# Furyton/Recommender-Baseline-Model

Measured on AMD Instinct MI355X. Metric: training sequences/sec, SASRec L=200 d=128 at 1/2/4/8 MI355X; HR@10 parity, higher is better.
Workload: dtype bf16; 1 GPU; SASRec ML-1M shape (|items|=3416, seq_len=200, d=128, 2 blocks, 1 head, dropout 0.2); model=SASRec, global_batch=128, per_gpu_batch=128, seq_len=200, hidden=128, blocks=2, heads=1, num_items=3416, parallelism=dp1, hip_graph=True, bench_config=cfg2, sampler=host, steps_per_graph=10, full=False

## Files before the change

include/recsys_hip.h:

```cpp
#ifndef RECSYS_HIP_H
#define RECSYS_HIP_H
#include <stdint.h>
#ifdef __cplusplus
extern "C" {
#endif

#define RS_ERR_ARG 1001
#define RS_ERR_UNSUPPORTED 1002

typedef struct rs_epilogue {
  const float* bias;
  float alpha;
  int act;
  const void* aux;
  void* aux_out;
  int64_t ldaux;
  float drop_p;
  uint64_t drop_seed;
  const uint64_t* seed_base;
  int64_t drop_ld;
  const void* resid;
  int64_t ldres;
  const int64_t* rowmask_ids;
  int accumulate;
// ... 153 lines not shown
#define RS_STAMP_WGRAD_GROUPED 2
#define RS_STAMP_VOCAB_CE_FWD 3
int rs_kernel_stamps(uint64_t* buf, const double* step, int kind_mask);
int rs_kernel_stamp_count(void);
int rs_kernel_stamp_kinds(int* kinds, int n);
int rs_wall_clock_khz(int* khz);

int rs_seed_advance(uint64_t* seed_base, void* stream);
int rs_graph_upload(void* graph_exec, void* stream);

#ifdef __HIPCC__
typedef __bf16 rs_bf16;
#else
typedef uint16_t rs_bf16;
#endif

typedef struct rs_sas_embed_args {
  const int64_t* ids;
  const rs_bf16* item_emb;
  const rs_bf16* pos_emb;
  int64_t T;
  float scale;
  float drop_p;
  uint64_t salt;
  const uint64_t* seed_base;
  rs_bf16* x0;
  const int64_t* count_ids;
  int* count_parts;
} rs_sas_embed_args;

typedef struct rs_sas_in_args {
  int64_t M;
  const rs_bf16* x;
  int64_t ldx;
  const float* ln_w;
  const float* ln_b;
  float eps;
  rs_bf16* Q;
  float* mean;
  float* rstd;
  const rs_bf16* Wq;
  const float* bq;
  rs_bf16* q;
  const rs_bf16* Wkv;
  const float* bkv;
  rs_bf16* kv;
  rs_sas_embed_args e;
} rs_sas_in_args;

typedef struct rs_sas_head_args {
  const rs_bf16* E;
  const int64_t* pos;
  const int64_t* neg;
  const float* ln_w;
  const float* ln_b;
  float eps;
  const int* count_parts;
  int ncount;
  const float* divisor;
  rs_bf16* f;
  float* pl;
  float* nl;
  float* dpl;
  float* dnl;
  rs_bf16* dx;
  float* lnpart;
  float* part;
} rs_sas_head_args;

typedef struct rs_sas_out_args {
  int64_t M;
  const rs_bf16* o;
  const rs_bf16* Q;
  const rs_bf16* Wo;
  const float* bo;
  rs_bf16* x1;
  const float* ln_w;
  const float* ln_b;
  float eps;
  rs_bf16* z;
  float* mean;
  float* rstd;
  const rs_bf16* W1;
  const float* b1;
  rs_bf16* h1;
  const rs_bf16* W2;
  const float* b2;
  rs_bf16* xn;
  const int64_t* ids;
  float drop_p;
  uint64_t salt1;
  uint64_t salt2;
  const uint64_t* seed_base;
  rs_sas_head_args h;
} rs_sas_out_args;

typedef struct rs_sas_out_bwd_args {
  int64_t M;
  const rs_bf16* dxn;
  const int64_t* ids;
  const rs_bf16* h1;
  const rs_bf16* x1;
  const float* mean2;
  const float* rstd2;
  const float* ln_w;
  const rs_bf16* W2T;
  const rs_bf16* W1T;
  const rs_bf16* WoT;
  rs_bf16* dy2;
  rs_bf16* da1;
  rs_bf16* dx1;
  rs_bf16* dout;
  float* part;
  float drop_p;
  uint64_t salt1;
  uint64_t salt2;
  const uint64_t* seed_base;
  const rs_bf16* o;
  float* delta;
} rs_sas_out_bwd_args;

typedef struct rs_sas_in_bwd_args {
  int64_t M;
  const rs_bf16* dq;
  const rs_bf16* dkv;
  const rs_bf16* dx1;
  const rs_bf16* x;
  const float* mean1;
  const float* rstd1;
  const float* ln_w;
  const rs_bf16* WinT;
  int64_t ldwt;
  rs_bf16* dx;
  float* part;
} rs_sas_in_bwd_args;

int64_t rs_sas_block_grid(int64_t M);
int rs_sas_block_boundary_fused(int64_t M, int64_t d);

int rs_sas_block_in(int64_t d, const rs_sas_in_args* in, void* stream);
int rs_sas_block_out(int64_t d, const rs_sas_out_args* out, void* stream);
int rs_sas_block_out_bwd_delta(int64_t d, const rs_sas_out_bwd_args* out_bwd, void* stream);
int rs_sas_block_out_bwd(int64_t M, int64_t d, const void* dxn, const int64_t* ids, const void* h1, const void* x1,
                         const float* mean2, const float* rstd2, const float* ln_w, const void* W2T, const void* W1T,
                         const void* WoT, void* dy2, void* da1, void* dx1, void* dout, float* part, float drop_p,
                         uint64_t salt1, uint64_t salt2, const uint64_t* seed_base, void* stream);
int rs_sas_block_in_bwd(int64_t d, const rs_sas_in_bwd_args* in_bwd, void* stream);
int rs_sas_block_out_in(int64_t d, const rs_sas_out_args* out, const rs_sas_in_args* in, void* stream);
int rs_sas_block_in_out_bwd(int64_t d, const rs_sas_in_bwd_args* in_bwd, const rs_sas_out_bwd_args* out_bwd,
                            void* stream);
int rs_sas_block_out_head_bwd(int64_t d, const rs_sas_out_args* out, const rs_sas_out_bwd_args* out_bwd,
                              void* stream);

int64_t rs_touched_rows_ws_numel(int64_t rows);
int rs_touched_rows(const int64_t* ids, int64_t n, int64_t rows, int32_t* flags, int32_t* index, int32_t* count,
                    int32_t* ws, void* stream);
int rs_rows_pack(const float* src, int64_t rows, int64_t d, const int32_t* index, const int32_t* count,
                 float* compact, int64_t cap, void* stream);
int rs_rows_unpack(float* dst, int64_t rows, int64_t d, const int32_t* index, const float* compact, void* stream);

int64_t rs_unique_rows_ws_bytes(int64_t table_rows);
int rs_unique_rows(const int64_t* keys0, int64_t n0, const int64_t* keys1, int64_t n1, const int64_t* keys2,
                   int64_t n2, int64_t table_rows, int32_t* rows, int32_t* count, int64_t cap, void* ws,
                   int64_t ws_bytes, void* stream);
int rs_adam_rows(int64_t d, int64_t table_rows, const int32_t* rows, const int32_t* count, int64_t cap, float* p,
                 float* g, float* m, float* v, void* p_bf16, const double* state, const double* hyper, int zero_grad,
                 int max_wg, void* stream);

int rs_sgd_step(int64_t n, float* p, float* g, float* buf, void* p_bf16, double* state, const double* hyper,
                int zero_grad, int prepare, const float* grad_divisor, uint64_t* seed_base, const int64_t* tdesc,
                int ntd, int64_t tbase, void* wT, const float* loss_sum, float* loss_out, int max_wg, void* stream);

int rs_transpose_bf16(int64_t nmat, const int64_t* desc, int64_t max_tiles, const void* src, void* dst,
                      void* stream);

typedef struct {
  const void* dY; int64_t lddy;
  const void* X;  int64_t ldx;
  int64_t N, K;
  float* dW;
  float* db;
} rs_wgrad_problem;
typedef struct {
  const float* src; int64_t stride; int64_t splits; int64_t n; float* out;
} rs_reduce_segment;
int64_t rs_wgrad_grouped_slab_numel(int nprob, const rs_wgrad_problem* probs, int64_t M, int64_t rows_per_split);
int rs_wgrad_grouped_tile(int nprob, const rs_wgrad_problem* probs);
int rs_wgrad_grouped_tile_max(int nprob, const rs_wgrad_problem* probs, int max_tile);
int rs_wgrad_grouped(int nprob, const rs_wgrad_problem* probs, int64_t M, int64_t rows_per_split, float* slab,
                     int64_t slab_numel, int nextra, const rs_reduce_segment* extra, void* stream);
int rs_wgrad_grouped_max(int nprob, const rs_wgrad_problem* probs, int64_t M, int64_t rows_per_split, float* slab,
                         int64_t slab_numel, int nextra, const rs_reduce_segment* extra, int max_tile, void* stream);

int rs_wgrad_grouped_pos(int nprob, const rs_wgrad_problem* probs, int64_t M, int64_t rows_per_split, float* slab,
                         int64_t slab_numel, int nextra, const rs_reduce_segment* extra, const int64_t* ids,
                         int64_t T, const void* dx, int64_t d, float drop_p, uint64_t salt,
                         const uint64_t* seed_base, float* dpos, void* stream);
int rs_wgrad_grouped_pos_stats(int nprob, const rs_wgrad_problem* probs, int64_t M, int64_t rows_per_split,
                               float* slab, int64_t slab_numel, int nextra, const rs_reduce_segment* extra,
                               const int64_t* ids, int64_t T, const void* dx, int64_t d, float drop_p, uint64_t salt,
                               const uint64_t* seed_base, float* dpos, const float* head_part, int64_t head_blocks,
                               const float* head_divisor, float* loss_out, float* aux_out, void* stream);
int rs_reduce_segments(int nseg, const rs_reduce_segment* segs, int accumulate, void* stream);

int64_t rs_item_index_ws_bytes(int nsrc, int64_t rows, int64_t table_rows, int64_t d);
int rs_item_index_build(int nsrc, const int64_t* keys0, const int64_t* keys1, const int64_t* keys2, int64_t rows,
                        int64_t table_rows, int64_t d, void* ws, int64_t ws_bytes, void* stream);
int rs_item_index_layout(int nsrc, int64_t rows, int64_t table_rows, int64_t d, int64_t* out);
int rs_item_grad(const void* ws, int nsrc, int64_t rows, int64_t table_rows, int64_t d, const void* dx, float scale,
                 float drop_p, uint64_t salt, const uint64_t* seed_base, const void* f, const float* w1,
                 const float* w2, float* dtable, void* stream);
int rs_item_grad_marked(const void* ws, int nsrc, int64_t rows, int64_t table_rows, int64_t d, const void* dx,
                        float scale, float drop_p, uint64_t salt, const uint64_t* seed_base, const void* f,
                        const float* w1, const float* w2, float* dtable, uint8_t* row_marks, uint8_t* epoch_out,
                        void* stream);
int rs_item_grad_f32(const void* ws, int nsrc, int64_t rows, int64_t table_rows, int64_t d, const float* dx, float scale,
                     float drop_p, uint64_t salt, const uint64_t* seed_base, const float* f, const float* w1,
                     const float* w2, float* dtable, void* stream);

int rs_sas_head_fwd(int64_t M, int64_t d, const void* x, const float* ln_w, const float* ln_b, float eps, void* f,
                    float* mean, float* rstd, const void* E, const int64_t* pos, const int64_t* neg, float* pl,
                    float* nl, float* part, void* stream);
int rs_sas_head_bwd(int64_t M, int64_t d, const float* part, const float* divisor, float* out, const float* pl,
                    const float* nl, const float* dpl_in, const float* dnl_in, float* dpl, float* dnl,
                    const int64_t* pos, const int64_t* neg, const void* E, const void* x, const float* ln_w,
                    const float* mean, const float* rstd, void* dx, float* lnpart, void* stream);
int rs_sas_head_finish(int64_t nblk, const float* part, const float* divisor, float* out, void* stream);

int rs_sas_sample(const int64_t* user_offsets, const int64_t* user_items, int64_t n_users, int64_t item_num,
                  int64_t batch, int64_t max_len, uint64_t* seed_base, uint64_t salt, int64_t* seq, int64_t* pos,
                  int64_t* neg, void* stream);
int rs_bert_mask(const int64_t* user_offsets, const int64_t* user_items, int64_t n_users, int64_t num_items,
                 int64_t batch, int64_t max_len, double mask_prob, const int64_t* perm, uint64_t* state, uint64_t salt,
                 int64_t* tokens, int64_t* labels, void* stream);
int rs_sas_sample_draws(const int64_t* user_offsets, const int64_t* user_items, int64_t n_users, int64_t item_num,
                        int64_t batch, int64_t max_len, uint64_t* seed_base, uint64_t salt, int64_t* seq, int64_t* pos,
                        int64_t* neg, int64_t* draws, void* stream);
int rs_bert_mask_draws(const int64_t* user_offsets, const int64_t* user_items, int64_t n_users, int64_t num_items,
                       int64_t batch, int64_t max_len, double mask_prob, const int64_t* perm, uint64_t* state,
                       uint64_t salt, int64_t* tokens, int64_t* labels, int64_t* draws, void* stream);

int rs_rank_metrics(const float* scores, const float* labels, int64_t rows, int64_t cands, int nk, const int* ks,
                    float* ws, float* out, void* stream);

#define RS_TOPK_MAX 128
int64_t rs_full_ws_bytes(int dtype, int64_t B, int64_t d, int64_t nrange, int64_t K);
int rs_full_rank(int dtype, const void* h, int64_t ldh, int64_t B, int64_t d, const void* E, int64_t lde,
                 const float* bias, int64_t v_lo, int64_t v_hi, const int64_t* target, const int64_t* excl, int64_t nx,
                 int64_t ldx, void* ws, int* rank, float* target_score, void* stream);
int rs_full_topk(int dtype, const void* h, int64_t ldh, int64_t B, int64_t d, const void* E, int64_t lde,
                 const float* bias, int64_t v_lo, int64_t v_hi, const int64_t* excl, int64_t nx, int64_t ldx, int64_t K,
                 void* ws, int64_t* ids, float* scores, void* stream);
int rs_rank_to_metrics(const int* rank, int64_t rows, int nk, const int* ks, float* ws, float* out, void* stream);

int rs_sas_ce_rows_fwd(int dtype, int64_t M, int64_t d, const void* x, int64_t ldx, const int64_t* labels,
                       int64_t cap, const float* gamma, const float* beta, float eps, int32_t* idx, int32_t* rank,
                       int32_t* count, float* divisor, void* hl, int64_t ldh, int64_t* lab, float* mean, float* rstd,
                       void* stream);
int64_t rs_sas_ce_rows_nparts(int64_t M);
int rs_sas_ce_rows_bwd(int dtype, int64_t M, int64_t d, const float* slab, int splits, int64_t cap,
                       const int32_t* rank, const void* x, int64_t ldx, const float* gamma, const float* mean,
                       const float* rstd, void* dx, int64_t lddx, float* part, void* stream);

int64_t rs_sas_sce_max_k(void);
int64_t rs_sas_sce_ws_bytes(int64_t cap, int64_t K, int64_t d);
int64_t rs_sas_sce_dh_splits(int64_t cap, int64_t K, int64_t d);
int rs_sas_sce_fwd(int dtype, int64_t cap, int64_t d, const void* hl, int64_t ldh, const int64_t* lab,
                   const int32_t* count, const void* E, int64_t V1, const int64_t* cand, int64_t K,
                   const float* divisor, void* ws, float* out, void* stream);
int rs_sas_sce_bwd(int dtype, int64_t cap, int64_t d, const void* hl, int64_t ldh, const int64_t* lab,
                   const int32_t* count, const void* E, int64_t V1, const int64_t* cand, int64_t K,
                   const float* divisor, const float* dloss, void* ws, float* dh, float* coef, float* pg, float* dEc,
                   int64_t* keys, void* stream);
int rs_uniform_items(const uint64_t* seed_base, uint64_t salt, int64_t item_num, int64_t K, int64_t* out,
                     void* stream);

int64_t rs_sce_head_ws_bytes(int dtype, int64_t cap, int64_t K, int64_t d, int has_bias);
int64_t rs_sce_head_dh_splits(int dtype, int64_t cap, int64_t K, int64_t d);
int rs_sce_head_path(int dtype, int64_t d);
int rs_sce_head_fwd(int dtype, int64_t cap, int64_t d, const void* hl, int64_t ldh, const int64_t* lab,
                    const int32_t* count, const void* E, const float* bias, int64_t V1, const int64_t* cand, int64_t K,
                    const float* divisor, void* ws, float* out, void* stream);
int rs_sce_head_bwd(int dtype, int64_t cap, int64_t d, const void* hl, int64_t ldh, const int64_t* lab,
                    const int32_t* count, const void* E, const float* bias, int64_t V1, const int64_t* cand, int64_t K,
                    const float* divisor, const float* dloss, void* ws, float* dh, float* coef, float* pg, float* dEc,
                    float* dbc, int64_t* keys, void* stream);

int rs_sce_head_logq_fwd(int dtype, int64_t cap, int64_t d, const void* hl, int64_t ldh, const int64_t* lab,
                         const int32_t* count, const void* E, const float* bias, const float* logq, int64_t V1,
                         const int64_t* cand, int64_t K, const float* divisor, void* ws, float* out, void* stream);
int rs_sce_head_logq_bwd(int dtype, int64_t cap, int64_t d, const void* hl, int64_t ldh, const int64_t* lab,
                         const int32_t* count, const void* E, const float* bias, const float* logq, int64_t V1,
                         const int64_t* cand, int64_t K, const float* divisor, const float* dloss, void* ws, float* dh,
                         float* coef, float* pg, float* dEc, float* dbc, int64_t* keys, void* stream);
int rs_alias_items(const uint64_t* seed_base, uint64_t salt, const uint64_t* table, int64_t item_num, int64_t K,
                   int64_t* out, void* stream);

int rs_abi_version(void);
enum {
  RS_SIZEOF_EPILOGUE = 0,
  RS_SIZEOF_WGRAD_PROBLEM = 1,
  RS_SIZEOF_REDUCE_SEGMENT = 2,
  RS_SIZEOF_SAS_EMBED_ARGS = 3,
  RS_SIZEOF_SAS_IN_ARGS = 4,
  RS_SIZEOF_SAS_HEAD_ARGS = 5,
  RS_SIZEOF_SAS_OUT_ARGS = 6,
  RS_SIZEOF_SAS_OUT_BWD_ARGS = 7,
  RS_SIZEOF_SAS_IN_BWD_ARGS = 8
};
int64_t rs_abi_sizeof(int which);

#ifdef __cplusplus
}
#endif
#endif
```

recommender-baseline-model_amd/_lib.py:

```python
import ctypes as C
import os

import torch

PKG = os.path.dirname(os.path.abspath(__file__))
LIB_PATH = os.path.join(PKG, "librecsys_hip.so" if not os.environ.get("RS_LIB_VARIANT")
                        else f"librecsys_hip.{os.environ['RS_LIB_VARIANT']}.so")

F32, BF16 = 0, 1

i32, i64, u64, f32, f64, vp = C.c_int, C.c_int64, C.c_uint64, C.c_float, C.c_double, C.c_void_p


class Epilogue(C.Structure):
    _fields_ = [
        ("bias", vp), ("alpha", f32), ("act", i32),
        ("aux", vp), ("aux_out", vp), ("ldaux", i64),
        ("drop_p", f32), ("drop_seed", u64), ("seed_base", vp), ("drop_ld", i64),
        ("resid", vp), ("ldres", i64),
        ("rowmask_ids", vp), ("accumulate", i32),
        ("post_drop_p", f32), ("post_drop_seed", u64), ("rows_dev", vp),
    ]


class WgradProblem(C.Structure):
    _fields_ = [("dY", vp), ("lddy", i64), ("X", vp), ("ldx", i64), ("N", i64), ("K", i64), ("dW", vp), ("db", vp)]


class ReduceSegment(C.Structure):
    _fields_ = [("src", vp), ("stride", i64), ("splits", i64), ("n", i64), ("out", vp)]


class SasEmbedArgs(C.Structure):
    _fields_ = [("ids", vp), ("item_emb", vp), ("pos_emb", vp), ("T", i64), ("scale", f32), ("drop_p", f32),
                ("salt", u64), ("seed_base", vp), ("x0", vp), ("count_ids", vp), ("count_parts", vp)]


class SasInArgs(C.Structure):
    _fields_ = [("M", i64), ("x", vp), ("ldx", i64), ("ln_w", vp), ("ln_b", vp), ("eps", f32), ("Q", vp),
                ("mean", vp), ("rstd", vp), ("Wq", vp), ("bq", vp), ("q", vp), ("Wkv", vp), ("bkv", vp), ("kv", vp),
                ("e", SasEmbedArgs)]


class SasHeadArgs(C.Structure):
    _fields_ = [("E", vp), ("pos", vp), ("neg", vp), ("ln_w", vp), ("ln_b", vp), ("eps", f32), ("count_parts", vp),
                ("ncount", i32), ("divisor", vp), ("f", vp), ("pl", vp), ("nl", vp), ("dpl", vp), ("dnl", vp),
                ("dx", vp), ("lnpart", vp), ("part", vp)]


class SasOutArgs(C.Structure):
    _fields_ = [("M", i64), ("o", vp), ("Q", vp), ("Wo", vp), ("bo", vp), ("x1", vp), ("ln_w", vp), ("ln_b", vp),
                ("eps", f32), ("z", vp), ("mean", vp), ("rstd", vp), ("W1", vp), ("b1", vp), ("h1", vp), ("W2", vp),
                ("b2", vp), ("xn", vp), ("ids", vp), ("drop_p", f32), ("salt1", u64), ("salt2", u64),
                ("seed_base", vp), ("h", SasHeadArgs)]


class SasOutBwdArgs(C.Structure):
    _fields_ = [("M", i64), ("dxn", vp), ("ids", vp), ("h1", vp), ("x1", vp), ("mean2", vp), ("rstd2", vp),
                ("ln_w", vp), ("W2T", vp), ("W1T", vp), ("WoT", vp), ("dy2", vp), ("da1", vp), ("dx1", vp),
                ("dout", vp), ("part", vp), ("drop_p", f32), ("salt1", u64), ("salt2", u64), ("seed_base", vp),
                ("o", vp), ("delta", vp)]


class SasInBwdArgs(C.Structure):
    _fields_ = [("M", i64), ("dq", vp), ("dkv", vp), ("dx1", vp), ("x", vp), ("mean1", vp), ("rstd1", vp),
                ("ln_w", vp), ("WinT", vp), ("ldwt", i64), ("dx", vp), ("part", vp)]


STRUCTS = {"rs_epilogue": Epilogue, "rs_wgrad_problem": WgradProblem, "rs_reduce_segment": ReduceSegment,
           "rs_sas_embed_args": SasEmbedArgs, "rs_sas_in_args": SasInArgs, "rs_sas_head_args": SasHeadArgs,
           "rs_sas_out_args": SasOutArgs, "rs_sas_out_bwd_args": SasOutBwdArgs, "rs_sas_in_bwd_args": SasInBwdArgs}

ACT_NONE, ACT_RELU, ACT_GELU, ACT_RELU_BWD, ACT_GELU_BWD = 0, 1, 2, 3, 4

SIGNATURES = {
    "rs_gemm": [i32, i32, i32, i64, i64, i64, vp, i64, vp, i64, vp, i64, i32, C.POINTER(Epilogue), i32, vp, vp],
    "rs_gemm_ln": [i64, i64, i64, vp, i64, vp, vp, f32, vp, i64, vp, i64, C.POINTER(Epilogue), vp, i64, vp, vp, vp],
    "rs_reduce_slabs": [vp, i32, i64, vp, i32, vp],
    "rs_reduce_slabs2": [vp, i32, i64, vp, i64, vp, i32, vp],
    "rs_linear_wgrad": [i32, i64, i64, i64, vp, i64, vp, i64, vp, vp, i32, i32, vp, vp, vp],
    "rs_colsum": [i32, vp, i64, i64, i64, vp, vp, i32, vp],
    "rs_embed_fwd": [i32, i32, vp, i64, i64, vp, vp, i64, f32, f32, u64, vp, vp, vp],
    "rs_embed_bwd": [i32, i32, vp, i64, i64, vp, i64, f32, f32, u64, vp, vp, vp, i32, vp],
    "rs_layernorm_fwd": [i32, i32, vp, i64, i64, i64, vp, vp, f32, vp, i64, vp, vp, vp],
    "rs_layernorm_bwd_nparts": [i32, i64, i64],
    "rs_layernorm_bwd_drop": [i32, i32, vp, i64, vp, i64, i64, i64, vp, vp, vp, f32, vp, i64, i32, vp, vp, vp, f32,
                              u64, u64, vp, vp, vp, vp],
    "rs_layernorm_bwd": [i32, i32, vp, i64, vp, i64, i64, i64, vp, vp, vp, f32, vp, i64, i32, vp, vp, vp, vp],
    "rs_attn_fwd": [i32, i64, i64, i64, i64, vp, i64, vp, i64, vp, i64, vp, i64, vp, f32, i32, vp, f32, u64, vp, vp],
    "rs_attn_row_delta": [i32, i64, i64, i64, i64, vp, i64, vp, i64, vp, vp],
    "rs_attn_bwd": [i32, i64, i64, i64, i64, vp, i64, vp, i64, vp, i64, vp, i64, vp, i64, vp, vp, i64, vp, i64,
                    vp, i64, f32, i32, vp, f32, u64, vp, vp, vp],
    "rs_sampled_logits_fwd": [i32, vp, i64, i64, vp, vp, vp, vp, vp, vp],
    "rs_sampled_logits_bwd": [i32, vp, i64, i64, vp, vp, vp, vp, vp, vp, i32, vp, vp],
    "rs_bce_fwd": [vp, vp, vp, i64, vp, vp, vp, vp],
    "rs_bce_bwd": [vp, vp, vp, i64, vp, vp, vp, vp, vp],
    "rs_ce_fwd": [vp, i64, i64, i64, vp, vp, vp, vp, vp, vp],
    "rs_ce_bwd": [i32, vp, i64, i64, i64, vp, vp, vp, vp, vp, i64, vp, vp],
    "rs_compact_rows": [vp, i64, i64, vp, vp, vp, vp],
    "rs_gather_rows": [i32, vp, i64, i64, vp, vp, i64, vp, i64, vp, vp, vp],
    "rs_scatter_rows": [i32, vp, i64, i64, vp, i64, vp, i64, vp],
    "rs_candidate_scores": [i32, vp, i64, i64, i64, vp, vp, vp, i64, i64, vp, vp],
    "rs_gemm_n256_splits": [i64, i64],
    "rs_gemm_n256": [i32, i64, i64, vp, i64, vp, i64, vp, i64, i32, i64, vp, vp, vp],
    "rs_adam_prepare": [vp, vp, vp, vp, vp],
    "rs_adam_step": [i64, vp, vp, vp, vp, vp, vp, vp, i32, vp],
    "rs_adam_step_wg": [i64, vp, vp, vp, vp, vp, vp, vp, i32, i32, vp],
    "rs_adam_step_marked": [i64, vp, vp, vp, vp, vp, vp, vp, i32, i32, vp, vp, i64, i64, i32, vp],
    "rs_graph_upload": [vp, vp],
    "rs_adam_prepare_step": [i64, vp, vp, vp, vp, vp, vp, vp, i32, vp, vp, vp, i32, i64, vp, vp],
    "rs_adam_prepare_step_loss": [i64, vp, vp, vp, vp, vp, vp, vp, i32, vp, vp, vp, i32, i64, vp, vp, vp, vp],
    "rs_adam_prepare_step_marked": [i64, vp, vp, vp, vp, vp, vp, vp, i32, vp, vp, vp, i32, i64, vp, vp, vp, vp, vp,
                                    i64, i64, i32, vp],
    "rs_cast_bf16": [i64, vp, vp, vp],
    "rs_l2_penalty": [vp, vp, vp, i64, f32, vp, vp, vp, vp],
    "rs_dropout_rowmask": [i32, vp, i64, i64, i64, f32, u64, vp, i64, vp, vp, vp, vp],
    "rs_dropout2": [i32, vp, i64, i64, i64, f32, u64, u64, vp, i64, vp, vp, vp],
    "rs_vocab_ce_ws_numel": [i64, i64],
    "rs_vocab_ce_fwd": [i64, i64, i64, vp, i64, vp, i64, vp, vp, vp, vp, vp, vp, vp],
    "rs_vocab_ce_bwd": [i64, i64, i64, vp, i64, vp, i64, vp, vp, vp, vp, vp, vp, vp, i64, vp],
    "rs_vocab_head_supported": [i64],
    "rs_vocab_head_fwd": [i64, i64, i64, vp, i64, vp, i64, vp, vp, vp, vp, vp, vp, vp],
    "rs_vocab_head_bwd": [i64, i64, i64, vp, i64, vp, i64, vp, vp, vp, vp, vp, vp, vp, i64, i64, vp],
    "rs_vocab_shard_lse": [i64, i64, i64, vp, i64, vp, i64, vp, vp, vp, vp, vp],
    "rs_vocab_shard_label_logits": [i64, i64, vp, i64, vp, i64, vp, vp, i64, i64, vp, vp],
    "rs_vocab_shard_combine": [i32, i64, vp, vp, vp, vp, vp, vp],
    "rs_seed_advance": [vp, vp],
    "rs_touched_rows_ws_numel": [i64],
    "rs_touched_rows": [vp, i64, i64, vp, vp, vp, vp, vp],
    "rs_rows_pack": [vp, i64, i64, vp, vp, vp, i64, vp],
    "rs_rows_unpack": [vp, i64, i64, vp, vp, vp],
    "rs_unique_rows_ws_bytes": [i64],
    "rs_unique_rows": [vp, i64, vp, i64, vp, i64, i64, vp, vp, i64, vp, i64, vp],
    "rs_adam_rows": [i64, i64, vp, vp, i64, vp, vp, vp, vp, vp, vp, vp, i32, i32, vp],
    "rs_sgd_step": [i64, vp, vp, vp, vp, vp, vp, i32, i32, vp, vp, vp, i32, i64, vp, vp, vp, i32, vp],
    "rs_sas_block_grid": [i64],
    "rs_sas_block_boundary_fused": [i64, i64],
    "rs_sas_block_in": [i64, C.POINTER(SasInArgs), vp],
    "rs_sas_block_out": [i64, C.POINTER(SasOutArgs), vp],
    "rs_sas_block_out_bwd_delta": [i64, C.POINTER(SasOutBwdArgs), vp],
    "rs_sas_block_out_bwd": [i64, i64, vp, vp, vp, vp, vp, vp, vp, vp, vp, vp, vp, vp, vp, vp, vp, f32, u64, u64,
                             vp, vp],
    "rs_sas_block_in_bwd": [i64, C.POINTER(SasInBwdArgs), vp],
    "rs_sas_block_out_in": [i64, C.POINTER(SasOutArgs), C.POINTER(SasInArgs), vp],
    "rs_sas_block_in_out_bwd": [i64, C.POINTER(SasInBwdArgs), C.POINTER(SasOutBwdArgs), vp],
    "rs_sas_block_out_head_bwd": [i64, C.POINTER(SasOutArgs), C.POINTER(SasOutBwdArgs), vp],
    "rs_wgrad_grouped": [i32, C.POINTER(WgradProblem), i64, i64, vp, i64, i32, C.POINTER(ReduceSegment), vp],
    "rs_reduce_segments": [i32, C.POINTER(ReduceSegment), i32, vp],
    "rs_wgrad_grouped_slab_numel": [i32, C.POINTER(WgradProblem), i64, i64],
    "rs_wgrad_grouped_tile": [i32, C.POINTER(WgradProblem)],
    "rs_wgrad_grouped_tile_max": [i32, C.POINTER(WgradProblem), i32],
    "rs_wgrad_grouped_max": [i32, C.POINTER(WgradProblem), i64, i64, vp, i64, i32, C.POINTER(ReduceSegment), i32, vp],
    "rs_item_index_ws_bytes": [i32, i64, i64, i64],
    "rs_item_index_build": [i32, vp, vp, vp, i64, i64, i64, vp, i64, vp],
    "rs_item_index_layout": [i32, i64, i64, i64, C.POINTER(i64)],
    "rs_sas_head_fwd": [i64, i64, vp, vp, vp, f32, vp, vp, vp, vp, vp, vp, vp, vp, vp, vp],
    "rs_sas_head_finish": [i64, vp, vp, vp, vp],
    "rs_sas_head_bwd": [i64, i64, vp, vp, vp, vp, vp, vp, vp, vp, vp, vp, vp, vp, vp, vp, vp, vp, vp, vp, vp],
    "rs_item_grad": [vp, i32, i64, i64, i64, vp, f32, f32, u64, vp, vp, vp, vp, vp, vp],
    "rs_item_grad_marked": [vp, i32, i64, i64, i64, vp, f32, f32, u64, vp, vp, vp, vp, vp, vp, vp, vp],
    "rs_item_grad_f32": [vp, i32, i64, i64, i64, vp, f32, f32, u64, vp, vp, vp, vp, vp, vp],
    "rs_wgrad_grouped_pos": [i32, C.POINTER(WgradProblem), i64, i64, vp, i64, i32, C.POINTER(ReduceSegment),
                             vp, i64, vp, i64, f32, u64, vp, vp, vp],
    "rs_wgrad_grouped_pos_stats": [i32, C.POINTER(WgradProblem), i64, i64, vp, i64, i32, C.POINTER(ReduceSegment),
                                   vp, i64, vp, i64, f32, u64, vp, vp, vp, i64, vp, vp, vp, vp],
    "rs_transpose_bf16": [i64, vp, i64, vp, vp, vp],
    "rs_sas_sample": [vp, vp, i64, i64, i64, i64, vp, u64, vp, vp, vp, vp],
    "rs_bert_mask": [vp, vp, i64, i64, i64, i64, f64, vp, vp, u64, vp, vp, vp],
    "rs_sas_sample_draws": [vp, vp, i64, i64, i64, i64, vp, u64, vp, vp, vp, vp, vp],
    "rs_bert_mask_draws": [vp, vp, i64, i64, i64, i64, f64, vp, vp, u64, vp, vp, vp, vp],
    "rs_splitk_scatter_rows": [i32, vp, i32, i64, i64, vp, i64, vp, i64, vp],
    "rs_rank_metrics": [vp, vp, i64, i64, i32, vp, vp, vp, vp],
    "rs_full_ws_bytes": [i32, i64, i64, i64, i64],
    "rs_full_rank": [i32, vp, i64, i64, i64, vp, i64, vp, i64, i64, vp, vp, i64, i64, vp, vp, vp, vp],
    "rs_full_topk": [i32, vp, i64, i64, i64, vp, i64, vp, i64, i64, vp, i64, i64, i64, vp, vp, vp, vp],
    "rs_rank_to_metrics": [vp, i64, i32, vp, vp, vp, vp],
    "rs_sas_ce_rows_fwd": [i32, i64, i64, vp, i64, vp, i64, vp, vp, f32, vp, vp, vp, vp, vp, i64, vp, vp, vp, vp],
    "rs_sas_ce_rows_nparts": [i64],
    "rs_sas_ce_rows_bwd": [i32, i64, i64, vp, i32, i64, vp, vp, i64, vp, vp, vp, vp, i64, vp, vp],
    "rs_sas_sce_max_k": [],
    "rs_sas_sce_ws_bytes": [i64, i64, i64],
    "rs_sas_sce_dh_splits": [i64, i64, i64],
    "rs_sas_sce_fwd": [i32, i64, i64, vp, i64, vp, vp, vp, i64, vp, i64, vp, vp, vp, vp],
    "rs_sas_sce_bwd": [i32, i64, i64, vp, i64, vp, vp, vp, i64, vp, i64, vp, vp, vp, vp, vp, vp, vp, vp, vp],
    "rs_uniform_items": [vp, u64, i64, i64, vp, vp],
    "rs_sce_head_ws_bytes": [i32, i64, i64, i64, i32],
    "rs_sce_head_dh_splits": [i32, i64, i64, i64],
    "rs_sce_head_path": [i32, i64],
    "rs_sce_head_fwd": [i32, i64, i64, vp, i64, vp, vp, vp, vp, i64, vp, i64, vp, vp, vp, vp],
    "rs_sce_head_bwd": [i32, i64, i64, vp, i64, vp, vp, vp, vp, i64, vp, i64, vp, vp, vp, vp, vp, vp, vp, vp, vp,
                        vp],
    "rs_sce_head_logq_fwd": [i32, i64, i64, vp, i64, vp, vp, vp, vp, vp, i64, vp, i64, vp, vp, vp, vp],
    "rs_sce_head_logq_bwd": [i32, i64, i64, vp, i64, vp, vp, vp, vp, vp, i64, vp, i64, vp, vp, vp, vp, vp, vp, vp, vp,
                             vp, vp],
    "rs_alias_items": [vp, u64, vp, i64, i64, vp, vp],
    "rs_kernel_stamps": [vp, vp, i32],
    "rs_kernel_stamp_count": [],
    "rs_kernel_stamp_kinds": [C.POINTER(i32), i32],
    "rs_wall_clock_khz": [C.POINTER(i32)],
    "rs_attn_bwd_plan": [i64, i64, i64, i32, vp, C.POINTER(i32)],
    "rs_attn_lds_regime": [i32, i64, i64, i64, i64, i32, C.POINTER(i32)],
    "rs_abi_version": [],
    "rs_abi_sizeof": [i32],
}

RESTYPES = {"rs_wgrad_grouped_slab_numel": C.c_int64, "rs_abi_sizeof": C.c_int64,
            "rs_touched_rows_ws_numel": C.c_int64, "rs_item_index_ws_bytes": C.c_int64,
            "rs_unique_rows_ws_bytes": C.c_int64,
            "rs_vocab_ce_ws_numel": C.c_int64, "rs_full_ws_bytes": C.c_int64,
            "rs_sas_block_grid": C.c_int64, "rs_layernorm_bwd_nparts": C.c_int64,
            "rs_sas_ce_rows_nparts": C.c_int64, "rs_sas_sce_max_k": C.c_int64,
            "rs_sas_sce_ws_bytes": C.c_int64, "rs_sas_sce_dh_splits": C.c_int64,
            "rs_sce_head_ws_bytes": C.c_int64, "rs_sce_head_dh_splits": C.c_int64}

_lib = None


def lib():
    global _lib
    if _lib is None:
        if not os.path.exists(LIB_PATH):
            raise RuntimeError(
                f"librecsys_hip.so not found at {LIB_PATH}; build it with "
                "`python recommender-baseline-model_amd/build.py` (there is no CPU fallback)")
        h = C.CDLL(LIB_PATH)
        for name, argt in SIGNATURES.items():
            fn = getattr(h, name)
            fn.argtypes = argt
            fn.restype = RESTYPES.get(name, C.c_int)
        _lib = h
    return _lib


def call(name, *args):
    rc = getattr(lib(), name)(*args)
    if rc != 0:
        raise RuntimeError(f"{name} failed with code {rc}")


def ptr(t):
    return None if t is None else t.data_ptr()


def stream():
    return torch.cuda.current_stream().cuda_stream
```

recommender-baseline-model_amd/build.py:

```python
import concurrent.futures as cf
import glob
import os
import subprocess
import sys

PKG = os.path.dirname(os.path.abspath(__file__))
ROOT = os.path.dirname(PKG)
CSRC = os.path.join(PKG, "csrc")
OBJ = os.path.join(CSRC, "build")
LIB = os.path.join(PKG, "librecsys_hip.so")
HIPCC = os.environ.get("HIPCC", "/opt/rocm/bin/hipcc")
ARCH = os.environ.get("RS_OFFLOAD_ARCH", "gfx950")
LINK_LAST = ("sas_ce.hip", "sas_sce.hip", "adam_rows.hip", "sgd.hip")
FLAGS = ["-O3", "-std=c++17", "-fPIC", f"--offload-arch={ARCH}", "-munsafe-fp-atomics",
         "-I", os.path.join(ROOT, "include"), "-I", CSRC]


def _headers_mtime():
    hs = glob.glob(os.path.join(CSRC, "*.h")) + glob.glob(os.path.join(ROOT, "include", "*.h"))
    return max((os.path.getmtime(h) for h in hs), default=0.0)


def _included(path):
    with open(path) as fh:
        return fh.readline().startswith("// rs-build: included")


def _included_mtime():
    inc = [p for p in glob.glob(os.path.join(CSRC, "*.hip")) if _included(p)]
    return max((os.path.getmtime(p) for p in inc), default=0.0)


def _compile(src, force):
    obj = os.path.join(OBJ, os.path.basename(src) + ".o")
    if not force and os.path.exists(obj):
        if os.path.getmtime(obj) >= max(os.path.getmtime(src), _headers_mtime(), _included_mtime()):
            return obj, False
    cmd = [HIPCC, *FLAGS, "-c", src, "-o", obj]
    r = subprocess.run(cmd, capture_output=True, text=True)
    if r.returncode != 0:
        raise RuntimeError(f"hipcc failed for {src}:\n{r.stdout}\n{r.stderr}")
    return obj, True


def build(force=False, jobs=None):
    os.makedirs(OBJ, exist_ok=True)
    srcs = [p for p in sorted(glob.glob(os.path.join(CSRC, "*.hip"))) if not _included(p)]
    srcs.sort(key=lambda p: LINK_LAST.index(os.path.basename(p)) + 1 if os.path.basename(p) in LINK_LAST else 0)
    jobs = jobs or min(len(srcs), max(1, min(8, os.cpu_count() or 1)))
    with cf.ThreadPoolExecutor(jobs) as ex:
        results = list(ex.map(lambda s: _compile(s, force), srcs))
    objs = [o for o, _ in results]
    rebuilt = any(b for _, b in results)
    if rebuilt or force or not os.path.exists(LIB) or \
            os.path.getmtime(LIB) < max(os.path.getmtime(o) for o in objs):
        cmd = [HIPCC, "-shared", "-fPIC", f"--offload-arch={ARCH}", *objs, "-o", LIB]
        r = subprocess.run(cmd, capture_output=True, text=True)
        if r.returncode != 0:
            raise RuntimeError(f"link failed:\n{r.stdout}\n{r.stderr}")
    return LIB


if __name__ == "__main__":
    print(build(force="--force" in sys.argv))
```

recommender-baseline-model_amd/csrc/attention_lds.hip:

```cpp
#include "common.h"
#include <algorithm>
#include <cstring>
#include "../../include/recsys_hip.h"

typedef __attribute__((ext_vector_type(4))) __bf16 bf4;
typedef __bf16 bf16;

#define PLAN_S 4
#define PLAN_I 6
struct AttnLdsArgs {
  int64_t B, T, H;
  const bf16* q; int64_t ldq;
  const bf16* k; int64_t ldk;
  const bf16* v; int64_t ldv;
  const bf16* o; int64_t ldo;
  const bf16* dout; int64_t lddo;
  bf16* out; int64_t ldout;
  bf16* dq; int64_t lddq;
  bf16* dk; int64_t lddk;
  bf16* dv; int64_t lddv;
  float* lse;
  float* delta;
  int delta_in;
  float scale;
// ... 67 lines not shown
  u4 v = *reinterpret_cast<const u4*>(base + rc * ld + col);
  const unsigned keep = row < T ? 0xffffffffu : 0u;
  v &= keep;
  return __builtin_bit_cast(bf16x8, v);
}

typedef __attribute__((address_space(3))) void* lds_ptr_t;
__device__ __forceinline__ uint32_t lds_addr(const void* p) { return (uint32_t)(uintptr_t)(lds_ptr_t)p; }
__device__ __forceinline__ void dma16(const void* gsrc, uint32_t dst) {
  unsigned keep;
  asm volatile("s_mov_b32 %0, m0\n\ts_mov_b32 m0, %2\n\ts_nop 0\n\tglobal_load_lds_dwordx4 %1, off\n\ts_mov_b32 m0, %0"
               : "=&s"(keep)
               : "v"(gsrc), "s"(dst)
               : "memory");
}
template <int N> __device__ __forceinline__ void vm_wait_n() { asm volatile("s_waitcnt vmcnt(%0)" ::"i"(N) : "memory"); }
#define LOADER (NW - 1)
#define NCNT 16
template <int DH> struct DmaStage {
  static constexpr int ROWB = Img<DH>::LD * 2, CHB = 32 * ROWB, PPC = CHB / 1024, PP = 2 * PPC, WIN = 3;
  static_assert(CHB % 1024 == 0, "a 32-row chunk is whole DMA pieces");
  static_assert(WIN * PP <= 63, "chunks in flight fit vmcnt");
  static __device__ __forceinline__ void chunk(const bf16* A, int64_t ldA, uint32_t la, const bf16* B, int64_t ldB,
                                               uint32_t lb, int T, int c, int lane) {
#pragma unroll
    for (int j = 0; j < PP; ++j) {
      const bool second = j >= PPC;
      const int pj = second ? j - PPC : j;
      const int off = c * CHB + pj * 1024 + lane * 16;
      const int row = off / ROWB, o = off - row * ROWB;
      const int col = o < DH * 2 ? o >> 1 : 0;
      const int64_t rr = row < T ? row : T - 1;
      const bf16* src = second ? B + rr * ldB + col : A + rr * ldA + col;
      dma16(src, __builtin_amdgcn_readfirstlane((second ? lb : la) + (uint32_t)(c * CHB + pj * 1024)));
    }
  }
  static __device__ __forceinline__ void prime(const bf16* A, int64_t ldA, const bf16* imgA, const bf16* B,
                                               int64_t ldB, const bf16* imgB, int T, int nch, int lane) {
    const uint32_t la = lds_addr(imgA), lb = lds_addr(imgB);
    for (int c = 0; c < min(nch, WIN); ++c) chunk(A, ldA, la, B, ldB, lb, T, c, lane);
  }
  static __device__ __forceinline__ void stream(const bf16* A, int64_t ldA, const bf16* imgA, const bf16* B,
                                                int64_t ldB, const bf16* imgB, int T, int nch, int* flag, int lane) {
    const uint32_t la = lds_addr(imgA), lb = lds_addr(imgB);
    for (int c = 0; c < nch; ++c) {
      const int later = min(nch, c + WIN) - (c + 1);
      if (later >= 2) vm_wait_n<2 * PP>();
      else if (later == 1) vm_wait_n<PP>();
      else vm_wait_n<0>();
      if (lane == 0) __hip_atomic_store(&flag[c], 1, __ATOMIC_RELAXED, __HIP_MEMORY_SCOPE_WORKGROUP);
      if (c + WIN < nch) chunk(A, ldA, la, B, ldB, lb, T, c + WIN, lane);
    }
  }
};
struct ChunkWait {
  const int* flag;
  int nch, ready;
  __device__ __forceinline__ void ensure(int c) {
    c = min(c, nch - 1);
    if (c <= ready) return;
    for (int spin = 0; spin < (1 << 22) &&
                       __hip_atomic_load(&flag[c], __ATOMIC_RELAXED, __HIP_MEMORY_SCOPE_WORKGROUP) == 0;
         ++spin)
      __builtin_amdgcn_s_sleep(1);
    asm volatile("" ::: "memory");
    ready = c;
  }
};
__device__ __forceinline__ void lds_barrier() {
  asm volatile("s_waitcnt lgkmcnt(0)" ::: "memory");
  __builtin_amdgcn_s_barrier();
  asm volatile("" ::: "memory");
}

template <int DH>
__device__ __forceinline__ void stage(bf16* img, const bf16* src, int64_t ld, int64_t T, int rows, int tid) {
  constexpr int CPR = DH / 8, LD = Img<DH>::LD, U = 8;
  const int n = rows * CPR;
  for (int i0 = tid; i0 < n; i0 += NT * U) {
    bf16x8 v[U];
#pragma unroll
    for (int u = 0; u < U; ++u) {
      const int i = min(i0 + u * NT, n - 1);
      v[u] = gload8(src, ld, i / CPR, T, (i % CPR) * 8);
    }
#pragma unroll
    for (int u = 0; u < U; ++u) {
      const int i = i0 + u * NT;
      if (i < n) *reinterpret_cast<bf16x8*>(img + (i / CPR) * LD + (i % CPR) * 8) = v[u];
    }
  }
}

template <int DH>
__device__ __forceinline__ void stage2(bf16* imgA, const bf16* srcA, int64_t ldA, bf16* imgB, const bf16* srcB,
                                       int64_t ldB, int64_t T, int rows, int tid) {
  constexpr int CPR = DH / 8, LD = Img<DH>::LD, U = 8;
  const int n = rows * CPR;
  for (int i0 = tid; i0 < n; i0 += NT * U) {
    bf16x8 va[U], vb[U];
#pragma unroll
    for (int u = 0; u < U; ++u) {
      const int i = min(i0 + u * NT, n - 1);
      va[u] = gload8(srcA, ldA, i / CPR, T, (i % CPR) * 8);
      vb[u] = gload8(srcB, ldB, i / CPR, T, (i % CPR) * 8);
    }
#pragma unroll
    for (int u = 0; u < U; ++u) {
      const int i = i0 + u * NT;
      if (i < n) {
        *reinterpret_cast<bf16x8*>(imgA + (i / CPR) * LD + (i % CPR) * 8) = va[u];
        *reinterpret_cast<bf16x8*>(imgB + (i / CPR) * LD + (i % CPR) * 8) = vb[u];
      }
    }
  }
}

__device__ __forceinline__ void stage_keymask(float* km, const AttnLdsArgs& a, int64_t b, int rows, int tid) {
  for (int i = tid; i < rows; i += NT)
    km[i] = (a.mask_kind == 1 && i < a.T && a.ids[b * a.T + i] == 0) ? 1.f : 0.f;
}

__device__ __forceinline__ int mask_state(const AttnLdsArgs& a, const float* km, int64_t q, int64_t key) {
  if (key >= a.T) return 1;
  if (a.mask_kind == 0) return key > q ? 1 : 0;
  return km[key] != 0.f ? 2 : 0;
}
__device__ __forceinline__ float apply_mask(int st, float s) { return st == 0 ? s : (st == 1 ? NEG_INF : -1e9f); }
__device__ __forceinline__ float masked(const AttnLdsArgs& a, const float* km, int64_t q, int64_t key, float s) {
  return apply_mask(mask_state(a, km, q, key), s);
}

__device__ __forceinline__ void block_coords(const AttnLdsArgs& a, int64_t lin, int64_t& bh, int& split) {
  const int ns = a.nsplit;
  const int64_t BH = a.B * a.H;
  if (BH % 8 == 0) {
    const int64_t xcd = lin & 7, slot = lin >> 3;
    bh = xcd * (BH >> 3) + slot / ns;
    split = (int)(slot % ns);
  } else {
    bh = lin / ns;
    split = (int)(lin % ns);
  }
}
__device__ __forceinline__ void block_coords(const AttnLdsArgs& a, int64_t& bh, int& split) {
  block_coords(a, blockIdx.x + (int64_t)a.nsplit * blockIdx.y, bh, split);
}

__device__ __forceinline__ int last_tile_of_split(int nq, int split, int nsplit) {
  return split + ((nq - 1 - split) / nsplit) * nsplit;
}

template <int DH>
__global__ __launch_bounds__(NT) void attn_fwd_lds_kernel(AttnLdsArgs a) {
  constexpr int LD = Img<DH>::LD, KC = DH / 32, DT = DH / 16, NKT = 16;
  extern __shared__ __attribute__((aligned(16))) char smem[];
  APROF(0);
  const int tid = threadIdx.x, lane = tid & 63, wave = __builtin_amdgcn_readfirstlane(tid >> 6), g = lane >> 4, cl = lane & 15;
  int64_t bh;
  int split;
  block_coords(a, bh, split);
  const int64_t b = bh / a.H, h = bh % a.H;
  const int T = (int)a.T;
  const int nq = (T + 15) / 16;
  if (split >= nq) return;
  const int lastq = last_tile_of_split(nq, split, a.nsplit);
  const int kneed = a.mask_kind == 0 ? min(T, 16 * (lastq + 1)) : T;
  const int rows = ((kneed + 31) / 32) * 32;
  bf16* Ks = reinterpret_cast<bf16*>(smem);
  bf16* Vs = Ks + rows * LD;
  float* km = reinterpret_cast<float*>(Vs + rows * LD);
  const bf16* Kg = a.k + b * a.T * a.ldk + h * DH;
  const bf16* Vg = a.v + b * a.T * a.ldv + h * DH;
  const bf16* Qg = a.q + b * a.T * a.ldq + h * DH;
  bf16x8 qf[KC];
  {
    const int64_t qrow0 = (split + wave * a.nsplit) * 16 + cl;
#pragma unroll
    for (int kc = 0; kc < KC; ++kc) qf[kc] = gload8(Qg, a.ldq, qrow0, a.T, kc * 32 + 8 * g);
  }
  stage2<DH>(Ks, Kg, a.ldk, Vs, Vg, a.ldv, a.T, rows, tid);
  stage_keymask(km, a, b, rows, tid);
  __syncthreads();
  APROF(1);
  const uint64_t seed = eff_seed(a.seed, a.seed_base);
  if (wave >= NW / 2) __builtin_amdgcn_s_setprio(1);

  for (int qt = split + wave * a.nsplit; qt < nq; qt += NW * a.nsplit) {
    const int q0 = qt * 16;
    const int64_t qrow = q0 + cl;
    if (qt != split + wave * a.nsplit) {
#pragma unroll
      for (int kc = 0; kc < KC; ++kc) qf[kc] = gload8(Qg, a.ldq, qrow, a.T, kc * 32 + 8 * g);
    }
    const int nkt = a.mask_kind == 0 ? qt + 1 : nq;
    const float sl2 = a.scale * LOG2E;
    const int qi = q0 + cl;
    f32x4 s[NKT];
    float mx = NEG_INF;
#pragma unroll
    for (int kt = 0; kt < NKT; ++kt) {
      s[kt] = (f32x4){0.f, 0.f, 0.f, 0.f};
      if (kt < nkt) {
#pragma unroll
        for (int kc = 0; kc < KC; ++kc) s[kt] = mfma16(row_frag(Ks, LD, kt * 16 + cl, kc * 32 + 8 * g), qf[kc], s[kt]);
        const bool need = a.mask_kind != 0 || kt == qt || kt * 16 + 16 > T;
        const int kb = kt * 16 + 4 * g;
        if (need) {
          const f32x4 kmv = *reinterpret_cast<const f32x4*>(km + kb);
#pragma unroll
          for (int r = 0; r < 4; ++r) {
            const int k = kb + r;
            const bool dead = (k >= T) | ((a.mask_kind == 0) & (k > qi));
            const float x = s[kt][r] * sl2;
            s[kt][r] = dead ? NEG_INF : (kmv[r] != 0.f ? MASK2 : x);
            mx = fmaxf(mx, s[kt][r]);
          }
        } else {
#pragma unroll
          for (int r = 0; r < 4; ++r) {
            s[kt][r] *= sl2;
            mx = fmaxf(mx, s[kt][r]);
          }
        }
      }
    }
    mx = max_xor32(max_xor16(mx));
    float sm = 0.f;
#pragma unroll
    for (int kt = 0; kt < NKT; ++kt) {
      if (kt < nkt) {
#pragma unroll
        for (int r = 0; r < 4; ++r) {
          const float e = ex2(s[kt][r] - mx);
          s[kt][r] = e;
          sm += e;
        }
      }
    }
    sm = add_xor32(add_xor16(sm));
    const float inv = 1.f / sm;
    if (g == 0 && qrow < a.T) a.lse[bh * a.T + qrow] = (mx + __builtin_amdgcn_logf(sm)) * LN2;
    const uint32_t s32 = seed32(seed);
    const uint32_t rowidx = (uint32_t)(((int)bh * T + qi) * (T + (T & 1)));
    f32x4 o[DT];
#pragma unroll
    for (int dt = 0; dt < DT; ++dt) o[dt] = (f32x4){0.f, 0.f, 0.f, 0.f};
#pragma unroll
    for (int c = 0; c < NKT / 2; ++c) {
      if (2 * c < nkt) {
        f32x4 pp[2] = {s[2 * c], s[2 * c + 1]};
#pragma unroll
        for (int hf = 0; hf < 2; ++hf) {
          const int t = 2 * c + hf;
          const float sc = t < nkt ? inv : 0.f;
          if (a.drop_p > 0.f) {
            float m[4];
            const uint32_t base = rowidx + (uint32_t)(t * 16 + 4 * g);
            drop_mul2(a.drop_p, s32, base, m[0], m[1]);
            drop_mul2(a.drop_p, s32, base + 2, m[2], m[3]);
#pragma unroll
            for (int r = 0; r < 4; ++r) pp[hf][r] *= sc * m[r];
          } else {
#pragma unroll
            for (int r = 0; r < 4; ++r) pp[hf][r] *= sc;
          }
        }
        const bf16x8 pb = pack8(pp[0], pp[1]);
#pragma unroll
        for (int dt = 0; dt < DT; ++dt) o[dt] = mfma16(tr_frag(Vs, LD, 32 * c, 16 * dt, lane), pb, o[dt]);
      }
    }
    if (qrow < a.T) {
      bf16* O = a.out + (b * a.T + qrow) * a.ldout + h * DH;
#pragma unroll
      for (int dt = 0; dt < DT; ++dt) {
        bf4 w;
        w[0] = (bf16)o[dt][0]; w[1] = (bf16)o[dt][1]; w[2] = (bf16)o[dt][2]; w[3] = (bf16)o[dt][3];
        *reinterpret_cast<bf4*>(O + 16 * dt + 4 * g) = w;
      }
    }
  }
  APROF(2);
}

template <int DH>
__device__ __forceinline__ void attn_bwd_dq_body(const AttnLdsArgs& a, int64_t lin) {
  constexpr int LD = Img<DH>::LD, KC = DH / 32, DT = DH / 16;
  extern __shared__ __attribute__((aligned(16))) char smem[];
  APROF(4);
  const int tid = threadIdx.x, lane = tid & 63, wave = __builtin_amdgcn_readfirstlane(tid >> 6), g = lane >> 4, cl = lane & 15;
  int64_t bh;
  int split;
  block_coords(a, lin, bh, split);
  const int64_t b = bh / a.H, h = bh % a.H;
  const int T = (int)a.T;
  const int nq = (T + 15) / 16;
  if (split >= nq) return;
  const int lastq = last_tile_of_split(nq, split, a.nsplit);
  const int kneed = a.mask_kind == 0 ? min(T, 16 * (lastq + 1)) : T;
  const int rows = ((kneed + 31) / 32) * 32;
  bf16* Ks = reinterpret_cast<bf16*>(smem);
  bf16* Vs = Ks + rows * LD;
  float* km = reinterpret_cast<float*>(Vs + rows * LD);
  int* cnt = reinterpret_cast<int*>(km + rows);
  float* slots = km + rows + NCNT;
  int* flags = reinterpret_cast<int*>(slots + DQ_SLOTS * DT * 4 * 64);
  const bf16* Qg = a.q + b * a.T * a.ldq + h * DH;
  const bf16* Og = a.o + b * a.T * a.ldo + h * DH;
  const bf16* dOg = a.dout + b * a.T * a.lddo + h * DH;
  auto item = [&](int it, int& qt, int& cb, int& ce, int& role, int& slot) -> bool {
    if (a.use_plan) {
      if (it >= PLAN_I) return false;
      const uint32_t e = a.plan[split][wave][it];
      if (!(e >> 31)) return false;
      qt = e & 255; cb = (e >> 8) & 255; ce = (e >> 16) & 255; role = (e >> 24) & 3; slot = (e >> 26) & 15;
      return true;
    }
    qt = split + (wave + it * NW) * a.nsplit;
    if (qt >= nq) return false;
    cb = 0;
    ce = ((a.mask_kind == 0 ? qt + 1 : nq) + 1) / 2;
    role = 0; slot = 0;
    return true;
  };
  if (a.use_plan && tid < DQ_SLOTS) flags[tid] = 0;
  if (tid < NCNT) cnt[tid] = 0;
  const int nch = rows / 32;
  bf16x8 qf[KC], df[KC], of[KC];
  int qt0 = 0, cb0, ce0, role0, slot0;
  const bool any = item(0, qt0, cb0, ce0, role0, slot0);
  const bf16* Kg = a.k + b * a.T * a.ldk + h * DH;
  const bf16* Vg = a.v + b * a.T * a.ldv + h * DH;
  if (wave == LOADER) {
    DmaStage<DH>::prime(Kg, a.ldk, Ks, Vg, a.ldv, Vs, T, nch, lane);
  } else {
    const int64_t qrow0 = (any ? qt0 : 0) * 16 + cl;
#pragma unroll
    for (int kc = 0; kc < KC; ++kc) {
      qf[kc] = gload8(Qg, a.ldq, qrow0, a.T, kc * 32 + 8 * g);
      df[kc] = gload8(dOg, a.lddo, qrow0, a.T, kc * 32 + 8 * g);
      if (!a.delta_in) of[kc] = gload8(Og, a.ldo, qrow0, a.T, kc * 32 + 8 * g);
    }
  }
  stage_keymask(km, a, b, rows, tid);
  lds_barrier();
  if (wave == LOADER) DmaStage<DH>::stream(Kg, a.ldk, Ks, Vg, a.ldv, Vs, T, nch, cnt, lane);
  ChunkWait ch{cnt, nch, wave == LOADER ? nch - 1 : -1};
  APROF(5);
  const uint64_t seed = eff_seed(a.seed, a.seed_base);

  if (wave >= NW / 2) __builtin_amdgcn_s_setprio(1);
  int qt, cb, ce, role, slot;
  for (int it = 0; item(it, qt, cb, ce, role, slot); ++it) {
    const int q0 = qt * 16;
    const int64_t qrow = q0 + cl;
    if (it > 0 || wave == LOADER) {
#pragma unroll
      for (int kc = 0; kc < KC; ++kc) {
        qf[kc] = gload8(Qg, a.ldq, qrow, a.T, kc * 32 + 8 * g);
        df[kc] = gload8(dOg, a.lddo, qrow, a.T, kc * 32 + 8 * g);
        if (!a.delta_in) of[kc] = gload8(Og, a.ldo, qrow, a.T, kc * 32 + 8 * g);
      }
    }
    float dl = 0.f;
    if (a.delta_in) {
      dl = a.delta[bh * a.T + (qrow < a.T ? qrow : a.T - 1)];
    } else {
#pragma unroll
      for (int kc = 0; kc < KC; ++kc) {
#pragma unroll
        for (int j = 0; j < 8; ++j) dl += (float)df[kc][j] * (float)of[kc][j];
      }
      dl = add_xor32(add_xor16(dl));
      if (role != 1 && g == 0 && qrow < a.T) a.delta[bh * a.T + qrow] = dl;
    }
    const float lq2 = (qrow < a.T ? a.lse[bh * a.T + qrow] : 0.f) * LOG2E;
    const float sl2 = a.scale * LOG2E;
    const int qi = q0 + cl;
    const uint32_t s32 = seed32(seed);
    const uint32_t rowidx = (uint32_t)(((int)bh * T + qi) * (T + (T & 1)));
    const bool qok = qi < T;
    const int nkt = a.mask_kind == 0 ? qt + 1 : nq;
    f32x4 acc[DT];
#pragma unroll
    for (int dt = 0; dt < DT; ++dt) acc[dt] = (f32x4){0.f, 0.f, 0.f, 0.f};
    const int tmax = rows / 16 - 1;
    auto sdp = [&](int t, f32x4& sv, f32x4& dp) {
      const int tr = min(t, tmax);
      bf16x8 fk[KC], fv[KC];
#pragma unroll
      for (int kc = 0; kc < KC; ++kc) {
        fk[kc] = row_frag(Ks, LD, tr * 16 + cl, kc * 32 + 8 * g);
        fv[kc] = row_frag(Vs, LD, tr * 16 + cl, kc * 32 + 8 * g);
      }
      sv = (f32x4){0.f, 0.f, 0.f, 0.f};
      dp = (f32x4){0.f, 0.f, 0.f, 0.f};
#pragma unroll
      for (int kc = 0; kc < KC; ++kc) {
        sv = mfma16(fk[kc], qf[kc], sv);
        dp = mfma16(fv[kc], df[kc], dp);
      }
    };
    auto dsv = [&](int t, const f32x4& sv, const f32x4& dp, f32x4& ds) {
      const bool need = a.mask_kind != 0 || t >= qt || t * 16 + 16 > T;
      const int kb = t * 16 + 4 * g;
      float m[4] = {1.f, 1.f, 1.f, 1.f};
      if (a.drop_p > 0.f) {
        drop_mul2(a.drop_p, s32, rowidx + (uint32_t)kb, m[0], m[1]);
        drop_mul2(a.drop_p, s32, rowidx + (uint32_t)kb + 2, m[2], m[3]);
      }
      const bool tok = (t < nkt) & qok, causal = a.mask_kind == 0;
      float pe[4];
#pragma unroll
      for (int r = 0; r < 4; ++r) pe[r] = ex2(sv[r] * sl2 - lq2) * a.scale;
      if (need) {
        const f32x4 kmv = *reinterpret_cast<const f32x4*>(km + kb);
#pragma unroll
        for (int r = 0; r < 4; ++r) {
          const int k = kb + r;
          const bool live = tok & (k < T) & !(causal & (k > qi)) & (kmv[r] == 0.f);
          const float v = pe[r] * (dp[r] * m[r] - dl);
          ds[r] = live ? v : 0.f;
        }
      } else {
#pragma unroll
        for (int r = 0; r < 4; ++r) ds[r] = tok ? pe[r] * (dp[r] * m[r] - dl) : 0.f;
      }
    };
    f32x4 sA, dA, sB, dB, dsA, dsB;
    ch.ensure(cb);
    sdp(2 * cb, sA, dA);
    for (int c = cb; c < ce; ++c) {
      sdp(2 * c + 1, sB, dB);
      dsv(2 * c, sA, dA, dsA);
      if (c + 1 < ce) ch.ensure(c + 1);
      sdp(2 * c + 2, sA, dA);
      dsv(2 * c + 1, sB, dB, dsB);
// ... 173 lines not shown
    for (int dt = 0; dt < DT; ++dt) {
      dk[dt] = (f32x4){0.f, 0.f, 0.f, 0.f};
      dv[dt] = (f32x4){0.f, 0.f, 0.f, 0.f};
    }
    const int tmax = rows / 16 - 1;
    auto sdp = [&](int t, f32x4& sv, f32x4& dp) {
      const int tr = min(t, tmax);
      bf16x8 fq[KC], fo[KC];
#pragma unroll
      for (int kc = 0; kc < KC; ++kc) {
        fq[kc] = row_frag(Qs, LD, tr * 16 + cl, kc * 32 + 8 * g);
        fo[kc] = row_frag(dOs, LD, tr * 16 + cl, kc * 32 + 8 * g);
      }
      sv = (f32x4){0.f, 0.f, 0.f, 0.f};
      dp = (f32x4){0.f, 0.f, 0.f, 0.f};
#pragma unroll
      for (int kc = 0; kc < KC; ++kc) {
        sv = mfma16(fq[kc], kf[kc], sv);
        dp = mfma16(fo[kc], vf[kc], dp);
      }
    };
    const bool kdead = ki >= T, kfill = km[min(ki, rows - 1)] != 0.f;
    auto pds = [&](int t, const f32x4& sv, const f32x4& dp, f32x4& pd, f32x4& ds) {
      const f32x4 ls = *reinterpret_cast<const f32x4*>(lse_s + t * 16 + 4 * g);
      const f32x4 dd = *reinterpret_cast<const f32x4*>(dl_s + t * 16 + 4 * g);
      float m[4] = {1.f, 1.f, 1.f, 1.f};
      if (a.drop_p > 0.f) drop_keys4(a.drop_p, s32, ((uint32_t)bh * (uint32_t)T + (uint32_t)(t * 16 + 4 * g)) * Tp,
                                     Tp, (uint32_t)ki, lane, m);
      const bool need = a.mask_kind != 0 || t <= kt || t * 16 + 16 > T || kt * 16 + 16 > T;
      if (need) {
#pragma unroll
        for (int r = 0; r < 4; ++r) {
          const int qr = t * 16 + 4 * g + r;
          const bool dead = kdead | (qr >= T) | ((a.mask_kind == 0) & (ki > qr));
          const float x2 = kfill ? MASK2 : sv[r] * sl2;
          const float p = ex2(dead ? NEG_INF : x2 - ls[r]);
          pd[r] = p * m[r];
          const float v = p * (dp[r] * m[r] - dd[r]) * a.scale;
          ds[r] = dead | kfill ? 0.f : v;
        }
      } else {
#pragma unroll
        for (int r = 0; r < 4; ++r) {
          const float p = ex2(sv[r] * sl2 - ls[r]);
          pd[r] = p * m[r];
          ds[r] = p * (dp[r] * m[r] - dd[r]) * a.scale;
        }
      }
    };
    f32x4 sA, dA, sB, dB, pdA, dsA, pdB, dsB;
    ch.ensure(cb);
    sdp(2 * cb, sA, dA);
    for (int c = cb; c < ce; ++c) {
      sdp(2 * c + 1, sB, dB);
      pds(2 * c, sA, dA, pdA, dsA);
      if (c + 1 < ce) ch.ensure(c + 1);
      sdp(2 * c + 2, sA, dA);
      pds(2 * c + 1, sB, dB, pdB, dsB);
      const bf16x8 bp = pack8(pdA, pdB);
      const bf16x8 bds = pack8(dsA, dsB);
#pragma unroll
      for (int dt = 0; dt < DT; ++dt) {
        dv[dt] = mfma16(tr_frag(dOs, LD, 32 * c, 16 * dt, lane), bp, dv[dt]);
        dk[dt] = mfma16(tr_frag(Qs, LD, 32 * c, 16 * dt, lane), bds, dk[dt]);
      }
    }
    bf16* sl = slots + slot * (2 * DT * 4 * 64);
    if (role == 1) {
#pragma unroll
      for (int dt = 0; dt < DT; ++dt)
#pragma unroll
        for (int r = 0; r < 4; ++r) {
          sl[(dt * 4 + r) * 64 + lane] = (bf16)dk[dt][r];
          sl[(DT * 4 + dt * 4 + r) * 64 + lane] = (bf16)dv[dt][r];
        }
      asm volatile("s_waitcnt lgkmcnt(0)" ::: "memory");
      if (lane == 0) __hip_atomic_store(&flags[slot], 1, __ATOMIC_RELAXED, __HIP_MEMORY_SCOPE_WORKGROUP);
      continue;
    }
    if (role == 2) {
      for (int spin = 0; spin < (1 << 22) &&
                         __hip_atomic_load(&flags[slot], __ATOMIC_RELAXED, __HIP_MEMORY_SCOPE_WORKGROUP) == 0;
           ++spin)
        __builtin_amdgcn_s_sleep(1);
      asm volatile("" ::: "memory");
#pragma unroll
      for (int dt = 0; dt < DT; ++dt)
#pragma unroll
        for (int r = 0; r < 4; ++r) {
          dk[dt][r] += (float)sl[(dt * 4 + r) * 64 + lane];
          dv[dt][r] += (float)sl[(DT * 4 + dt * 4 + r) * 64 + lane];
        }
    }
    if (key < a.T) {
      bf16* dK = a.dk + (b * a.T + key) * a.lddk + h * DH;
      bf16* dV = a.dv + (b * a.T + key) * a.lddv + h * DH;
#pragma unroll
      for (int dt = 0; dt < DT; ++dt) {
        bf4 wk, wv;
#pragma unroll
        for (int r = 0; r < 4; ++r) {
          wk[r] = (bf16)dk[dt][r];
          wv[r] = (bf16)dv[dt][r];
        }
        *reinterpret_cast<bf4*>(dK + 16 * dt + 4 * g) = wk;
        *reinterpret_cast<bf4*>(dV + 16 * dt + 4 * g) = wv;
      }
    }
  }
  APROF(9);
}

template <int DH>
__global__ __launch_bounds__(NT) void attn_bwd_lds_kernel(AttnLdsArgs aq, AttnLdsArgs akv) {
  KStampBegin begin_(aq.ks);
  KStampEnd end_(aq.ks);
  const int64_t nq = (int64_t)aq.nsplit * aq.B * aq.H;
  if ((int64_t)blockIdx.x < nq) attn_bwd_dq_body<DH>(aq, blockIdx.x);
  else attn_bwd_dkv_body<DH>(akv, blockIdx.x - nq, !akv.delta_in);
}

template <int DH>
static size_t fwd_lds_bytes(int T) {
  const int rows = ((T + 31) / 32) * 32;
  return (size_t)2 * rows * Img<DH>::LD * 2 + rows * 4 + NCNT * 4;
}
template <int DH>
static size_t dkv_lds_bytes(int T) {
  const int rows = ((T + 31) / 32) * 32;
  return (size_t)2 * rows * Img<DH>::LD * 2 + 3 * rows * 4 + NCNT * 4;
}

static int pick_split(int64_t BH, int ntiles) {
  int s = 1;
  while (BH * s < 256 && s * 2 <= std::max(1, ntiles / 4)) s *= 2;
  return s;
}

static int pick_split_bwd(int64_t BH, int ntiles) {
  int s = 1;
  while (2 * BH * s * 2 <= 256 && s * 2 <= std::max(1, ntiles / 4)) s *= 2;
  return s;
}

bool attn_lds_supported(int64_t T, int64_t Dh) {
  if (T <= 0 || T > 256) return false;
  if (Dh != 32 && Dh != 64 && Dh != 128) return false;
  const size_t need = Dh == 128 ? dkv_lds_bytes<128>((int)T) : Dh == 64 ? dkv_lds_bytes<64>((int)T)
                                                                            : dkv_lds_bytes<32>((int)T);
  return need <= 160 * 1024;
}

static int fwd_split(const AttnLdsArgs& a) { return pick_split(a.B * a.H, (int)cdiv(a.T, 16)); }

template <int DH>
static hipError_t fwd_t(AttnLdsArgs& a, hipStream_t s) {
  a.nsplit = fwd_split(a);
  const size_t lds = fwd_lds_bytes<DH>((int)a.T);
  hipLaunchKernelGGL((attn_fwd_lds_kernel<DH>), dim3((unsigned)a.nsplit, (unsigned)(a.B * a.H)), dim3(NT), lds, s,
                     a);
  return hipGetLastError();
}

#define LOADER_HANDICAP 3
struct PlanItem {
  int tile, cb, ce, role, slot;
};

static bool make_plan(AttnLdsArgs& a, int ntiles, bool dkv, int slots) {
  const int T = (int)a.T, nqc = (T + 31) / 32;
  if (a.nsplit > PLAN_S) return false;
  memset(a.plan, 0, sizeof(a.plan));
  for (int sp = 0; sp < a.nsplit; ++sp) {
    PlanItem items[64];
    int n = 0;
    for (int t = sp; t < ntiles; t += a.nsplit) {
      if (n >= 32) return false;
      items[n++] = dkv ? PlanItem{t, t / 2, nqc, 0, 0} : PlanItem{t, 0, (t + 2) / 2, 0, 0};
    }
    std::sort(items, items + n, [](const PlanItem& x, const PlanItem& y) {
      return x.ce - x.cb != y.ce - y.cb ? x.ce - x.cb > y.ce - y.cb : x.tile < y.tile;
    });
    const int n0 = n;
    for (int k = 0, used = 0; k < n0 && used < slots; ++k) {
      PlanItem& it = items[k];
      const int w = it.ce - it.cb;
      if (w < 2) break;
      const int hmid = it.cb + (w + 1) / 2;
      items[n++] = PlanItem{it.tile, hmid, it.ce, 2, used};
      it.ce = hmid;
      it.role = 1;
      it.slot = used++;
    }
    std::sort(items, items + n, [](const PlanItem& x, const PlanItem& y) {
      return x.ce - x.cb != y.ce - y.cb ? x.ce - x.cb > y.ce - y.cb : x.tile < y.tile;
    });
    int load[NW] = {0}, cnt[NW] = {0};
    load[LOADER] = LOADER_HANDICAP;
    PlanItem lists[NW][PLAN_I];
    for (int k = 0; k < n; ++k) {
      int w = 0;
      for (int j = 1; j < NW; ++j)
        if (load[j] < load[w]) w = j;
      if (cnt[w] == PLAN_I) return false;
      lists[w][cnt[w]++] = items[k];
      load[w] += items[k].ce - items[k].cb;
    }
    for (int w = 0; w < NW; ++w) {
      int o = 0;
      for (int pass = 0; pass < 3; ++pass) {
        const int want = pass == 0 ? 1 : pass == 1 ? 0 : 2;
        for (int k = 0; k < cnt[w]; ++k) {
          const PlanItem& it = lists[w][k];
          if (it.role != want) continue;
          a.plan[sp][w][o++] = 1u << 31 | (uint32_t)it.slot << 26 | (uint32_t)it.role << 24 |
                               (uint32_t)it.ce << 16 | (uint32_t)it.cb << 8 | (uint32_t)it.tile;
        }
      }
    }
  }
  return true;
}

extern "C" int rs_attn_bwd_plan(int64_t B, int64_t T, int64_t H, int dkv, uint32_t* plan, int* nsplit) {
  if (B <= 0 || T <= 0 || H <= 0 || !plan || !nsplit) return RS_ERR_ARG;
  AttnLdsArgs a = {};
  a.B = B; a.T = T; a.H = H; a.mask_kind = 0;
  const int nq = (int)cdiv(T, 16);
  a.nsplit = pick_split_bwd(B * H, nq);
  *nsplit = a.nsplit;
  const bool ok = nq >= 8 && make_plan(a, nq, dkv != 0, dkv ? DKV_SLOTS : DQ_SLOTS);
  memcpy(plan, a.plan, sizeof(a.plan));
  return ok ? 0 : RS_ERR_UNSUPPORTED;
}

template <int DH>
static size_t bwd_setup(AttnLdsArgs& a, AttnLdsArgs& aq, AttnLdsArgs& akv) {
  const int nq = (int)cdiv(a.T, 16);
  a.nsplit = pick_split_bwd(a.B * a.H, nq);
  constexpr int DT = DH / 16;
  const size_t lds_q = fwd_lds_bytes<DH>((int)a.T), lds_kv = dkv_lds_bytes<DH>((int)a.T);
  const size_t ext_q = (size_t)DQ_SLOTS * DT * 4 * 64 * 4 + 16, ext_kv = (size_t)DKV_SLOTS * 2 * DT * 4 * 64 * 2 + 16;
  aq = a;
  akv = a;
  const bool want = a.mask_kind == 0 && nq >= 8;
  aq.use_plan = want && lds_q + ext_q <= 160 * 1024 && make_plan(aq, nq, false, DQ_SLOTS);
  akv.use_plan = want && lds_kv + ext_kv <= 160 * 1024 && make_plan(akv, nq, true, DKV_SLOTS);
  const size_t bq = lds_q + (aq.use_plan ? ext_q : 0), bkv = lds_kv + (akv.use_plan ? ext_kv : 0);
  return std::max(bq, bkv);
}

template <int DH>
static hipError_t bwd_t(AttnLdsArgs& a, hipStream_t s) {
  AttnLdsArgs aq, akv;
  const size_t lds = bwd_setup<DH>(a, aq, akv);
  hipLaunchKernelGGL((attn_bwd_lds_kernel<DH>), dim3((unsigned)(2 * a.nsplit * a.B * a.H)), dim3(NT), lds, s, aq,
                     akv);
  return hipGetLastError();
}

void attn_lds_regime(int64_t B, int64_t T, int64_t H, int64_t Dh, int mask_kind, int* out) {
  AttnLdsArgs a = {}, aq, akv;
  a.B = B; a.T = T; a.H = H; a.mask_kind = mask_kind;
  out[0] = fwd_split(a);
  if (Dh == 128) bwd_setup<128>(a, aq, akv);
  else if (Dh == 64) bwd_setup<64>(a, aq, akv);
  else bwd_setup<32>(a, aq, akv);
  out[1] = a.nsplit;
  out[2] = aq.use_plan;
  out[3] = akv.use_plan;
}

template <int DH>
static void set_lds_limits() {
  hipFuncSetAttribute((const void*)attn_fwd_lds_kernel<DH>, hipFuncAttributeMaxDynamicSharedMemorySize, 160 * 1024);
  hipFuncSetAttribute((const void*)attn_bwd_lds_kernel<DH>, hipFuncAttributeMaxDynamicSharedMemorySize, 160 * 1024);
}

static void init_once() {
  static bool done = false;
  if (!done) {
    set_lds_limits<32>();
    set_lds_limits<64>();
    set_lds_limits<128>();
    done = true;
  }
}

hipError_t attn_lds_fwd(int64_t B, int64_t T, int64_t H, int64_t Dh, const void* q, int64_t ldq, const void* k,
                        int64_t ldk, const void* v, int64_t ldv, void* o, int64_t ldo, float* lse, float scale,
                        int mask_kind, const int64_t* ids, float drop_p, uint64_t seed, const uint64_t* seed_base,
                        hipStream_t s) {
  init_once();
  AttnLdsArgs a = {};
  a.B = B; a.T = T; a.H = H;
  a.q = (const bf16*)q; a.ldq = ldq; a.k = (const bf16*)k; a.ldk = ldk; a.v = (const bf16*)v; a.ldv = ldv;
  a.out = (bf16*)o; a.ldout = ldo; a.lse = lse; a.scale = scale; a.mask_kind = mask_kind; a.ids = ids;
  a.drop_p = drop_p; a.seed = seed; a.seed_base = seed_base;
  if (Dh == 128) return fwd_t<128>(a, s);
  if (Dh == 64) return fwd_t<64>(a, s);
  return fwd_t<32>(a, s);
}

hipError_t attn_lds_bwd(int64_t B, int64_t T, int64_t H, int64_t Dh, const void* q, int64_t ldq, const void* k,
                        int64_t ldk, const void* v, int64_t ldv, const void* o, int64_t ldo, const void* dout,
                        int64_t lddo, const float* lse, void* dq, int64_t lddq, void* dk, int64_t lddk, void* dv,
                        int64_t lddv, float scale, int mask_kind, const int64_t* ids, float drop_p, uint64_t seed,
                        const uint64_t* seed_base, float* delta, hipStream_t s) {
  init_once();
  AttnLdsArgs a = {};
  a.B = B; a.T = T; a.H = H;
  a.delta_in = (mask_kind & RS_ATTN_DELTA_IN) != 0;
  mask_kind &= ~RS_ATTN_DELTA_IN;
  a.q = (const bf16*)q; a.ldq = ldq; a.k = (const bf16*)k; a.ldk = ldk; a.v = (const bf16*)v; a.ldv = ldv;
  a.o = (const bf16*)o; a.ldo = ldo; a.dout = (const bf16*)dout; a.lddo = lddo;
  a.dq = (bf16*)dq; a.lddq = lddq; a.dk = (bf16*)dk; a.lddk = lddk; a.dv = (bf16*)dv; a.lddv = lddv;
  a.lse = const_cast<float*>(lse); a.delta = delta; a.scale = scale; a.mask_kind = mask_kind; a.ids = ids;
  a.drop_p = drop_p; a.seed = seed; a.seed_base = seed_base;
  a.ks = kstamp_next(RS_STAMP_ATTN_BWD);
  if (Dh == 128) return bwd_t<128>(a, s);
  if (Dh == 64) return bwd_t<64>(a, s);
  return bwd_t<32>(a, s);
}
```

recommender-baseline-model_amd/csrc/misc.hip:

```cpp
#include "adam_math.h"
#include "common.h"
#include "stream4.h"
#include "../../include/recsys_hip.h"

__device__ __forceinline__ void adam_commit(double* state, double t, AdamScalars c, uint64_t* seed_base) {
  if (seed_base) *seed_base += 1;
  state[0] = t;
  state[1] = c.step_size;
  state[2] = c.bc2s;
  state[3] = c.gs;
}

__global__ void adam_prepare_kernel(double* state, const double* hyper, const float* divisor, uint64_t* seed_base) {
  if (threadIdx.x != 0 || blockIdx.x != 0) return;
  const double t = state[0] + 1.0;
  adam_commit(state, t, adam_scalars(t, hyper, divisor), seed_base);
}

template <bool BF16OUT, bool NT>
__device__ __forceinline__ void adam4(int64_t i, float4 pp, float4 gg, float4 mm, float4 vv, float* __restrict__ p,
                                      float* __restrict__ g, float* __restrict__ m, float* __restrict__ v,
                                      __bf16* __restrict__ pb, AdamElem h,
                                      float step_size, float bc2s, float gs, int zero_grad,
                                      const int64_t* __restrict__ tdesc, int ntd, int64_t tbase,
// ... 359 lines not shown
  RowMarks rm;
  if (int e = row_marks(n, row_marks_, epoch, moff, mrows, dshift, rm)) return e;
  if (!loss_out != !loss_sum || (loss_out && !grad_divisor)) return RS_ERR_ARG;
  if (ntd < 0 || (ntd > 0 && (!tdesc || !wT || !p_bf16))) return RS_ERR_ARG;
#ifndef ADAM_PREP_MAX_WG
#define ADAM_PREP_MAX_WG 2048
#endif
  const int64_t blocks = std::max<int64_t>(1, std::min<int64_t>(cdiv(n / 4, 256), ADAM_PREP_MAX_WG));
  hipStream_t s = (hipStream_t)stream;
  if (p_bf16)
    ADAM_LAUNCH(true, true, dim3((unsigned)blocks), dim3(256), 0, s, n, p, g, m, v,
                       (__bf16*)p_bf16, state, hyper, zero_grad, grad_divisor, seed_base, tdesc, ntd,
                       tbase, (__bf16*)wT, loss_sum, loss_out);
  else
    ADAM_LAUNCH(false, true, dim3((unsigned)blocks), dim3(256), 0, s, n, p, g, m, v,
                       (__bf16*)nullptr, state, hyper, zero_grad, grad_divisor, seed_base, nullptr, 0,
                       0, nullptr, loss_sum, loss_out);
  return (int)hipGetLastError();
}

int rs_cast_bf16(int64_t n, const float* src, void* dst, void* stream) {
  if (n <= 0) return RS_ERR_ARG;
  const int64_t blocks = std::min<int64_t>(cdiv(n, 256), 8192);
  hipLaunchKernelGGL(cast_bf16_kernel, dim3((unsigned)blocks), dim3(256), 0, (hipStream_t)stream, n, src,
                     (__bf16*)dst);
  return (int)hipGetLastError();
}

int rs_colsum(int dtype, const void* X, int64_t M, int64_t N, int64_t ldx, float* ws, float* out, int accumulate,
              void* stream) {
  if (M <= 0 || N <= 0) return RS_ERR_ARG;
  hipStream_t s = (hipStream_t)stream;
  const int nblk = (int)std::min<int64_t>(COLSUM_BLOCKS, cdiv(M, 64));
  hipError_t e = dtype == RS_DTYPE_BF16 ? colsum_partial<__bf16>((const __bf16*)X, M, N, ldx, ws, nblk, s)
                                        : colsum_partial<float>((const float*)X, M, N, ldx, ws, nblk, s);
  if (e != hipSuccess) return (int)e;
  return (int)launch_reduce_slabs(ws, nblk, N, N, out, nullptr, accumulate, s);
}

int rs_dropout_rowmask(int dtype, const void* x, int64_t M, int64_t N, int64_t ld, float drop_p, uint64_t seed,
                       const uint64_t* seed_base, int64_t drop_ld, const int64_t* rowmask_ids, void* out,
                       void* out_masked, void* stream) {
  if (M <= 0 || N <= 0) return RS_ERR_ARG;
  hipStream_t s = (hipStream_t)stream;
  const int es = dtype == RS_DTYPE_BF16 ? 2 : 4;
  if (N % 8 == 0 && ld % 8 == 0 && drop_ld % 2 == 0 && ((uintptr_t)x | (uintptr_t)out | (uintptr_t)out_masked) % 16 == 0) {
    dim3 g8((unsigned)cdiv(M * (N / 8), 256));
    if (es == 2)
      hipLaunchKernelGGL((dropout_v8_kernel<__bf16, false>), g8, dim3(256), 0, s, (const __bf16*)x, M, N, ld, drop_p,
                         seed, 0ull, seed_base, drop_ld, rowmask_ids, (__bf16*)out, (__bf16*)out_masked);
    else
      hipLaunchKernelGGL((dropout_v8_kernel<float, false>), g8, dim3(256), 0, s, (const float*)x, M, N, ld, drop_p,
                         seed, 0ull, seed_base, drop_ld, rowmask_ids, (float*)out, (float*)out_masked);
    return (int)hipGetLastError();
  }
  dim3 grid((unsigned)cdiv(M * N, 256));
  if (dtype == RS_DTYPE_BF16)
    hipLaunchKernelGGL((dropout_rowmask_kernel<__bf16>), grid, dim3(256), 0, s, (const __bf16*)x, M, N, ld, drop_p,
                       seed, seed_base, drop_ld, rowmask_ids, (__bf16*)out, (__bf16*)out_masked);
  else
    hipLaunchKernelGGL((dropout_rowmask_kernel<float>), grid, dim3(256), 0, s, (const float*)x, M, N, ld, drop_p,
                       seed, seed_base, drop_ld, rowmask_ids, (float*)out, (float*)out_masked);
  return (int)hipGetLastError();
}

int rs_dropout2(int dtype, const void* x, int64_t M, int64_t N, int64_t ld, float drop_p, uint64_t salt1,
                uint64_t salt2, const uint64_t* seed_base, int64_t drop_ld, void* out1, void* out2, void* stream) {
  if (M <= 0 || N <= 0 || N % 8 || ld % 8 || drop_ld % 2 || !x || !out1 || !out2 ||
      ((uintptr_t)x | (uintptr_t)out1 | (uintptr_t)out2) % 16)
    return RS_ERR_ARG;
  hipStream_t s = (hipStream_t)stream;
  dim3 g8((unsigned)cdiv(M * (N / 8), 256));
  if (dtype == RS_DTYPE_BF16)
    hipLaunchKernelGGL((dropout_v8_kernel<__bf16, true>), g8, dim3(256), 0, s, (const __bf16*)x, M, N, ld, drop_p,
                       salt1, salt2, seed_base, drop_ld, (const int64_t*)nullptr, (__bf16*)out1, (__bf16*)out2);
  else
    hipLaunchKernelGGL((dropout_v8_kernel<float, true>), g8, dim3(256), 0, s, (const float*)x, M, N, ld, drop_p,
                       salt1, salt2, seed_base, drop_ld, (const int64_t*)nullptr, (float*)out1, (float*)out2);
  return (int)hipGetLastError();
}

__global__ void seed_advance_kernel(uint64_t* s) {
  if (threadIdx.x == 0) *s += 1;
}

int rs_graph_upload(void* graph_exec, void* stream) {
  if (!graph_exec) return RS_ERR_ARG;
  return (int)hipGraphUpload((hipGraphExec_t)graph_exec, (hipStream_t)stream);
}

int rs_seed_advance(uint64_t* seed_base, void* stream) {
  hipLaunchKernelGGL(seed_advance_kernel, dim3(1), dim3(64), 0, (hipStream_t)stream, seed_base);
  return (int)hipGetLastError();
}

static unsigned long long* g_kstamp_buf = nullptr;
static const double* g_kstamp_step = nullptr;
static int g_kstamp_next = 0, g_kstamp_mask = 0;
static int g_kstamp_kind[256];

}

KStamp kstamp_next(int kind) {
  KStamp k{nullptr, nullptr, 0};
  if (g_kstamp_buf && (g_kstamp_mask >> kind & 1)) {
    k.buf = g_kstamp_buf;
    k.step = g_kstamp_step;
    if (g_kstamp_next < 256) g_kstamp_kind[g_kstamp_next] = kind;
    k.mark = g_kstamp_next++;
  }
  return k;
}

extern "C" {

int rs_kernel_stamps(uint64_t* buf, const double* step, int kind_mask) {
  if ((buf == nullptr) != (step == nullptr)) return RS_ERR_ARG;
  g_kstamp_buf = (unsigned long long*)buf;
  g_kstamp_step = step;
  g_kstamp_mask = kind_mask;
  if (buf) g_kstamp_next = 0;
  return 0;
}

int rs_kernel_stamp_kinds(int* kinds, int n) {
  const int m = g_kstamp_next < 256 ? g_kstamp_next : 256;
  for (int i = 0; i < n && i < m; ++i) kinds[i] = g_kstamp_kind[i];
  return 0;
}

int rs_kernel_stamp_count(void) { return g_kstamp_next; }

int rs_wall_clock_khz(int* khz) {
  if (!khz) return RS_ERR_ARG;
  int dev = 0;
  hipError_t e = hipGetDevice(&dev);
  if (e != hipSuccess) return (int)e;
  return (int)hipDeviceGetAttribute(khz, hipDeviceAttributeWallClockRate, dev);
}

int rs_abi_version(void) { return 2; }

int64_t rs_abi_sizeof(int which) {
  switch (which) {
    case RS_SIZEOF_EPILOGUE: return sizeof(rs_epilogue);
    case RS_SIZEOF_WGRAD_PROBLEM: return sizeof(rs_wgrad_problem);
    case RS_SIZEOF_REDUCE_SEGMENT: return sizeof(rs_reduce_segment);
    case RS_SIZEOF_SAS_EMBED_ARGS: return sizeof(rs_sas_embed_args);
    case RS_SIZEOF_SAS_IN_ARGS: return sizeof(rs_sas_in_args);
    case RS_SIZEOF_SAS_HEAD_ARGS: return sizeof(rs_sas_head_args);
    case RS_SIZEOF_SAS_OUT_ARGS: return sizeof(rs_sas_out_args);
    case RS_SIZEOF_SAS_OUT_BWD_ARGS: return sizeof(rs_sas_out_bwd_args);
    case RS_SIZEOF_SAS_IN_BWD_ARGS: return sizeof(rs_sas_in_bwd_args);
    default: return -1;
  }
}

}
```

recommender-baseline-model_amd/csrc/rowchain.hip:

```cpp
#include "common.h"
#include "../../include/recsys_hip.h"

namespace rc {

#ifdef RC_PROF
__device__ unsigned long long g_rc_prof[4096 * 8 * 16];
#define RCPROF(slot)                                                                                 \
  do {                                                                                               \
    if ((threadIdx.x & 63) == 0) g_rc_prof[(blockIdx.x * 8 + (threadIdx.x >> 6)) * 16 + (slot)] = wall_clock64(); \
  } while (0)
#else
#define RCPROF(slot) \
  do {               \
  } while (0)
#endif

#ifndef RC_NOSTORE
#define RC_NOSTORE 0
#endif

typedef __bf16 bf16;
typedef __attribute__((address_space(3))) void* lds_ptr;

constexpr int NW = 8;
constexpr int NT = 64 * NW;
constexpr int TR = 16;

template <int D> struct Lay {
  static constexpr int J = D / 16;
  static constexpr int S = D / 32;
  static constexpr int CPR = D / 8;
  static constexpr int WBYTES = D * D * 2;
};

__device__ __forceinline__ int perm_row(int n) { return 32 * (n >> 5) + 8 * ((n >> 2) & 3) + 4 * ((n >> 4) & 1) + (n & 3); }
template <int D> __device__ __forceinline__ int swz(int n) { return (n / (128 / D)) & (Lay<D>::CPR - 1); }

template <int D, int NM>
__device__ __forceinline__ void stage_w(char* lds, const bf16* const (&W)[NM], const int64_t (&ldw)[NM], int wave,
                                        int lane) {
  constexpr int IPM = Lay<D>::WBYTES / 1024, CPR = Lay<D>::CPR;
  static_assert(NM * IPM % NW == 0, "staging split");
#pragma unroll
  for (int u = 0; u < NM * IPM / NW; ++u) {
    const int q = wave + NW * u, mtx = q / IPM, qi = q % IPM;
    const int idx = qi * 64 + lane, n = idx / CPR, pc = idx % CPR, lc = pc ^ swz<D>(n);
    const bf16* src = W[mtx] + (int64_t)perm_row(n) * ldw[mtx] + 8 * lc;
    __builtin_amdgcn_global_load_lds(src, (lds_ptr)(lds + mtx * Lay<D>::WBYTES + qi * 1024), 16, 0, 0);
  }
}
template <int D, int NV>
__device__ __forceinline__ void stage_v(float* lv, const float* const (&V)[NV], int tid) {
  for (int i = tid; i < NV * D; i += NT) lv[i] = V[i / D][i % D];
}

template <int D> struct Act { f32x4 v[Lay<D>::J]; };
template <int D> struct Raw { bf16x8 v[Lay<D>::S]; };

template <int D>
__device__ __forceinline__ void load_raw(Raw<D>& a, const bf16* base, int64_t ld, int64_t m, int g) {
  const bf16* p = base + m * ld + 8 * g;
#pragma unroll
  for (int s = 0; s < Lay<D>::S; ++s) a.v[s] = *reinterpret_cast<const bf16x8*>(p + 32 * s);
}
template <int D>
__device__ __forceinline__ void to_act(Act<D>& a, const Raw<D>& r) {
#pragma unroll
  for (int j = 0; j < Lay<D>::J; ++j)
#pragma unroll
    for (int e = 0; e < 4; ++e) a.v[j][e] = (float)r.v[j >> 1][4 * (j & 1) + e];
}
template <int D>
__device__ __forceinline__ void round_act(Act<D>& a, Raw<D>& r) {
#pragma unroll
  for (int j = 0; j < Lay<D>::J; ++j)
#pragma unroll
    for (int e = 0; e < 4; ++e) {
      r.v[j >> 1][4 * (j & 1) + e] = (bf16)a.v[j][e];
      a.v[j][e] = (float)r.v[j >> 1][4 * (j & 1) + e];
    }
}
template <int D>
__device__ __forceinline__ void store_raw(bf16* base, int64_t ld, int64_t m, bool ok, const Raw<D>& r, int g) {
  if (!ok) return;
  bf16* p = base + m * ld + 8 * g;
#pragma unroll
  for (int s = 0; s < Lay<D>::S; ++s) *reinterpret_cast<bf16x8*>(p + 32 * s) = r.v[s];
}
template <int D>
__device__ __forceinline__ void mm(const bf16* wl, const Raw<D>& b, Act<D>& acc, int lane) {
  constexpr int J = Lay<D>::J, S = Lay<D>::S;
  const int g = lane >> 4, cl = lane & 15;
  auto frag = [&](int j, int s) {
    const int n = 16 * j + cl;
    return *reinterpret_cast<const bf16x8*>(wl + n * D + 8 * ((4 * s + g) ^ swz<D>(n)));
  };
  bf16x8 f[2][S];
#pragma unroll
  for (int s = 0; s < S; ++s) f[0][s] = frag(0, s);
#pragma unroll
  for (int j = 0; j < J; ++j) {
    if (j + 1 < J) {
#pragma unroll
      for (int s = 0; s < S; ++s) f[(j + 1) & 1][s] = frag(j + 1, s);
    }
#pragma unroll
    for (int s = 0; s < S; ++s)
      acc.v[j] = __builtin_amdgcn_mfma_f32_16x16x32_bf16(f[j & 1][s], b.v[s], acc.v[j], 0, 0, 0);
    __builtin_amdgcn_sched_barrier(0);
  }
}
template <int D>
__device__ __forceinline__ void zero(Act<D>& a) {
#pragma unroll
  for (int j = 0; j < Lay<D>::J; ++j) a.v[j] = (f32x4){0.f, 0.f, 0.f, 0.f};
}
template <int D>
__device__ __forceinline__ f32x4 vec4(const float* lv, int j, int g) {
  return *reinterpret_cast<const f32x4*>(lv + 32 * (j >> 1) + 8 * g + 4 * (j & 1));
}
__device__ __forceinline__ int feat(int j, int g, int r) { return 32 * (j >> 1) + 8 * g + 4 * (j & 1) + r; }
__device__ __forceinline__ float row_sum(float s) { return add_xor32(add_xor16(s)); }

template <int D>
__device__ __forceinline__ void ln_fwd(Act<D>& x, const float* gw, const float* gb, float eps, int g, float& mu,
                                       float& rs) {
  float s = 0.f;
#pragma unroll
  for (int j = 0; j < Lay<D>::J; ++j)
#pragma unroll
    for (int e = 0; e < 4; ++e) s += x.v[j][e];
  mu = row_sum(s) / (float)D;
  float q = 0.f;
#pragma unroll
  for (int j = 0; j < Lay<D>::J; ++j)
#pragma unroll
    for (int e = 0; e < 4; ++e) {
      const float u = x.v[j][e] - mu;
      q += u * u;
    }
  rs = 1.0f / sqrtf(row_sum(q) / (float)D + eps);
#pragma unroll
  for (int j = 0; j < Lay<D>::J; ++j) {
    const f32x4 w = vec4<D>(gw, j, g), b = vec4<D>(gb, j, g);
#pragma unroll
    for (int e = 0; e < 4; ++e) x.v[j][e] = (x.v[j][e] - mu) * rs * w[e] + b[e];
  }
}

template <int D>
__device__ __forceinline__ void ln_fwd_head(Act<D>& x, const float* gw, const float* gb, float eps, int g, float& mu,
                                            float& rs) {
  float s = 0.f;
#pragma unroll
  for (int j = 0; j < Lay<D>::J; ++j)
#pragma unroll
    for (int e = 0; e < 4; ++e) s += x.v[j][e];
  mu = row_sum(s) / (float)D;
  float q = 0.f, u0 = 0.f;
#pragma unroll
  for (int j = 0; j < Lay<D>::J; ++j)
#pragma unroll
    for (int e = 0; e < 4; ++e) {
      const float u = x.v[j][e] - mu;
      if (j == 0 && e == 0) {
        u0 = u;
      } else if (j == 0 && e == 1) {
        float sq = u * u;
        asm volatile("" : "+v"(sq));
        q = __builtin_fmaf(u0, u0, sq);
      } else if ((j & 1) == 0 && e < 2) {
        q = __builtin_fmaf(u, u, q);
      } else {
        float sq = u * u;
        asm volatile("" : "+v"(sq));
        q += sq;
      }
    }
  rs = 1.0f / sqrtf(row_sum(q) / (float)D + eps);
#pragma unroll
  for (int j = 0; j < Lay<D>::J; ++j) {
    const f32x4 w = vec4<D>(gw, j, g), b = vec4<D>(gb, j, g);
#pragma unroll
    for (int e = 0; e < 4; ++e) x.v[j][e] = (x.v[j][e] - mu) * rs * w[e] + b[e];
  }
}

__device__ __forceinline__ float row16_sum(float v) { return row16_sum_up(v); }

template <int D, bool HEAD_FORM = false>
__device__ __forceinline__ void ln_bwd(Act<D>& dy, const Raw<D>& xr, bool valid, const float* gw, float mu, float a,
                                       float* red, int lane, int wave) {
  const int g = lane >> 4, cl = lane & 15;
  float* rw = red + wave * 2 * D;
  float sg = 0.f, sgu = 0.f;
#pragma unroll
  for (int j = 0; j < Lay<D>::J; ++j) {
    const f32x4 w = vec4<D>(gw, j, g);
#pragma unroll
    for (int e = 0; e < 4; ++e) {
      const float gy = valid ? dy.v[j][e] : 0.f;
      const float u = (float)xr.v[j >> 1][4 * (j & 1) + e] - mu;
      const float gq = gy * w[e];
      const float pg = row16_sum(gy * (u * a)), pb = row16_sum(gy);
      if (cl == 0) {
        rw[feat(j, g, e)] += pg;
        rw[D + feat(j, g, e)] += pb;
      }
      if constexpr (HEAD_FORM) {
        sg = __builtin_fmaf(gy, w[e], sg);
        sgu = __builtin_fmaf(u, gq, sgu);
      } else {
        sg += gq;
        sgu += gq * u;
      }
      dy.v[j][e] = gq;
    }
  }
  sg = row_sum(sg);
  sgu = row_sum(sgu);
  const float mg = sg / (float)D, coef = a * a * a * sgu / (float)D;
#pragma unroll
  for (int j = 0; j < Lay<D>::J; ++j) asm volatile("" : "+v"(dy.v[j]));
#pragma unroll
  for (int j = 0; j < Lay<D>::J; ++j)
#pragma unroll
    for (int e = 0; e < 4; ++e) {
      const float u = (float)xr.v[j >> 1][4 * (j & 1) + e] - mu;
      if constexpr (HEAD_FORM) {
        float p1 = a * (dy.v[j][e] - mg), p2 = coef * u;
        if ((j & 1) == 0 && e < 2) {
          asm volatile("" : "+v"(p1), "+v"(p2));
          dy.v[j][e] = p1 - p2;
        } else {
          asm volatile("" : "+v"(p2));
          dy.v[j][e] = __builtin_fmaf(a, dy.v[j][e] - mg, -p2);
        }
      } else {
        dy.v[j][e] = a * (dy.v[j][e] - mg) - coef * u;
      }
    }
}

__device__ __forceinline__ void ln_zero(float* red, int D, int lane, int wave) {
  for (int i = lane; i < 2 * D; i += 64) red[wave * 2 * D + i] = 0.f;
}
template <int D>
__device__ __forceinline__ void ln_partials(const float* red, float* part, int tid) {
  __syncthreads();
  if (tid < 2 * D) {
    const int which = tid / D, c = tid % D;
    float s = 0.f;
#pragma unroll
    for (int w = 0; w < NW; ++w) s += red[(w * 2 + which) * D + c];
    part[((int64_t)blockIdx.x * 2 + which) * D + c] = s;
  }
}

__device__ __forceinline__ int64_t n_tiles(int64_t M) { return (M + TR - 1) / TR; }

struct TileRange {
  int64_t first, step, end;
};
__device__ __forceinline__ TileRange tiles_of_wave(int64_t nt, int wave) {
  const int64_t G = gridDim.x, w = blockIdx.x;
  if (G >= 8 && G % 8 == 0) {
    const int64_t x = w & 7, Gx = G >> 3;
    return TileRange{x * nt / 8 + (w >> 3) + Gx * wave, Gx * NW, (x + 1) * nt / 8};
  }
  return TileRange{w + G * wave, G * NW, nt};
}

template <int D, int NM, int NV, int NR> struct Smem {
  static constexpr size_t W = (size_t)NM * Lay<D>::WBYTES;
  static constexpr size_t V = W + (size_t)NV * D * 4;
  static constexpr size_t BYTES = V + (size_t)NR * NW * 2 * D * 4;
};
__device__ __forceinline__ const bf16* wslot(const char* smem, int i, int wbytes) {
  return reinterpret_cast<const bf16*>(smem + (size_t)i * wbytes);
}

struct Tile {
  int64_t m, mc;
  bool ok;
};
__device__ __forceinline__ Tile tile_of(int64_t t, int64_t M, int cl) {
  Tile x;
  x.m = t * TR + cl;
  x.ok = x.m < M;
  x.mc = x.ok ? x.m : M - 1;
  return x;
}
template <int D>
__device__ __forceinline__ void fwd_in_q(const Raw<D>& xr, const Tile& T, const bf16* wq, const float* lv, float eps,
                                         bf16* Q, float* mean, float* rstd, bf16* q, int lane) {
  const int g = lane >> 4;
  Act<D> y;
  to_act<D>(y, xr);
  float mu, rs;
  ln_fwd<D>(y, lv, lv + D, eps, g, mu, rs);
  Raw<D> Qr;
  round_act<D>(y, Qr);
  store_raw<D>(Q, D, T.m, T.ok, Qr, g);
  if (T.ok && g == 0) {
    mean[T.m] = mu;
    rstd[T.m] = rs;
  }
  Act<D> acc;
  zero<D>(acc);
  mm<D>(wq, Qr, acc, lane);
#pragma unroll
  for (int j = 0; j < Lay<D>::J; ++j) acc.v[j] += vec4<D>(lv + 2 * D, j, g);
  Raw<D> r;
  round_act<D>(acc, r);
  store_raw<D>(q, D, T.m, T.ok, r, g);
}
template <int D>
__device__ __forceinline__ void fwd_in_kv(const Raw<D>& xr, const Tile& T, const bf16* wk, const bf16* wv,
                                          const float* lv, bf16* kv, int lane) {
  const int g = lane >> 4;
#pragma unroll
  for (int h = 0; h < 2; ++h) {
    Act<D> acc;
    zero<D>(acc);
    mm<D>(h == 0 ? wk : wv, xr, acc, lane);
#pragma unroll
    for (int j = 0; j < Lay<D>::J; ++j) acc.v[j] += vec4<D>(lv + (3 + h) * D, j, g);
    Raw<D> r;
    round_act<D>(acc, r);
    store_raw<D>(kv + h * D, 2 * D, T.m, T.ok, r, g);
  }
}

struct OutFwd {
  bf16 *x1, *z, *h1, *xn;
  float *mean, *rstd;
  const int64_t* ids;
  float drop_p, eps;
  uint32_t s1, s2;
};
__device__ __forceinline__ void drop4(float p, uint32_t s32, int64_t m, int D, int j, int g, float (&dm)[4]) {
  const uint64_t idx = (uint64_t)(m * D + feat(j, g, 0));
  drop_mul2(p, s32, idx, dm[0], dm[1]);
  drop_mul2(p, s32, idx + 2, dm[2], dm[3]);
}
template <int D>
__device__ __forceinline__ void fwd_out_a_x(const Raw<D>& orr, const Raw<D>& Qr, const Tile& T, const bf16* wo,
                                            const bf16* w1, const float* lv, const OutFwd& o, Raw<D>& zr, Raw<D>& hr,
                                            int lane, Raw<D>& r, float& mu, float& rs) {
  const int g = lane >> 4;
  Act<D> acc;
  zero<D>(acc);
  mm<D>(wo, orr, acc, lane);
#pragma unroll
  for (int j = 0; j < Lay<D>::J; ++j) {
    const f32x4 bb = vec4<D>(lv, j, g);
#pragma unroll
    for (int e = 0; e < 4; ++e) acc.v[j][e] = acc.v[j][e] + bb[e] + (float)Qr.v[j >> 1][4 * (j & 1) + e];
  }
  round_act<D>(acc, r);
  if (!RC_NOSTORE) store_raw<D>(o.x1, D, T.m, T.ok, r, g);
  ln_fwd<D>(acc, lv + D, lv + 2 * D, o.eps, g, mu, rs);
  round_act<D>(acc, zr);
  if (!RC_NOSTORE) store_raw<D>(o.z, D, T.m, T.ok, zr, g);
  if (T.ok && g == 0) {
    o.mean[T.m] = mu;
    o.rstd[T.m] = rs;
  }
  zero<D>(acc);
  mm<D>(w1, zr, acc, lane);
  const bool drop = o.drop_p > 0.f;
#pragma unroll
  for (int j = 0; j < Lay<D>::J; ++j) {
    float dm[4] = {1.f, 1.f, 1.f, 1.f};
    if (drop) drop4(o.drop_p, o.s1, T.m, D, j, g, dm);
    const f32x4 bb = vec4<D>(lv + 3 * D, j, g);
#pragma unroll
    for (int e = 0; e < 4; ++e) acc.v[j][e] = fmaxf(acc.v[j][e] + bb[e], 0.f) * dm[e];
  }
  round_act<D>(acc, hr);
  if (!RC_NOSTORE) store_raw<D>(o.h1, D, T.m, T.ok, hr, g);
}
template <int D>
__device__ __forceinline__ void fwd_out_a(const Raw<D>& orr, const Raw<D>& Qr, const Tile& T, const bf16* wo,
                                          const bf16* w1, const float* lv, const OutFwd& o, Raw<D>& zr, Raw<D>& hr,
                                          int lane) {
  Raw<D> r;
  float mu, rs;
  fwd_out_a_x<D>(orr, Qr, T, wo, w1, lv, o, zr, hr, lane, r, mu, rs);
}
template <int D>
__device__ __forceinline__ void fwd_out_b(const Raw<D>& hr, const Raw<D>& zr, const Tile& T, const bf16* w2,
                                          const float* lv, const OutFwd& o, Raw<D>& xr, int lane, bool keep) {
  const int g = lane >> 4;
  Act<D> acc;
  zero<D>(acc);
  mm<D>(w2, hr, acc, lane);
  const bool drop = o.drop_p > 0.f;
#pragma unroll
  for (int j = 0; j < Lay<D>::J; ++j) {
    float dm[4] = {1.f, 1.f, 1.f, 1.f};
    if (drop) drop4(o.drop_p, o.s2, T.m, D, j, g, dm);
    const f32x4 bb = vec4<D>(lv + 4 * D, j, g);
#pragma unroll
    for (int e = 0; e < 4; ++e) {
      const float v = __builtin_fmaf(acc.v[j][e] + bb[e], dm[e], (float)zr.v[j >> 1][4 * (j & 1) + e]);
      acc.v[j][e] = keep ? v : 0.f;
    }
  }
  round_act<D>(acc, xr);
  store_raw<D>(o.xn, D, T.m, T.ok, xr, g);
}
template <int D>
__device__ __forceinline__ void fwd_out_b(const Raw<D>& hr, const Raw<D>& zr, const Tile& T, const bf16* w2,
                                          const float* lv, const OutFwd& o, Raw<D>& xr, int lane) {
  fwd_out_b<D>(hr, zr, T, w2, lv, o, xr, lane, T.ok && o.ids[T.mc] != 0);
}

template <int D>
__device__ __forceinline__ void bwd_in_a(const Raw<D>& kr, const Raw<D>& vr, const bf16* wk, const bf16* wv,
                                         Raw<D>& dxkv, int lane) {
  Act<D> acc;
  zero<D>(acc);
  mm<D>(wk, kr, acc, lane);
  mm<D>(wv, vr, acc, lane);
  round_act<D>(acc, dxkv);
}
template <int D>
__device__ __forceinline__ void bwd_in_b(const Raw<D>& qr, const Raw<D>& rr, const Raw<D>& xr, const Raw<D>& dxkv,
                                         const Tile& T, float mu, float rs, const bf16* wq, const float* lnw,
                                         float* red, Raw<D>& dxr, int lane, int wave) {
  const int g = lane >> 4;
  Act<D> dQ;
  Raw<D> r;
  to_act<D>(dQ, rr);
  mm<D>(wq, qr, dQ, lane);
  round_act<D>(dQ, r);
  ln_bwd<D>(dQ, xr, T.ok, lnw, mu, rs, red, lane, wave);
#pragma unroll
  for (int j = 0; j < Lay<D>::J; ++j)
#pragma unroll
    for (int e = 0; e < 4; ++e) dQ.v[j][e] += (float)dxkv.v[j >> 1][4 * (j & 1) + e];
  round_act<D>(dQ, dxr);
}

struct OutBwd {
  bf16 *dy2, *da1, *dx1, *dout;
  float* delta;
  const int64_t* ids;
  float drop_p;
  uint32_t s1, s2;
};
template <int D>
__device__ __forceinline__ void bwd_out_a(const Raw<D>& dr, const Raw<D>& hr, const Tile& T, const bf16* w2,
                                          const OutBwd& o, Raw<D>& dzr, Raw<D>& dar, int lane, bool keep) {
  const int g = lane >> 4;
  const bool drop = o.drop_p > 0.f;
  Act<D> acc;
  Raw<D> r;
#pragma unroll
  for (int j = 0; j < Lay<D>::J; ++j) {
    float dm[4] = {1.f, 1.f, 1.f, 1.f};
    if (drop) drop4(o.drop_p, o.s2, T.m, D, j, g, dm);
#pragma unroll
    for (int e = 0; e < 4; ++e) {
      const bf16 v = keep ? dr.v[j >> 1][4 * (j & 1) + e] : (bf16)0.f;
      dzr.v[j >> 1][4 * (j & 1) + e] = v;
      acc.v[j][e] = (float)v * dm[e];
    }
  }
  round_act<D>(acc, r);
  store_raw<D>(o.dy2, D, T.m, T.ok, r, g);
  zero<D>(acc);
  mm<D>(w2, r, acc, lane);
#pragma unroll
  for (int j = 0; j < Lay<D>::J; ++j) {
    float dm[4] = {1.f, 1.f, 1.f, 1.f};
    if (drop) drop4(o.drop_p, o.s1, T.m, D, j, g, dm);
#pragma unroll
    for (int e = 0; e < 4; ++e) acc.v[j][e] = ((float)hr.v[j >> 1][4 * (j & 1) + e] > 0.f ? acc.v[j][e] : 0.f) * dm[e];
  }
  round_act<D>(acc, dar);
  store_raw<D>(o.da1, D, T.m, T.ok, dar, g);
// ... 481 lines not shown
  }
  ln_zero(red, D, lane, wave);
  ln_zero(red2, D, lane, wave);
  __syncthreads();
  asm volatile("" : "+v"(id));
  Raw<D> dxkv, dxr, hr, x1r, orr, dzr, dar;
  float mu2 = 0.f, rs2 = 0.f;
  if (has) {
    bwd_in_a<D>(kr, vr, wimg(w0), wimg(w1), dxkv, lane);
    load_raw<D>(hr, b.h1, D, T.mc, g);
    load_raw<D>(x1r, b.x1, D, T.mc, g);
    if (b.delta) load_raw<D>(orr, b.o, D, T.mc, g);
    mu2 = b.mean2[T.mc];
    rs2 = b.rstd2[T.mc];
    bwd_in_b<D>(qr, rr, xr, dxkv, T, mu, rs, wimg(w2), lv, red, dxr, lane, wave);
  }
  if constexpr (R::ON) {
    __syncthreads();
    stage_slot<D>(w0, b.W1T, D, wave, lane);
    stage_slot<D>(w1, b.WoT, D, wave, lane);
  }
  asm volatile("" ::: "memory");
  if (has) {
    as_loaded<D>(dxr);
    bwd_out_a<D>(dxr, hr, T, wimg(w3), ob, dzr, dar, lane, T.ok && id != 0);
  }
  if constexpr (R::ON) __syncthreads();
  asm volatile("" ::: "memory");
  if (has)
    bwd_out_b<D>(dar, x1r, dzr, orr, T, mu2, rs2, wimg(R::ON ? w0 : w4), wimg(R::ON ? w1 : w5), lv + D, ob, red2,
                 lane, wave);
  ln_partials<D>(red, a.part, tid);
  ln_partials<D>(red2, b.part, tid);
}

struct TurnArgs {
  rs_sas_out_args a;
  rs_sas_out_bwd_args b;
};
typedef const __attribute__((address_space(4))) TurnArgs* TurnArgsPtr;
__device__ __forceinline__ TurnArgsPtr turn_args_late() {
  TurnArgsPtr kp = (TurnArgsPtr)__builtin_amdgcn_kernarg_segment_ptr();
  asm volatile("" : "+s"(kp));
  return kp;
}
template <int D>
__global__ __launch_bounds__(NT) void block_out_head_bwd_kernel(TurnArgs k) {
  const rs_sas_out_args& a = k.a;
  typedef Roll<D> R;
  RC_BOUNDARY_SLOTS(D);
  __shared__ __attribute__((aligned(16))) float lv[7 * D];
  __shared__ __attribute__((aligned(16))) float red[NW * 2 * D], red2[NW * 2 * D];
  __shared__ float hred[4][NW];
  const int tid = threadIdx.x, lane = tid & 63, wave = __builtin_amdgcn_readfirstlane(tid >> 6), g = lane >> 4,
            cl = lane & 15;
  RCPROF(0);
  const TileRange tr = tiles_of_wave(n_tiles(a.M), wave);
  const bool has = tr.first < tr.end;
  const Tile T = tile_of(has ? tr.first : 0, a.M, cl);
  const OutFwd of = out_fwd_of(a);
  Raw<D> orr, Qr;
  int64_t id = 0, ip = 0, in = 0;
  if (has) {
    load_raw<D>(orr, a.o, D, T.mc, g);
    load_raw<D>(Qr, a.Q, D, T.mc, g);
    id = a.ids[T.mc];
    ip = a.h.pos[T.mc];
    in = a.h.neg[T.mc];
  }
  stage_slot<D>(w0, a.Wo, D, wave, lane);
  stage_slot<D>(w1, a.W1, D, wave, lane);
  stage_slot<D>(w2, a.W2, D, wave, lane);
  stage_slot<D>(w3, k.b.W2T, D, wave, lane);
  if constexpr (!R::ON) {
    stage_slot<D>(w4, k.b.W1T, D, wave, lane);
    stage_slot<D>(w5, k.b.WoT, D, wave, lane);
  }
  {
    const float* const V[7] = {a.bo, a.ln_w, a.ln_b, a.b1, a.b2, a.h.ln_w, a.h.ln_b};
    stage_v<D, 7>(lv, V, tid);
  }
  ln_zero(red, D, lane, wave);
  ln_zero(red2, D, lane, wave);
  float hacc[3] = {0.f, 0.f, 0.f};
  {
    int c = 0;
    for (int i = tid; i < a.h.ncount; i += NT) c += a.h.count_parts[i];
    c = (int)wave_sum((float)c);
    if (lane == 0) hred[3][wave] = (float)c;
  }
  __syncthreads();
  float hscale;
  {
    float c = 0.f;
#pragma unroll
    for (int w = 0; w < NW; ++w) c += hred[3][w];
    hscale = 1.f / (a.h.divisor ? *a.h.divisor : c);
  }
  asm volatile("" : "+v"(id), "+v"(ip), "+v"(in));
  RCPROF(1);
  Raw<D> zr, hr, x1r, xr, er, nr, dr, dzr, dar;
  float mu2 = 0.f, rs2 = 0.f;
  if (has) {
    fwd_out_a_x<D>(orr, Qr, T, wimg(w0), wimg(w1), lv, of, zr, hr, lane, x1r, mu2, rs2);
    load_raw<D>(er, a.h.E, D, ip, g);
    load_raw<D>(nr, a.h.E, D, in, g);
  }
  RCPROF(2);
  if constexpr (R::ON) {
    __syncthreads();
    const TurnArgsPtr kp = turn_args_late();
    stage_slot<D>(w0, kp->b.W1T, D, wave, lane);
    stage_slot<D>(w1, kp->b.WoT, D, wave, lane);
  }
  asm volatile("" ::: "memory");
  const TurnArgsPtr kb = turn_args_late();
  const OutBwd ob = {kb->b.dy2, kb->b.da1, kb->b.dx1, kb->b.dout, kb->b.delta, a.ids, a.drop_p, of.s1, of.s2};
  if (has) {
    const bool keep = T.ok && id != 0;
    fwd_out_b<D>(hr, zr, T, wimg(w2), lv, of, xr, lane, keep);
    RCPROF(4);
    head_tile_x<D, false>(xr, er, nr, ip, T, lv + 5 * D, lv + 6 * D, a.h, hscale, red, hacc, lane, wave, dr);
    RCPROF(6);
    asm volatile("" ::: "memory");
    as_loaded<D>(dr);
    as_loaded<D>(hr);
    bwd_out_a<D>(dr, hr, T, wimg(w3), ob, dzr, dar, lane, keep);
  }
  if constexpr (R::ON) __syncthreads();
  asm volatile("" ::: "memory");
  if (has) {
    as_loaded<D>(x1r);
    as_loaded<D>(orr);
    asm volatile("" : "+v"(mu2), "+v"(rs2));
    bwd_out_b<D>(dar, x1r, dzr, orr, T, mu2, rs2, wimg(R::ON ? w0 : w4), wimg(R::ON ? w1 : w5), lv + D, ob, red2, lane,
                 wave);
  }
  RCPROF(5);
#pragma unroll
  for (int k = 0; k < 3; ++k) {
    const float v = wave_sum(hacc[k]);
    if (lane == 0) hred[k][wave] = v;
  }
  ln_partials<D>(red, a.h.lnpart, tid);
  ln_partials<D>(red2, kb->b.part, tid);
  if (tid < 3) {
    float v = 0.f;
#pragma unroll
    for (int w = 0; w < NW; ++w) v += hred[tid][w];
    a.h.part[blockIdx.x * 3 + tid] = v;
  }
}

static int g_ncu = 0;
static int64_t grid_for(int64_t M) {
  if (g_ncu == 0) {
    int dev = 0, n = 0;
    if (hipGetDevice(&dev) == hipSuccess && hipDeviceGetAttribute(&n, hipDeviceAttributeMultiprocessorCount, dev) ==
                                                 hipSuccess && n > 0)
      g_ncu = n;
    else
      g_ncu = 256;
  }
  const int64_t nt = (M + TR - 1) / TR;
  return nt < g_ncu ? nt : g_ncu;
}
static bool width_ok(int64_t d) { return d == 64 || d == 128; }
static bool boundary_fused(int64_t M, int64_t d) {
  return M > 0 && width_ok(d) && (M + TR - 1) / TR <= grid_for(M) * NW;
}

template <typename K, typename... A>
static int launch(K kern, size_t lds, int64_t M, void* stream, const A&... a) {
  const void* fn = reinterpret_cast<const void*>(kern);
  if (lds) (void)hipFuncSetAttribute(fn, hipFuncAttributeMaxDynamicSharedMemorySize, (int)lds);
  hipLaunchKernelGGL(kern, dim3((unsigned)grid_for(M)), dim3(NT), lds, (hipStream_t)stream, a...);
  return (int)hipGetLastError();
}
template <int D>
static int launch_out_t(const rs_sas_out_args& a, void* s) {
  return a.h.E ? launch(block_out_kernel<D, true>, Smem<D, 3, 7, 1>::BYTES, a.M, s, a)
               : launch(block_out_kernel<D, false>, Smem<D, 3, 5, 0>::BYTES, a.M, s, a);
}
static int launch_out(const rs_sas_out_args& a, int64_t d, void* s) {
  return d == 64 ? launch_out_t<64>(a, s) : launch_out_t<128>(a, s);
}
static int launch_in(const rs_sas_in_args& a, int64_t d, void* s) {
  return d == 64 ? launch(block_in_kernel<64>, Smem<64, 3, 5, 0>::BYTES, a.M, s, a)
                 : launch(block_in_kernel<128>, Smem<128, 3, 5, 0>::BYTES, a.M, s, a);
}
static int launch_out_bwd(const rs_sas_out_bwd_args& a, int64_t d, void* s) {
  return d == 64 ? launch(block_out_bwd_kernel<64>, Smem<64, 3, 1, 1>::BYTES, a.M, s, a)
                 : launch(block_out_bwd_kernel<128>, Smem<128, 3, 1, 1>::BYTES, a.M, s, a);
}
static int launch_in_bwd(const rs_sas_in_bwd_args& a, int64_t d, void* s) {
  return d == 64 ? launch(block_in_bwd_kernel<64>, Smem<64, 3, 1, 1>::BYTES, a.M, s, a)
                 : launch(block_in_bwd_kernel<128>, Smem<128, 3, 1, 1>::BYTES, a.M, s, a);
}
static int launch_out_in(const rs_sas_out_args& a, const rs_sas_in_args& b, int64_t d, void* s) {
  return d == 64 ? launch(block_out_in_kernel<64>, 0, a.M, s, a, b) : launch(block_out_in_kernel<128>, 0, a.M, s, a, b);
}
static int launch_in_out_bwd(const rs_sas_in_bwd_args& a, const rs_sas_out_bwd_args& b, int64_t d, void* s) {
  return d == 64 ? launch(block_in_out_bwd_kernel<64>, 0, a.M, s, a, b)
                 : launch(block_in_out_bwd_kernel<128>, 0, a.M, s, a, b);
}
static int launch_out_head_bwd(const rs_sas_out_args& a, const rs_sas_out_bwd_args& b, int64_t d, void* s) {
  const TurnArgs k = {a, b};
  return d == 64 ? launch(block_out_head_bwd_kernel<64>, 0, a.M, s, k)
                 : launch(block_out_head_bwd_kernel<128>, 0, a.M, s, k);
}

__global__ __launch_bounds__(256) void transpose_bf16_kernel(const int64_t* __restrict__ desc, const __bf16* src,
                                                             __bf16* dst) {
  __shared__ __bf16 t[64][66];
  const int64_t* dsc = desc + 6 * blockIdx.y;
  const int64_t rows = dsc[0], cols = dsc[1];
  const int64_t tc = cdiv(cols, 64);
  const int64_t tr = blockIdx.x / tc, tcc = blockIdx.x % tc;
  if (tr * 64 >= rows) return;
  const __bf16* sp = src + dsc[2];
  __bf16* dp = dst + dsc[4];
  const int64_t lds = dsc[3], ldd = dsc[5];
  for (int e = threadIdx.x; e < 64 * 64; e += 256) {
    const int r = e / 64, c = e % 64;
    const int64_t gr = tr * 64 + r, gc = tcc * 64 + c;
    t[r][c] = (gr < rows && gc < cols) ? sp[gr * lds + gc] : (__bf16)0.f;
  }
  __syncthreads();
  for (int e = threadIdx.x; e < 64 * 64; e += 256) {
    const int c = e / 64, r = e % 64;
    const int64_t gr = tr * 64 + r, gc = tcc * 64 + c;
    if (gr < rows && gc < cols) dp[gc * ldd + gr] = t[r][c];
  }
}

static bool aligned16(const void* a, const void* b, const void* c) {
  return (((uintptr_t)a | (uintptr_t)b | (uintptr_t)c) & 15) == 0;
}
static bool in_ok(const rs_sas_in_args* a, bool x_given) {
  if (!a || a->M <= 0) return false;
  const rs_sas_embed_args& e = a->e;
  if (!e.item_emb) return !x_given || a->ldx % 8 == 0;
  return e.T > 0 && a->M % e.T == 0 && e.ids && e.pos_emb && e.x0 && !e.count_ids == !e.count_parts &&
         aligned16(e.item_emb, e.pos_emb, e.x0);
}
static bool out_ok(const rs_sas_out_args* a, bool dx_needed) {
  if (!a || a->M <= 0) return false;
  const rs_sas_head_args& h = a->h;
  if (!h.E) return true;
  return h.pos && h.neg && h.count_parts && h.ncount > 0 && h.f && h.lnpart && h.part && (h.dx || !dx_needed);
}
static bool out_bwd_ok(const rs_sas_out_bwd_args* a) { return a && a->M > 0 && !a->o == !a->delta; }
static bool in_bwd_ok(const rs_sas_in_bwd_args* a) { return a && a->M > 0; }

}

extern "C" {

int64_t rs_sas_block_grid(int64_t M) { return M > 0 ? rc::grid_for(M) : 0; }

int rs_sas_block_boundary_fused(int64_t M, int64_t d) { return rc::boundary_fused(M, d) ? 1 : 0; }

int rs_sas_block_in(int64_t d, const rs_sas_in_args* in, void* stream) {
  if (!rc::in_ok(in, true)) return RS_ERR_ARG;
  if (!rc::width_ok(d)) return in->e.item_emb ? RS_ERR_ARG : RS_ERR_UNSUPPORTED;
  rs_sas_in_args a = *in;
  if (a.e.item_emb) {
    a.x = a.e.x0;
    a.ldx = d;
  }
  return rc::launch_in(a, d, stream);
}

int rs_sas_block_out(int64_t d, const rs_sas_out_args* out, void* stream) {
  if (!rc::out_ok(out, true)) return RS_ERR_ARG;
  if (!rc::width_ok(d)) return RS_ERR_UNSUPPORTED;
  rs_sas_out_args a = *out;
  if (a.h.E) a.h.eps = a.eps;
  return rc::launch_out(a, d, stream);
}

int rs_sas_block_out_bwd_delta(int64_t d, const rs_sas_out_bwd_args* out_bwd, void* stream) {
  if (!rc::out_bwd_ok(out_bwd)) return RS_ERR_ARG;
  if (!rc::width_ok(d)) return RS_ERR_UNSUPPORTED;
  return rc::launch_out_bwd(*out_bwd, d, stream);
}

int rs_sas_block_out_bwd(int64_t M, int64_t d, const void* dxn, const int64_t* ids, const void* h1, const void* x1,
                         const float* mean2, const float* rstd2, const float* ln_w, const void* W2T, const void* W1T,
                         const void* WoT, void* dy2, void* da1, void* dx1, void* dout, float* part, float drop_p,
                         uint64_t salt1, uint64_t salt2, const uint64_t* seed_base, void* stream) {
  rs_sas_out_bwd_args a = {};
  a.M = M, a.dxn = (const rs_bf16*)dxn, a.ids = ids, a.h1 = (const rs_bf16*)h1, a.x1 = (const rs_bf16*)x1;
  a.mean2 = mean2, a.rstd2 = rstd2, a.ln_w = ln_w;
  a.W2T = (const rs_bf16*)W2T, a.W1T = (const rs_bf16*)W1T, a.WoT = (const rs_bf16*)WoT;
  a.dy2 = (rs_bf16*)dy2, a.da1 = (rs_bf16*)da1, a.dx1 = (rs_bf16*)dx1, a.dout = (rs_bf16*)dout, a.part = part;
  a.drop_p = drop_p, a.salt1 = salt1, a.salt2 = salt2, a.seed_base = seed_base;
  return rs_sas_block_out_bwd_delta(d, &a, stream);
}

int rs_sas_block_in_bwd(int64_t d, const rs_sas_in_bwd_args* in_bwd, void* stream) {
  if (!rc::in_bwd_ok(in_bwd)) return RS_ERR_ARG;
  if (!rc::width_ok(d)) return RS_ERR_UNSUPPORTED;
  if (in_bwd->ldwt != 3 * d) return RS_ERR_ARG;
  return rc::launch_in_bwd(*in_bwd, d, stream);
}

int rs_sas_block_out_in(int64_t d, const rs_sas_out_args* out, const rs_sas_in_args* in, void* stream) {
  if (!rc::out_ok(out, true) || !rc::in_ok(in, false) || out->h.E || in->e.item_emb || out->M != in->M)
    return RS_ERR_ARG;
  if (!rc::width_ok(d)) return RS_ERR_UNSUPPORTED;
  const rs_sas_out_args a = *out;
  rs_sas_in_args b = *in;
  b.x = a.xn;
  b.ldx = d;
  if (rc::boundary_fused(a.M, d)) return rc::launch_out_in(a, b, d, stream);
  const int rc1 = rc::launch_out(a, d, stream);
  return rc1 ? rc1 : rc::launch_in(b, d, stream);
}

int rs_sas_block_in_out_bwd(int64_t d, const rs_sas_in_bwd_args* in_bwd, const rs_sas_out_bwd_args* out_bwd,
                            void* stream) {
  if (!rc::in_bwd_ok(in_bwd) || !rc::out_bwd_ok(out_bwd) || in_bwd->M != out_bwd->M) return RS_ERR_ARG;
  if (!rc::width_ok(d)) return RS_ERR_UNSUPPORTED;
  if (in_bwd->ldwt != 3 * d) return RS_ERR_ARG;
  rs_sas_in_bwd_args a = *in_bwd;
  rs_sas_out_bwd_args b = *out_bwd;
  if (rc::boundary_fused(a.M, d)) {
    a.dx = nullptr;
    b.dxn = nullptr;
    return rc::launch_in_out_bwd(a, b, d, stream);
  }
  if (!a.dx) return RS_ERR_ARG;
  b.dxn = a.dx;
  const int rc1 = rc::launch_in_bwd(a, d, stream);
  return rc1 ? rc1 : rc::launch_out_bwd(b, d, stream);
}

int rs_sas_block_out_head_bwd(int64_t d, const rs_sas_out_args* out, const rs_sas_out_bwd_args* out_bwd,
                              void* stream) {
  if (!rc::out_ok(out, false) || !out->h.E || !out_bwd || out->M != out_bwd->M) return RS_ERR_ARG;
  if (!rc::width_ok(d)) return RS_ERR_UNSUPPORTED;
  rs_sas_out_args a = *out;
  rs_sas_out_bwd_args b = *out_bwd;
  a.h.eps = a.eps;
  b.ids = a.ids, b.h1 = a.h1, b.x1 = a.x1, b.mean2 = a.mean, b.rstd2 = a.rstd, b.ln_w = a.ln_w;
  b.drop_p = a.drop_p, b.salt1 = a.salt1, b.salt2 = a.salt2, b.seed_base = a.seed_base;
  if (rc::boundary_fused(a.M, d)) {
    a.h.dx = nullptr;
    b.dxn = nullptr;
    b.o = a.o;
    return rc::launch_out_head_bwd(a, b, d, stream);
  }
  if (!a.h.dx) return RS_ERR_ARG;
  b.dxn = a.h.dx;
  b.o = b.delta ? a.o : nullptr;
  const int rc1 = rc::launch_out(a, d, stream);
  return rc1 ? rc1 : rc::launch_out_bwd(b, d, stream);
}

int rs_transpose_bf16(int64_t nmat, const int64_t* desc, int64_t max_tiles, const void* src, void* dst,
                      void* stream) {
  if (nmat <= 0 || max_tiles <= 0) return RS_ERR_ARG;
  hipLaunchKernelGGL(rc::transpose_bf16_kernel, dim3((unsigned)max_tiles, (unsigned)nmat), dim3(256), 0,
                     (hipStream_t)stream, desc, (const __bf16*)src, (__bf16*)dst);
  return (int)hipGetLastError();
}

}
```

recommender-baseline-model_amd/models/sas_model/sas.py:

```python
import math
import os

import torch
import torch.nn as nn

from ... import ops
from ...engine_util import (SideBranch, Workspace, as_ids, check_logq, compute_dtype, neg_dist_args, require_cuda,
                            site_salt)
from ...flat import FlatParams

LN_EPS = 1e-8
SAS_LOSSES = ("bce", "ce", "sampled_ce")
SCE_INDEX_ROWS = 32769


class PointWiseFeedForward(nn.Module):

    def __init__(self, hidden_units, dropout_rate):
        super().__init__()
        self.conv1 = nn.Conv1d(hidden_units, hidden_units, kernel_size=1)
        self.conv2 = nn.Conv1d(hidden_units, hidden_units, kernel_size=1)
        self.dropout_rate = dropout_rate


# ... 30 lines not shown
        for _ in range(self.num_blocks):
            self.attention_layernorms.append(nn.LayerNorm(d, eps=LN_EPS))
            self.attention_layers.append(nn.MultiheadAttention(d, self.heads, self.dropout_rate))
            self.forward_layernorms.append(nn.LayerNorm(d, eps=LN_EPS))
            self.forward_layers.append(PointWiseFeedForward(d, self.dropout_rate))

        self._flat = None
        self._engine = None
        if torch.device(self.device).type == "cuda":
            self.to(self.device)

    def _apply(self, fn, recurse=True):
        super()._apply(fn, recurse)
        p = next(self.parameters())
        self._flat = FlatParams(self, p.device) if p.device.type == "cuda" else None
        self._engine = None
        return self

    def engine(self):
        p = self.item_emb.weight
        require_cuda(p.device)
        if self._flat is None or not self._flat.is_bound(self):
            self._flat = FlatParams(self, p.device)
            self._engine = None
        if self._engine is None:
            self._engine = SASEngine(self, self._flat)
        return self._engine

    def forward(self, log_seqs, pos_seqs, neg_seqs):
        eng = self.engine()
        dev = self._flat.device
        ids, pos, neg = as_ids(log_seqs, dev), as_ids(pos_seqs, dev), as_ids(neg_seqs, dev)
        params = [p for _, p in self.named_parameters()]
        return _SASFunction.apply(eng, ids, pos, neg, self.training, *params)

    def ce_loss(self, log_seqs, pos_seqs):
        eng = self.engine()
        dev = self._flat.device
        ids, pos = as_ids(log_seqs, dev), as_ids(pos_seqs, dev)
        params = [p for _, p in self.named_parameters()]
        return _SASCEFunction.apply(eng, ids, pos, self.training, *params)

    def sampled_ce_loss(self, log_seqs, pos_seqs, cand, logq=None):
        eng = self.engine()
        dev = self._flat.device
        ids, pos, cand = as_ids(log_seqs, dev), as_ids(pos_seqs, dev), as_ids(cand, dev)
        params = [p for _, p in self.named_parameters()]
        return _SASSCEFunction.apply(eng, ids, pos, cand, logq, self.training, *params)

    def log2feats(self, log_seqs):
        eng = self.engine()
        ids = as_ids(log_seqs, self._flat.device)
        with torch.no_grad():
            return eng.features(ids).clone()

    @torch.no_grad()
    def predict(self, log_seqs, item_indices):
        eng = self.engine()
        dev = self._flat.device
        return eng.predict(as_ids(log_seqs, dev), as_ids(item_indices, dev))

    @torch.no_grad()
    def recommend(self, log_seqs, k, exclude_seen=True):
        eng = self.engine()
        return eng.topk(as_ids(log_seqs, self._flat.device), k, exclude_seen)

    @torch.no_grad()
    def full_rank(self, log_seqs, target, exclude_seen=True):
        eng = self.engine()
        dev = self._flat.device
        return eng.full_rank(as_ids(log_seqs, dev), as_ids(target, dev).reshape(-1), exclude_seen)


class _SASFunction(torch.autograd.Function):
    @staticmethod
    def forward(ctx, engine, ids, pos, neg, training, *params):
        engine.sync_compute_weights()
        pl, nl, saved = engine.forward(ids, pos, neg, training)
        ctx.engine = engine
        ctx.saved = saved
        return pl, nl

    @staticmethod
    def backward(ctx, dpl, dnl):
        eng = ctx.engine
        grad = torch.zeros(eng.flat.numel, dtype=torch.float32, device=eng.flat.device)
        eng.backward(ctx.saved, dpl.contiguous().float(), dnl.contiguous().float(), grad)
        ctx.saved = None
        grads = [eng.flat.view(n, grad) for n in eng.flat.names]
        return (None, None, None, None, None, *grads)


class _SASCEFunction(torch.autograd.Function):
    @staticmethod
    def forward(ctx, engine, ids, pos, training, *params):
        engine.sync_compute_weights()
        out = torch.zeros(4, dtype=torch.float32, device=engine.dev)
        ctx.saved = engine.ce_forward(ids, pos, training, out)
        ctx.engine = engine
        return out[2].clone()

    @staticmethod
    def backward(ctx, dloss):
        eng = ctx.engine
        grad = torch.zeros(eng.flat.numel, dtype=torch.float32, device=eng.flat.device)
        eng.ce_backward(ctx.saved, grad, dloss=dloss.contiguous().float().reshape(1))
        ctx.saved = None
        grads = [eng.flat.view(n, grad) for n in eng.flat.names]
        return (None, None, None, None, *grads)


class _SASSCEFunction(torch.autograd.Function):
    @staticmethod
    def forward(ctx, engine, ids, pos, cand, logq, training, *params):
        engine.sync_compute_weights()
        out = torch.zeros(4, dtype=torch.float32, device=engine.dev)
        ctx.saved = engine.sce_forward(ids, pos, cand, training, out, logq=logq)
        ctx.engine = engine
        return out[2].clone()

    @staticmethod
    def backward(ctx, dloss):
        eng = ctx.engine
        grad = torch.zeros(eng.flat.numel, dtype=torch.float32, device=eng.flat.device)
        eng.sce_backward(ctx.saved, grad, dloss=dloss.contiguous().float().reshape(1))
        ctx.saved = None
        grads = [eng.flat.view(n, grad) for n in eng.flat.names]
        return (None, None, None, None, None, None, *grads)


class SASEngine:

    def __init__(self, model: SAS, flat: FlatParams):
        self.m = model
        self.flat = flat
        self.d = model.hidden
        self.L = model.num_blocks
        self.H = model.heads
        self.Dh = self.d // self.H
        self.p = float(model.dropout_rate)
        self.dt = model.cdtype
        self.dev = flat.device
        if self.dt == torch.bfloat16:
            flat.enable_bf16()
        self.ws = Workspace(self.dev)
        self.side = SideBranch(self.dev)
        self._side_refreshed = False
        self.seed_base = torch.zeros(1, dtype=torch.int64, device=self.dev)
        self.external_seed = False
        self.adam_transposes = False
        self._wT = None
        self.boundary_fuse = os.environ.get("RS_SAS_BOUNDARY_FUSE", "1") != "0"
        self.turnaround_fuse = os.environ.get("RS_SAS_TURNAROUND_FUSE", "1") != "0"
        salt0 = int(torch.randint(0, 2 ** 62, (1,)).item())
        self.salt = {"emb": site_salt(salt0, 0)}
        for i in range(self.L):
            self.salt[f"attn{i}"] = site_salt(salt0, 1 + 4 * i)
            self.salt[f"ffn1_{i}"] = site_salt(salt0, 2 + 4 * i)
            self.salt[f"ffn2_{i}"] = site_salt(salt0, 3 + 4 * i)

    def sync_compute_weights(self):
        f = self.flat
        if f.bf16 is not None:
            if not f.stale:
                ops.cast_bf16(f.data, f.bf16)
            else:
                a = 0
                for lo, hi in sorted(f.stale) + [(f.numel, f.numel)]:
                    if lo > a:
                        ops.cast_bf16(f.data[a:lo], f.bf16[a:lo])
                    a = max(a, hi)
            if self._wT is not None:
                self._refresh_transposed()

    def transposed_spec(self):
        if not self.adam_transposes or self._wT is None:
            return None
        return self._wT_desc, self._wT_desc_host, self._wT

    def W(self, n):
        return self.flat.cview(n)

    def Wf(self, n):
        return self.flat.view(n)

    def _buf(self, name, shape, dtype=None):
        return torch.empty(shape, dtype=dtype or self.dt, device=self.dev)

    def forward(self, ids, pos, neg, training, need_logits=True, clone_seed=True, fuse_head=False,
                head_divisor=None, ce=False):
        B, T = ids.shape
        M, d, H, Dh, L = B * T, self.d, self.H, self.Dh, self.L
        p = self.p if training else 0.0
        if p > 0 and not self.external_seed:
            ops.seed_advance(self.seed_base)
        sb = self.seed_base.clone() if clone_seed else self.seed_base
        e = self._buf
        s = {"B": B, "T": T, "p": p, "ids": ids, "pos": pos, "neg": neg, "sb": sb,
             "x": [], "Q": [], "mu1": [], "r1": [], "q": [], "kv": [], "o": [], "lse": [],
             "x1": [], "z": [], "mu2": [], "r2": [], "h1": []}
        fused = ops.sas_block_fused_ok(d, self.dt)
        side = fused and training and pos is not None
        nsrc = 1 if ce else 3
        if side:
            fork = self.side.mark()
        x = e("x0", (M, d))
        fuse_head = fuse_head and side and need_logits
        cntp = None
        if fuse_head:
            cntp = self.ws.get("cntp", (ops.sas_block_in_count_parts(M),), torch.int32)
            s["cntp"] = cntp
        emb = None
        if fused:
            emb = (ids, T, self.W("item_emb.weight"), self.W("pos_emb.weight"), math.sqrt(d), p, self.salt["emb"], sb,
                   x, pos if cntp is not None else None, cntp)
        else:
            ops.embed_fwd(0, ids, T, self.W("item_emb.weight"), self.W("pos_emb.weight"), math.sqrt(d), p,
                          self.salt["emb"], sb, x)

        def after_first():
            if side:
                s["side"] = self._side_prologue(ids, pos, neg, after=fork, nsrc=nsrc)
        head = None
        if cntp is not None:
            Gb = ops.sas_block_grid(M)
            f32 = torch.float32
            s.update(head_in_block=True, hdiv=head_divisor, f=e("f", (M, d)), pl=e("pl", (B, T), f32),
                     nl=e("nl", (B, T), f32), dpl=e("dpl", (B, T), f32), dnl=e("dnl", (B, T), f32),
                     hdx=e("dx", (M, d)), lnh=self.ws.get("lnh_blk", (2 * d * Gb,), f32),
                     headp=e("headp", (3 * Gb,), f32))
            head = (self.W("item_emb.weight"), pos, neg, self.Wf("last_layernorm.weight"),
                    self.Wf("last_layernorm.bias"), cntp, head_divisor, s["f"], s["pl"], s["nl"], s["dpl"], s["dnl"],
                    s["hdx"], s["lnh"], s["headp"])
        if fused:
            x = self._forward_blocks_fused(s, x, emb=emb, after_first=after_first, head=head)
        else:
            for i in range(L):
                pre = f"attention_layers.{i}."
                Q, mu1, r1 = e("Q", (M, d)), e("mu", (M,), torch.float32), e("r", (M,), torch.float32)
                Win, bin_ = self.W(pre + "in_proj_weight"), self.Wf(pre + "in_proj_bias")
                q, kv = e("q", (M, d)), e("kv", (M, 2 * d))
                o, lse = e("o", (M, d)), e("lse", (B * H * T,), torch.float32)
                x1 = e("x1", (M, d))
                z, mu2, r2 = e("z", (M, d)), e("mu", (M,), torch.float32), e("r", (M,), torch.float32)
                fw = f"forward_layers.{i}."
                h1, xn = e("h1", (M, d)), e("x", (M, d))
                ops.layernorm_fwd(x, self.Wf(f"attention_layernorms.{i}.weight"),
                                  self.Wf(f"attention_layernorms.{i}.bias"), LN_EPS, Q, mu1, r1, 0)
                ops.linear_fwd(Q, Win[:d], q, bias=bin_[:d])
                ops.linear_fwd(x, Win[d:], kv, bias=bin_[d:])
                ops.attn_fwd(B, T, H, Dh, q, kv[:, :d], kv[:, d:], o, lse, 1.0 / math.sqrt(Dh), 0, ids, p,
                             self.salt[f"attn{i}"], sb)
                ops.linear_fwd(o, self.W(pre + "out_proj.weight"), x1, bias=self.Wf(pre + "out_proj.bias"), resid=Q)
                ops.layernorm_fwd(x1, self.Wf(f"forward_layernorms.{i}.weight"),
                                  self.Wf(f"forward_layernorms.{i}.bias"), LN_EPS, z, mu2, r2, 0)
                ops.linear_fwd(z, self.W(fw + "conv1.weight").view(d, d), h1, bias=self.Wf(fw + "conv1.bias"),
                               act=ops.ACT_RELU, drop_p=p, drop_seed=self.salt[f"ffn1_{i}"], seed_base=sb, drop_ld=d)
                ops.linear_fwd(h1, self.W(fw + "conv2.weight").view(d, d), xn, bias=self.Wf(fw + "conv2.bias"),
                               drop_p=p, drop_seed=self.salt[f"ffn2_{i}"], seed_base=sb, drop_ld=d, resid=z,
                               rowmask_ids=ids)
                for k_, v_ in (("x", x), ("Q", Q), ("mu1", mu1), ("r1", r1), ("q", q), ("kv", kv), ("o", o),
                               ("lse", lse), ("x1", x1), ("z", z), ("mu2", mu2), ("r2", r2), ("h1", h1)):
                    s[k_].append(v_)
                x = xn
        if "head_in_block" in s:
            s.update(xL=x)
            return s["pl"], s["nl"], s
        if ce:
            s.update(xL=x)
            return None, None, s
        f, muf, rf = e("f", (M, d)), e("mu", (M,), torch.float32), e("r", (M,), torch.float32)
        s.update(xL=x, f=f, muf=muf, rf=rf)
        if fused and need_logits:
            pl, nl = e("pl", (B, T), torch.float32), e("nl", (B, T), torch.float32)
            headp = e("headp", (3 * (-(-M // 64)),), torch.float32)
            ops.sas_head_fwd(x, self.Wf("last_layernorm.weight"), self.Wf("last_layernorm.bias"), LN_EPS, f, muf, rf,
                             self.W("item_emb.weight"), pos, neg, pl, nl, headp)
            s.update(pl=pl, nl=nl, headp=headp)
            return pl, nl, s
        ops.layernorm_fwd(x, self.Wf("last_layernorm.weight"), self.Wf("last_layernorm.bias"), LN_EPS, f, muf, rf, 0)
        if not need_logits:
            return None, None, s
        pl, nl = e("pl", (B, T), torch.float32), e("nl", (B, T), torch.float32)
        ops.sampled_logits_fwd(f, self.W("item_emb.weight"), pos, neg, pl, nl)
        return pl, nl, s

    def _forward_blocks_fused(self, s, x, emb=None, after_first=None, head=None):
        B, T, p, ids, sb = s["B"], s["T"], s["p"], s["ids"], s["sb"]
        M, d, H, Dh, L = B * T, self.d, self.H, self.Dh, self.L
        e = self._buf
        f32 = torch.float32
        lay = [dict(Q=e("Q", (M, d)), mu1=e("mu", (M,), f32), r1=e("r", (M,), f32), q=e("q", (M, d)),
                    kv=e("kv", (M, 2 * d)), o=e("o", (M, d)), lse=e("lse", (B * H * T,), f32), x1=e("x1", (M, d)),
                    z=e("z", (M, d)), mu2=e("mu", (M,), f32), r2=e("r", (M,), f32), h1=e("h1", (M, d)),
                    xn=e("x", (M, d))) for _ in range(L)]

        def in_args(i):
            pre = f"attention_layers.{i}."
            Win, bin_ = self.W(pre + "in_proj_weight"), self.Wf(pre + "in_proj_bias")
            b = lay[i]
            return (self.Wf(f"attention_layernorms.{i}.weight"), self.Wf(f"attention_layernorms.{i}.bias"),
                    b["Q"], b["mu1"], b["r1"], Win[:d], bin_[:d], b["q"], Win[d:], bin_[d:], b["kv"])

        def out_args(i):
            pre, fw, b = f"attention_layers.{i}.", f"forward_layers.{i}.", lay[i]
            return (b["o"], b["Q"], self.W(pre + "out_proj.weight"), self.Wf(pre + "out_proj.bias"), b["x1"],
                    self.Wf(f"forward_layernorms.{i}.weight"), self.Wf(f"forward_layernorms.{i}.bias"), LN_EPS,
                    b["z"], b["mu2"], b["r2"], self.W(fw + "conv1.weight"), self.Wf(fw + "conv1.bias"), b["h1"],
                    self.W(fw + "conv2.weight"), self.Wf(fw + "conv2.bias"), b["xn"], ids, p,
                    self.salt[f"ffn1_{i}"], self.salt[f"ffn2_{i}"], sb)

        ln_w, ln_b, Q, mu1, r1, Wq, bq, q, Wkv, bkv, kv = in_args(0)
        if emb is not None:
            ops.sas_block_in_embed(*emb, ln_w, ln_b, LN_EPS, Q, mu1, r1, Wq, bq, q, Wkv, bkv, kv)
        else:
            ops.sas_block_in(x, ln_w, ln_b, LN_EPS, Q, mu1, r1, Wq, bq, q, Wkv, bkv, kv)
        if after_first is not None:
            after_first()
        xs = [x]
        for i in range(L):
            b = lay[i]
            ops.attn_fwd(B, T, H, Dh, b["q"], b["kv"][:, :d], b["kv"][:, d:], b["o"], b["lse"], 1.0 / math.sqrt(Dh),
                         0, ids, p, self.salt[f"attn{i}"], sb)
            if i + 1 < L:
                ln_w, ln_b, Q, mu1, r1, Wq, bq, q, Wkv, bkv, kv = in_args(i + 1)
                if self.boundary_fuse:
                    ops.sas_block_out_in(out_args(i), ln_w, ln_b, LN_EPS, Q, mu1, r1, Wq, bq, q, Wkv, bkv, kv)
                else:
                    ops.sas_block_out(*out_args(i))
                    ops.sas_block_in(b["xn"], ln_w, ln_b, LN_EPS, Q, mu1, r1, Wq, bq, q, Wkv, bkv, kv)
            elif head is not None and self.turnaround_fuse:
                if self._side_refreshed:
                    self.side.join(s["side"][0])
                tb = self._out_bwd_bufs(s, i)
                ops.sas_block_out_head_bwd(out_args(i), head, *tb["args"])
                s["turnaround"] = tb
            elif head is not None:
                ops.sas_block_out_head(out_args(i), *head)
            else:
                ops.sas_block_out(*out_args(i))
            xs.append(b["xn"])
        for i in range(L):
            b = lay[i]
            for k_ in ("Q", "mu1", "r1", "q", "kv", "o", "lse", "x1", "z", "mu2", "r2", "h1"):
                s[k_].append(b[k_])
            s["x"].append(xs[i])
        return xs[L]

    @property
    def fused_head(self):
        return ops.sas_block_fused_ok(self.d, self.dt)

    def backward(self, s, dpl, dnl, grad, loss_out=None, divisor=None, split=None, aux_out=None):
        B, T, p, ids = s["B"], s["T"], s["p"], s["ids"]
        M, d, H, Dh, L = B * T, self.d, self.H, self.Dh, self.L
        sb = s["sb"]
        e = self._buf
        G = lambda n: self.flat.view(n, grad)
        slab = self.ws.get("slab", (ops.wgrad_slab_numel(M, 2 * d, d),), torch.float32)
        wln = self.ws.get("ln", (2 * 512 * d,), torch.float32)
        wat = self.ws.get("attn", (B * H * T,), torch.float32)

        fused = ops.sas_block_fused_ok(d, self.dt)
        if fused:
            ev, iws = s["side"] if "side" in s else self._side_prologue(ids, s["pos"], s["neg"])
        if fused:
            dx = e("dx", (M, d))
            lnh = self.ws.get("lnh", (2 * d * (-(-M // 64)),), torch.float32)
            E, gl = self.W("item_emb.weight"), self.Wf("last_layernorm.weight")
            stats = ()
            nb = -(-M // 64)
            assert dpl is None or "turnaround" not in s, "the forward already ran the backward of its own BCE gradient"
            if dpl is None and "head_in_block" in s:
                assert s["hdiv"] is divisor, "backward's divisor must be the one forward's head used"
                dx, dpl, dnl, lnh = s["hdx"], s["dpl"], s["dnl"], s["lnh"]
                nb = s["headp"].numel() // 3
                if loss_out is not None:
                    stats = (s["headp"], divisor, loss_out) + ((aux_out,) if aux_out is not None else ())
            elif dpl is None:
                dpl, dnl = e("dpl", (B, T), torch.float32), e("dnl", (B, T), torch.float32)
                ops.sas_head_bwd(s["headp"], divisor, loss_out, s["pl"], s["nl"], None, None, dpl, dnl, s["pos"],
                                 s["neg"], E, s["xL"], gl, s["muf"], s["rf"], dx, lnh)
            else:
                ops.sas_head_bwd(None, None, None, None, None, dpl, dnl, None, None, s["pos"], s["neg"], E, s["xL"],
                                 gl, s["muf"], s["rf"], dx, lnh)
            segs = ops.ln_partial_segments(lnh, M, d, G("last_layernorm.weight"), G("last_layernorm.bias"), nb=nb)
            if self._side_refreshed:
                self.side.join(ev)

            def item_grads(dx):
                ops.item_grad(iws, 3, M, dx, math.sqrt(d), p, self.salt["emb"], sb, s["f"], dpl, dnl,
                              G("item_emb.weight"), marks=getattr(self, "row_marks", None))
            dx = self._backward_blocks_fused(s, dx, grad, segs, tail=item_grads,
                                             pos=lambda dx: (ids, T, dx, p, self.salt["emb"], sb,
                                                             G("pos_emb.weight")) + stats)
            self.side.join()
            if split is not None:
                split("dense")
            return len(stats) > 3
        df = e("df", (M, d))
        by_index = self.dt == torch.float32 or d in (64, 128, 256)
        ops.sampled_logits_bwd(s["f"], self.W("item_emb.weight"), s["pos"], s["neg"], dpl, dnl, df,
                               None if by_index else G("item_emb.weight"))
        dx = e("dx", (M, d))
        ops.layernorm_bwd(s["xL"], df, self.Wf("last_layernorm.weight"), s["muf"], s["rf"], LN_EPS, dx,
                          G("last_layernorm.weight"), G("last_layernorm.bias"), wln, 0)
        self._backward_blocks_unfused(s, dx, grad, by_index, [ids, s["pos"], s["neg"]], s["f"], dpl, dnl)

    def _backward_blocks_unfused(self, s, dx, grad, by_index, keys, f, w1, w2):
        B, T, p, ids = s["B"], s["T"], s["p"], s["ids"]
        M, d, H, Dh, L = B * T, self.d, self.H, self.Dh, self.L
        sb = s["sb"]
        e = self._buf
        G = lambda n: self.flat.view(n, grad)
        slab = self.ws.get("slab", (ops.wgrad_slab_numel(M, 2 * d, d),), torch.float32)
        wln = self.ws.get("ln", (2 * 512 * d,), torch.float32)
        wat = self.ws.get("attn", (B * H * T,), torch.float32)
        for i in reversed(range(L)):
            pre = f"attention_layers.{i}."
            fw = f"forward_layers.{i}."
            dy2, dzres = e("dy2", (M, d)), e("dzres", (M, d))
            ops.dropout_rowmask(dx, p, self.salt[f"ffn2_{i}"], sb, ids, dy2, dzres)
            ops.linear_wgrad(dy2, s["h1"][i], G(fw + "conv2.weight").view(d, d), slab, db=G(fw + "conv2.bias"))
            da1 = e("da1", (M, d))
            ops.linear_dgrad(dy2, self.W(fw + "conv2.weight").view(d, d), da1, act=ops.ACT_RELU_BWD,
                             aux=s["h1"][i], drop_p=p, drop_seed=self.salt[f"ffn1_{i}"], seed_base=sb, drop_ld=d)
            ops.linear_wgrad(da1, s["z"][i], G(fw + "conv1.weight").view(d, d), slab, db=G(fw + "conv1.bias"))
            dz = e("dz", (M, d))
            ops.linear_dgrad(da1, self.W(fw + "conv1.weight").view(d, d), dz, resid=dzres)
            dx1 = e("dx1", (M, d))
            ops.layernorm_bwd(s["x1"][i], dz, self.Wf(f"forward_layernorms.{i}.weight"), s["mu2"][i], s["r2"][i],
                              LN_EPS, dx1, G(f"forward_layernorms.{i}.weight"), G(f"forward_layernorms.{i}.bias"),
                              wln, 0)
            ops.linear_wgrad(dx1, s["o"][i], G(pre + "out_proj.weight"), slab, db=G(pre + "out_proj.bias"))
            do = e("do", (M, d))
            ops.linear_dgrad(dx1, self.W(pre + "out_proj.weight"), do)
            dq, dkv = e("dq", (M, d)), e("dkv", (M, 2 * d))
            kv = s["kv"][i]
            ops.attn_bwd(B, T, H, Dh, s["q"][i], kv[:, :d], kv[:, d:], s["o"][i], do, s["lse"][i], dq,
                         dkv[:, :d], dkv[:, d:], 1.0 / math.sqrt(Dh), 0, ids, p, self.salt[f"attn{i}"], sb, wat)
            Gin, Gb = G(pre + "in_proj_weight"), G(pre + "in_proj_bias")
            Win = self.W(pre + "in_proj_weight")
            ops.linear_wgrad(dq, s["Q"][i], Gin[:d], slab, db=Gb[:d])
            ops.linear_wgrad(dkv, s["x"][i], Gin[d:], slab, db=Gb[d:])
            dQ = e("dQ", (M, d))
            ops.linear_dgrad(dq, Win[:d], dQ, resid=dx1)
            dxi = e("dxi", (M, d))
            ops.linear_dgrad(dkv, Win[d:], dxi)
            ops.layernorm_bwd(s["x"][i], dQ, self.Wf(f"attention_layernorms.{i}.weight"), s["mu1"][i], s["r1"][i],
                              LN_EPS, dxi, G(f"attention_layernorms.{i}.weight"),
                              G(f"attention_layernorms.{i}.bias"), wln, 0, accumulate=True)
            dx = dxi
        ops.embed_bwd(0, ids, T, dx, math.sqrt(d), p, self.salt["emb"], sb, None if by_index else G("item_emb.weight"),
                      G("pos_emb.weight"))
        if by_index:
            V1 = self.flat.shapes["item_emb.weight"][0]
            n = len(keys)
            iws = self.ws.get("itemidx", (ops.item_index_ws_bytes(n, M, V1, d),), torch.uint8)
            ops.item_index_build(keys, V1, d, iws)
            ops.item_grad(iws, n, M, dx, math.sqrt(d), p, self.salt["emb"], sb, f, w1, w2,
                          G("item_emb.weight"), marks=getattr(self, "row_marks", None) if n == 3 else None)

    @property
    def ce_rows_fused(self):
        return ops.sas_ce_rows_ok(self.d, self.dt) and os.environ.get("RS_SAS_CE_ROWS", "1") != "0"

    def _valid_rows_forward(self, s, pos, max_labelled):
        d, dt = self.d, self.dt
        M = s["B"] * s["T"]
        f32 = torch.float32
        g = self.ws.get
        dense = dt == torch.float32 and d % 4 != 0
        cap = M if dense else int(max_labelled or M)
        V1 = self.flat.shapes["item_emb.weight"][0]
        V1p = -(-V1 // 64) * 64
        x, labels = s["xL"], pos.reshape(-1)
# ... 315 lines not shown
```

recommender-baseline-model_amd/ops.py:

```python
import ctypes as C
import os

import torch

from . import _lib
from ._lib import BF16, F32, Epilogue, call, ptr, stream

ACT_NONE, ACT_RELU, ACT_GELU, ACT_RELU_BWD, ACT_GELU_BWD = (
    _lib.ACT_NONE, _lib.ACT_RELU, _lib.ACT_GELU, _lib.ACT_RELU_BWD, _lib.ACT_GELU_BWD)


STAMP_KINDS = {1: "attn_bwd", 2: "wgrad_grouped", 3: "vocab_ce_fwd"}


def kernel_stamps(buf, step, kinds=()):
    mask = sum(1 << k for k, n in STAMP_KINDS.items() if n in kinds)
    call("rs_kernel_stamps", ptr(buf), ptr(step), mask)


def read_kernel_stamps(buf, khz):
    import numpy as np
    h = buf.cpu().numpy().view(np.uint64)
    steps, marks, W = int(h[1]), int(h[2]), int(h[3])
    rec = h[4:4 + steps * marks * (1 + W)].reshape(steps, marks, 1 + W)
# ... 370 lines not shown
         stream())


def cast_bf16(src, dst):
    call("rs_cast_bf16", src.numel(), ptr(src), ptr(dst), stream())


def dropout_rowmask(x, drop_p, seed, seed_base, rowmask_ids, out, out_masked=None):
    M, N = x.shape
    call("rs_dropout_rowmask", dtype_code(x), ptr(x), M, N, ld(x), drop_p, seed, ptr(seed_base), N,
         ptr(rowmask_ids), ptr(out), ptr(out_masked), stream())


def dropout2(x, drop_p, salt1, salt2, seed_base, out1, out2):
    M, N = x.shape
    call("rs_dropout2", dtype_code(x), ptr(x), M, N, ld(x), drop_p, salt1, salt2, ptr(seed_base), N, ptr(out1),
         ptr(out2), stream())


def vocab_ce_ws_numel(R, V1):
    n = _lib.lib().rs_vocab_ce_ws_numel(R, V1)
    if n < 0:
        raise RuntimeError("rs_vocab_ce_ws_numel: bad arguments")
    return n


def vocab_ce_fwd(h, E, bias, labels, ws, out, rows_dev=None, count_override=None):
    R, d = h.shape
    V1 = E.shape[0]
    call("rs_vocab_ce_fwd", R, V1, d, ptr(h), ld(h), ptr(E), ld(E), ptr(bias), ptr(labels), ptr(rows_dev),
         ptr(count_override), ptr(ws), ptr(out), stream())


def vocab_head_supported(d):
    return bool(_lib.lib().rs_vocab_head_supported(d))


def vocab_head_fwd(h, E, bias, labels, ws, out, rows_dev=None, count_override=None):
    R, d = h.shape
    V1 = E.shape[0]
    ev = _ev_begin("vocab_ce_fwd")
    call("rs_vocab_head_fwd", R, V1, d, ptr(h), ld(h), ptr(E), ld(E), ptr(bias), ptr(labels), ptr(rows_dev),
         ptr(count_override), ptr(ws), ptr(out), stream())
    _ev_end(ev)


def vocab_head_bwd(h, E, bias, labels, ws, count, dl, rows_dev=None, dloss=None, voff=0):
    R, d = h.shape
    V1 = E.shape[0]
    call("rs_vocab_head_bwd", R, V1, d, ptr(h), ld(h), ptr(E), ld(E), ptr(bias), ptr(labels), ptr(rows_dev),
         ptr(count), ptr(dloss), ptr(ws), ptr(dl), ld(dl), int(voff), stream())


def vocab_shard_lse(h, E, bias, labels, ws, lse):
    R, d = h.shape
    call("rs_vocab_shard_lse", R, E.shape[0], d, ptr(h), ld(h), ptr(E), ld(E), ptr(bias), ptr(labels), ptr(ws),
         ptr(lse), stream())


def vocab_shard_label_logits(h, E, bias, labels, v0, v1, tgt):
    R, d = h.shape
    call("rs_vocab_shard_label_logits", R, d, ptr(h), ld(h), ptr(E), ld(E), ptr(bias), ptr(labels), int(v0), int(v1),
         ptr(tgt), stream())


def vocab_shard_combine(lse_parts, tgt, labels, lse, out):
    N, R = lse_parts.shape
    call("rs_vocab_shard_combine", N, R, ptr(lse_parts), ptr(tgt), ptr(labels), ptr(lse), ptr(out), stream())


def vocab_ce_bwd(h, E, bias, labels, ws, count, dl, rows_dev=None, dloss=None):
    R, d = h.shape
    V1 = E.shape[0]
    call("rs_vocab_ce_bwd", R, V1, d, ptr(h), ld(h), ptr(E), ld(E), ptr(bias), ptr(labels), ptr(rows_dev),
         ptr(count), ptr(dloss), ptr(ws), ptr(dl), ld(dl), stream())


def graph_upload(graph):
    call("rs_graph_upload", C.c_void_p(int(graph.raw_cuda_graph_exec())), stream())


def seed_advance(seed_base):
    call("rs_seed_advance", ptr(seed_base), stream())


def sas_block_fused_ok(d, dtype):
    return dtype == torch.bfloat16 and d in (64, 128)


def sas_block_grid(M):
    return int(_lib.lib().rs_sas_block_grid(M))


sas_block_parts = sas_block_in_count_parts = sas_block_grid


def sas_block_boundary_fused(M, d):
    return bool(_lib.lib().rs_sas_block_boundary_fused(M, d))


def _sas_args(cls, **fields):
    return cls(**{k: ptr(v) if isinstance(v, torch.Tensor) else v for k, v in fields.items() if v is not None})


def _sas_in(x, ln_w, ln_b, eps, Q, mean, rstd, Wq, bq, q, Wkv, bkv, kv, embed=None):
    return _sas_args(_lib.SasInArgs, M=x.shape[0], x=x, ldx=ld(x), ln_w=ln_w, ln_b=ln_b, eps=eps, Q=Q, mean=mean,
                     rstd=rstd, Wq=Wq, bq=bq, q=q, Wkv=Wkv, bkv=bkv, kv=kv, e=embed)


def _sas_out(o, Q, Wo, bo, x1, ln_w, ln_b, eps, z, mean, rstd, W1, b1, h1, W2, b2, xn, ids, drop_p, salt1, salt2,
             seed_base, head=None):
    return _sas_args(_lib.SasOutArgs, M=o.shape[0], o=o, Q=Q, Wo=Wo, bo=bo, x1=x1, ln_w=ln_w, ln_b=ln_b, eps=eps,
                     z=z, mean=mean, rstd=rstd, W1=W1, b1=b1, h1=h1, W2=W2, b2=b2, xn=xn, ids=ids, drop_p=drop_p,
                     salt1=salt1, salt2=salt2, seed_base=seed_base, h=head)


def _sas_head(M, d, E, pos, neg, ln_w, ln_b, count_parts, divisor, f, pl, nl, dpl, dnl, dx, lnpart, part):
    G = sas_block_grid(M)
    assert part.numel() == 3 * G and lnpart.numel() >= 2 * d * G and count_parts.dtype == torch.int32
    return _sas_args(_lib.SasHeadArgs, E=E, pos=pos, neg=neg, ln_w=ln_w, ln_b=ln_b, count_parts=count_parts,
                     ncount=count_parts.numel(), divisor=divisor, f=f, pl=pl, nl=nl, dpl=dpl, dnl=dnl, dx=dx,
                     lnpart=lnpart, part=part)


def _sas_out_bwd(M, dxn, ids, h1, x1, mean2, rstd2, ln_w, W2T, W1T, WoT, dy2, da1, dx1, dout, part, drop_p, salt1,
                 salt2, seed_base, o=None, delta=None):
    return _sas_args(_lib.SasOutBwdArgs, M=M, dxn=dxn, ids=ids, h1=h1, x1=x1, mean2=mean2, rstd2=rstd2, ln_w=ln_w,
                     W2T=W2T, W1T=W1T, WoT=WoT, dy2=dy2, da1=da1, dx1=dx1, dout=dout, part=part, drop_p=drop_p,
                     salt1=salt1, salt2=salt2, seed_base=seed_base, o=o, delta=delta)


def _sas_in_bwd(dq, dkv, dx1, x, mean1, rstd1, ln_w, WinT, dx, part):
    return _sas_args(_lib.SasInBwdArgs, M=dq.shape[0], dq=dq, dkv=dkv, dx1=dx1, x=x, mean1=mean1, rstd1=rstd1,
                     ln_w=ln_w, WinT=WinT, ldwt=ld(WinT), dx=dx, part=part)


def sas_block_in(x, ln_w, ln_b, eps, Q, mean, rstd, Wq, bq, q, Wkv, bkv, kv):
    a = _sas_in(x, ln_w, ln_b, eps, Q, mean, rstd, Wq, bq, q, Wkv, bkv, kv)
    call("rs_sas_block_in", x.shape[1], C.byref(a), stream())


def sas_block_in_embed(ids, T, item_emb, pos_emb, scale, drop_p, salt, seed_base, x0, count_ids, count_parts,
                       ln_w, ln_b, eps, Q, mean, rstd, Wq, bq, q, Wkv, bkv, kv):
    M, d = x0.shape
    assert ids.numel() == M and item_emb.dtype == torch.bfloat16 and x0.dtype == torch.bfloat16
    if count_parts is not None:
        assert count_parts.dtype == torch.int32 and count_parts.numel() >= sas_block_grid(M)
    e = _sas_args(_lib.SasEmbedArgs, ids=ids, item_emb=item_emb, pos_emb=pos_emb, T=T, scale=scale, drop_p=drop_p,
                  salt=salt, seed_base=seed_base, x0=x0, count_ids=count_ids, count_parts=count_parts)
    a = _sas_in(x0, ln_w, ln_b, eps, Q, mean, rstd, Wq, bq, q, Wkv, bkv, kv, embed=e)
    call("rs_sas_block_in", d, C.byref(a), stream())


def sas_block_out_head(out_args, E, pos, neg, lnl_w, lnl_b, count_parts, divisor, f, pl, nl, dpl, dnl, dx, lnpart,
                       part):
    M, d = out_args[0].shape
    h = _sas_head(M, d, E, pos, neg, lnl_w, lnl_b, count_parts, divisor, f, pl, nl, dpl, dnl, dx, lnpart, part)
    a = _sas_out(*out_args, head=h)
    call("rs_sas_block_out", d, C.byref(a), stream())


def sas_block_out(o, Q, Wo, bo, x1, ln_w, ln_b, eps, z, mean, rstd, W1, b1, h1, W2, b2, xn, ids, drop_p,
                  salt1, salt2, seed_base):
    a = _sas_out(o, Q, Wo, bo, x1, ln_w, ln_b, eps, z, mean, rstd, W1, b1, h1, W2, b2, xn, ids, drop_p, salt1, salt2,
                 seed_base)
    call("rs_sas_block_out", o.shape[1], C.byref(a), stream())


def sas_block_out_bwd(dxn, ids, h1, x1, mean2, rstd2, ln_w, W2T, W1T, WoT, dy2, da1, dx1, dout, part, drop_p, salt1,
                      salt2, seed_base, o=None, delta=None):
    M, d = dxn.shape
    a = _sas_out_bwd(M, dxn, ids, h1, x1, mean2, rstd2, ln_w, W2T, W1T, WoT, dy2, da1, dx1, dout, part, drop_p, salt1,
                     salt2, seed_base, o, delta)
    call("rs_sas_block_out_bwd_delta", d, C.byref(a), stream())


def sas_block_in_bwd(dq, dkv, dx1, x, mean1, rstd1, ln_w, WinT, dx, part):
    a = _sas_in_bwd(dq, dkv, dx1, x, mean1, rstd1, ln_w, WinT, dx, part)
    call("rs_sas_block_in_bwd", dq.shape[1], C.byref(a), stream())


def sas_block_out_in(out_args, ln1_w, ln1_b, eps1, Qn, mean1, rstd1, Wq, bq, q, Wkv, bkv, kv):
    a = _sas_out(*out_args)
    b = _sas_args(_lib.SasInArgs, M=a.M, ln_w=ln1_w, ln_b=ln1_b, eps=eps1, Q=Qn, mean=mean1, rstd=rstd1, Wq=Wq,
                  bq=bq, q=q, Wkv=Wkv, bkv=bkv, kv=kv)
    call("rs_sas_block_out_in", out_args[0].shape[1], C.byref(a), C.byref(b), stream())


def sas_block_in_out_bwd(in_args, dx, part1, out_args):
    M, d = in_args[0].shape
    a = _sas_in_bwd(*in_args, dx, part1)
    b = _sas_out_bwd(M, None, *out_args)
    call("rs_sas_block_in_out_bwd", d, C.byref(a), C.byref(b), stream())


def sas_block_out_head_bwd(out_args, head_args, W2T, W1T, WoT, dy2, da1, dx1, dout, part2, delta=None):
    M, d = out_args[0].shape
    assert part2.numel() >= 2 * d * sas_block_grid(M)
    a = _sas_out(*out_args, head=_sas_head(M, d, *head_args))
    b = _sas_args(_lib.SasOutBwdArgs, M=M, W2T=W2T, W1T=W1T, WoT=WoT, dy2=dy2, da1=da1, dx1=dx1, dout=dout,
                  part=part2, delta=delta)
    call("rs_sas_block_out_head_bwd", d, C.byref(a), C.byref(b), stream())


def touched_rows_ws_numel(rows):
    return int(_lib.lib().rs_touched_rows_ws_numel(rows))


def touched_rows(ids, rows, flags, index, count, ws):
    call("rs_touched_rows", ptr(ids), ids.numel(), rows, ptr(flags), ptr(index), ptr(count), ptr(ws), stream())


def rows_pack(src, index, count, compact):
    rows, d = src.shape
    call("rs_rows_pack", ptr(src), rows, d, ptr(index), ptr(count), ptr(compact), compact.shape[0], stream())


def rows_unpack(dst, index, compact):
    rows, d = dst.shape
    call("rs_rows_unpack", ptr(dst), rows, d, ptr(index), ptr(compact), stream())


def unique_rows_ws_bytes(table_rows):
    n = int(_lib.lib().rs_unique_rows_ws_bytes(int(table_rows)))
    if n < 0:
        raise ValueError("rs_unique_rows_ws_bytes: table_rows must be positive")
    return n


def _i32(t, name, numel=None):
    if not isinstance(t, torch.Tensor) or t.dtype != torch.int32 or not t.is_contiguous():
        raise ValueError(f"{name} must be a contiguous int32 tensor")
    if numel is not None and t.numel() != numel:
        raise ValueError(f"{name} must hold {numel} element(s), got {t.numel()}")


def unique_rows(keys, table_rows, rows, count, ws):
    keys = list(keys)
    if not 1 <= len(keys) <= 3:
        raise ValueError(f"unique_rows takes one to three key tensors, got {len(keys)}")
    for k in keys:
        if not isinstance(k, torch.Tensor) or k.dtype != torch.int64 or not k.is_contiguous():
            raise ValueError("unique_rows: every key tensor must be contiguous int64")
    table_rows = int(table_rows)
    if not 0 < table_rows < 2 ** 31:
        raise ValueError(f"unique_rows: table_rows must be in [1, 2^31), got {table_rows}")
    _i32(rows, "rows")
    _i32(count, "count", 1)
    total = sum(k.numel() for k in keys)
    if rows.numel() < max(total, 1):
        raise ValueError(f"unique_rows: rows holds {rows.numel()} ids but the keys number {total}")
    if ws.dtype != torch.uint8 or ws.numel() < unique_rows_ws_bytes(table_rows):
        raise ValueError(f"unique_rows: ws must be uint8 with at least {unique_rows_ws_bytes(table_rows)} bytes")
    kp = [(ptr(k) if k.numel() else None, k.numel()) for k in keys] + [(None, 0)] * (3 - len(keys))
    call("rs_unique_rows", kp[0][0], kp[0][1], kp[1][0], kp[1][1], kp[2][0], kp[2][1], table_rows, ptr(rows),
         ptr(count), rows.numel(), ptr(ws), ws.numel(), stream())


def adam_rows(rows, count, p, g, m, v, p_bf16, state, hyper, zero_grad=False, max_wg=None):
    _i32(rows, "rows")
    _i32(count, "count", 1)
    if p.dim() not in (1, 2):
        raise ValueError("adam_rows: the table must be [R, d] or [R]")
    R, d = p.shape[0], (p.shape[1] if p.dim() == 2 else 1)
    for name, t in (("p", p), ("g", g), ("m", m), ("v", v)):
        if t.dtype != torch.float32 or t.shape != p.shape or not t.is_contiguous():
            raise ValueError(f"adam_rows: {name} must be contiguous fp32 of the table's shape {tuple(p.shape)}")
    if p_bf16 is not None and (p_bf16.dtype != torch.bfloat16 or p_bf16.shape != p.shape or not p_bf16.is_contiguous()):
        raise ValueError("adam_rows: p_bf16 must be a contiguous bf16 tensor of the table's shape")
    if R < 1 or d < 1 or rows.numel() < 1:
        raise ValueError("adam_rows: empty table or list")
    if rows.numel() * d >= 2 ** 31:
        raise ValueError("adam_rows: list capacity * row width must stay below 2^31")
    if max_wg is not None and int(max_wg) < 1:
        raise ValueError("adam_rows: max_wg must be positive")
    if state.dtype != torch.float64 or state.numel() < 4 or hyper.dtype != torch.float64 or hyper.numel() < 5:
        raise ValueError("adam_rows: state / hyper must be the optimizer's float64 device arrays")
    call("rs_adam_rows", d, R, ptr(rows), ptr(count), rows.numel(), ptr(p), ptr(g), ptr(m), ptr(v), ptr(p_bf16),
         ptr(state), ptr(hyper), int(zero_grad), int(max_wg or 8192), stream())


def ln_partial_segments(part, M, d, dgamma, dbeta, nb=None):
    nb = sas_block_grid(M) if nb is None else nb
    return [(part, 2 * d, nb, d, dgamma), (part[d:], 2 * d, nb, d, dbeta)]


def _segments(segs):
    arr = (_lib.ReduceSegment * max(1, len(segs)))()
    for i, (src, stride, splits, n, out) in enumerate(segs):
        arr[i] = _lib.ReduceSegment(ptr(src), stride, splits, n, ptr(out))
    return arr


def wgrad_grouped(problems, M, rows_per_split, slab, extra=(), pos=None, max_tile=256):
    ev = _ev_begin("wgrad_grouped")
    _wgrad_grouped(problems, M, rows_per_split, slab, extra, pos, max_tile)
    _ev_end(ev)


def _wgrad_grouped(problems, M, rows_per_split, slab, extra=(), pos=None, max_tile=256):
    arr = (_lib.WgradProblem * len(problems))()
    for i, (dY, X, dW, db) in enumerate(problems):
        N, K = dY.shape[1], X.shape[1]
        assert dW.numel() == N * K and dY.shape[0] >= M and X.shape[0] >= M
        arr[i] = _lib.WgradProblem(ptr(dY), ld(dY), ptr(X), ld(X), N, K, ptr(dW), ptr(db) if db is not None else None)
    segs = _segments(list(extra))
# ... 327 lines not shown
```

Before: 499,800 sequences/s.

## Fuse first block embedding, input projections and causal attention into one kernel

Adds a new kernel that, per sequence split, embeds the tokens, applies LayerNorm and the Q/KV projections into LDS, and then runs the first layer's causal attention in the same workgroup. This replaces the separate block-in and attention-forward launches for layer 0. It removes the K/V round trip through global memory and one launch. The attention tile code is factored into a shared device function, and a dual-operand matmul helper shares weight fragments across two row tiles. The fused path is on by default when heads equal 1 and the split count is at least 2. It risks higher LDS and register pressure, and redundant K/V computation across the splits of a sequence.

```diff
diff --git a/include/recsys_hip.h b/include/recsys_hip.h
--- a/include/recsys_hip.h
+++ b/include/recsys_hip.h
@@ -329,6 +329,19 @@
 int rs_sas_block_out_head_bwd(int64_t d, const rs_sas_out_args* out, const rs_sas_out_bwd_args* out_bwd,
                               void* stream);
 
+typedef struct rs_sas_in_attn_args {
+  rs_sas_in_args in;
+  int64_t B;
+  rs_bf16* o;
+  float* lse;
+  float scale;
+  float drop_p;
+  uint64_t salt;
+  int64_t ncount;
+} rs_sas_in_attn_args;
+int rs_sas_block_in_attn_nsplit(int64_t d, int64_t B, int64_t T);
+int rs_sas_block_in_attn(int64_t d, const rs_sas_in_attn_args* args, void* stream);
+
 int64_t rs_touched_rows_ws_numel(int64_t rows);
 int rs_touched_rows(const int64_t* ids, int64_t n, int64_t rows, int32_t* flags, int32_t* index, int32_t* count,
                     int32_t* ws, void* stream);
@@ -483,7 +496,8 @@
   RS_SIZEOF_SAS_HEAD_ARGS = 5,
   RS_SIZEOF_SAS_OUT_ARGS = 6,
   RS_SIZEOF_SAS_OUT_BWD_ARGS = 7,
-  RS_SIZEOF_SAS_IN_BWD_ARGS = 8
+  RS_SIZEOF_SAS_IN_BWD_ARGS = 8,
+  RS_SIZEOF_SAS_IN_ATTN_ARGS = 9
 };
 int64_t rs_abi_sizeof(int which);
 
diff --git a/recommender-baseline-model_amd/_lib.py b/recommender-baseline-model_amd/_lib.py
--- a/recommender-baseline-model_amd/_lib.py
+++ b/recommender-baseline-model_amd/_lib.py
@@ -67,9 +67,15 @@
                 ("ln_w", vp), ("WinT", vp), ("ldwt", i64), ("dx", vp), ("part", vp)]
 
 
+class SasInAttnArgs(C.Structure):
+    _fields_ = [("in", SasInArgs), ("B", i64), ("o", vp), ("lse", vp), ("scale", f32), ("drop_p", f32), ("salt", u64),
+                ("ncount", i64)]
+
+
 STRUCTS = {"rs_epilogue": Epilogue, "rs_wgrad_problem": WgradProblem, "rs_reduce_segment": ReduceSegment,
            "rs_sas_embed_args": SasEmbedArgs, "rs_sas_in_args": SasInArgs, "rs_sas_head_args": SasHeadArgs,
-           "rs_sas_out_args": SasOutArgs, "rs_sas_out_bwd_args": SasOutBwdArgs, "rs_sas_in_bwd_args": SasInBwdArgs}
+           "rs_sas_out_args": SasOutArgs, "rs_sas_out_bwd_args": SasOutBwdArgs, "rs_sas_in_bwd_args": SasInBwdArgs,
+           "rs_sas_in_attn_args": SasInAttnArgs}
 
 ACT_NONE, ACT_RELU, ACT_GELU, ACT_RELU_BWD, ACT_GELU_BWD = 0, 1, 2, 3, 4
 
@@ -142,6 +148,8 @@
     "rs_sas_block_out_bwd": [i64, i64, vp, vp, vp, vp, vp, vp, vp, vp, vp, vp, vp, vp, vp, vp, vp, f32, u64, u64,
                              vp, vp],
     "rs_sas_block_in_bwd": [i64, C.POINTER(SasInBwdArgs), vp],
+    "rs_sas_block_in_attn": [i64, C.POINTER(SasInAttnArgs), vp],
+    "rs_sas_block_in_attn_nsplit": [i64, i64, i64],
     "rs_sas_block_out_in": [i64, C.POINTER(SasOutArgs), C.POINTER(SasInArgs), vp],
     "rs_sas_block_in_out_bwd": [i64, C.POINTER(SasInBwdArgs), C.POINTER(SasOutBwdArgs), vp],
     "rs_sas_block_out_head_bwd": [i64, C.POINTER(SasOutArgs), C.POINTER(SasOutBwdArgs), vp],
diff --git a/recommender-baseline-model_amd/build.py b/recommender-baseline-model_amd/build.py
--- a/recommender-baseline-model_amd/build.py
+++ b/recommender-baseline-model_amd/build.py
@@ -1,6 +1,7 @@
 import concurrent.futures as cf
 import glob
 import os
+import re
 import subprocess
 import sys
 
@@ -11,7 +12,7 @@
 LIB = os.path.join(PKG, "librecsys_hip.so")
 HIPCC = os.environ.get("HIPCC", "/opt/rocm/bin/hipcc")
 ARCH = os.environ.get("RS_OFFLOAD_ARCH", "gfx950")
-LINK_LAST = ("sas_ce.hip", "sas_sce.hip", "adam_rows.hip", "sgd.hip")
+LINK_LAST = ("sas_ce.hip", "sas_sce.hip", "adam_rows.hip", "sgd.hip", "block_in_attn.hip")
 FLAGS = ["-O3", "-std=c++17", "-fPIC", f"--offload-arch={ARCH}", "-munsafe-fp-atomics",
          "-I", os.path.join(ROOT, "include"), "-I", CSRC]
 
@@ -31,10 +32,17 @@
     return max((os.path.getmtime(p) for p in inc), default=0.0)
 
 
+def _hip_includes_mtime(src):
+    with open(src) as fh:
+        inc = re.findall(r'^#include "(\w+\.hip)"', fh.read(), flags=re.M)
+    return max((os.path.getmtime(os.path.join(CSRC, i)) for i in inc), default=0.0)
+
+
 def _compile(src, force):
     obj = os.path.join(OBJ, os.path.basename(src) + ".o")
     if not force and os.path.exists(obj):
-        if os.path.getmtime(obj) >= max(os.path.getmtime(src), _headers_mtime(), _included_mtime()):
+        if os.path.getmtime(obj) >= max(os.path.getmtime(src), _headers_mtime(), _included_mtime(),
+                                       _hip_includes_mtime(src)):
             return obj, False
     cmd = [HIPCC, *FLAGS, "-c", src, "-o", obj]
     r = subprocess.run(cmd, capture_output=True, text=True)
diff --git a/recommender-baseline-model_amd/csrc/attention_lds.hip b/recommender-baseline-model_amd/csrc/attention_lds.hip
--- a/recommender-baseline-model_amd/csrc/attention_lds.hip
+++ b/recommender-baseline-model_amd/csrc/attention_lds.hip
@@ -243,6 +243,103 @@
 }
 
 template <int DH>
+__device__ __forceinline__ void attn_fwd_tile(const AttnLdsArgs& a, const bf16* Ks, const bf16* Vs, const float* km,
+                                              const bf16x8 (&qf)[DH / 32], int qt, int64_t bh, int64_t b, int64_t h,
+                                              int T, int nq, uint64_t seed, int lane) {
+  constexpr int LD = Img<DH>::LD, KC = DH / 32, DT = DH / 16, NKT = 16;
+  const int g = lane >> 4, cl = lane & 15;
+  const int q0 = qt * 16;
+  const int64_t qrow = q0 + cl;
+  const int nkt = a.mask_kind == 0 ? qt + 1 : nq;
+  const float sl2 = a.scale * LOG2E;
+  const int qi = q0 + cl;
+  f32x4 s[NKT];
+  float mx = NEG_INF;
+#pragma unroll
+  for (int kt = 0; kt < NKT; ++kt) {
+    s[kt] = (f32x4){0.f, 0.f, 0.f, 0.f};
+    if (kt < nkt) {
+#pragma unroll
+      for (int kc = 0; kc < KC; ++kc) s[kt] = mfma16(row_frag(Ks, LD, kt * 16 + cl, kc * 32 + 8 * g), qf[kc], s[kt]);
+      const bool need = a.mask_kind != 0 || kt == qt || kt * 16 + 16 > T;
+      const int kb = kt * 16 + 4 * g;
+      if (need) {
+        const f32x4 kmv = *reinterpret_cast<const f32x4*>(km + kb);
+#pragma unroll
+        for (int r = 0; r < 4; ++r) {
+          const int k = kb + r;
+          const bool dead = (k >= T) | ((a.mask_kind == 0) & (k > qi));
+          const float x = s[kt][r] * sl2;
+          s[kt][r] = dead ? NEG_INF : (kmv[r] != 0.f ? MASK2 : x);
+          mx = fmaxf(mx, s[kt][r]);
+        }
+      } else {
+#pragma unroll
+        for (int r = 0; r < 4; ++r) {
+          s[kt][r] *= sl2;
+          mx = fmaxf(mx, s[kt][r]);
+        }
+      }
+    }
+  }
+  mx = max_xor32(max_xor16(mx));
+  float sm = 0.f;
+#pragma unroll
+  for (int kt = 0; kt < NKT; ++kt) {
+    if (kt < nkt) {
+#pragma unroll
+      for (int r = 0; r < 4; ++r) {
+        const float e = ex2(s[kt][r] - mx);
+        s[kt][r] = e;
+        sm += e;
+      }
+    }
+  }
+  sm = add_xor32(add_xor16(sm));
+  const float inv = 1.f / sm;
+  if (g == 0 && qrow < a.T) a.lse[bh * a.T + qrow] = (mx + __builtin_amdgcn_logf(sm)) * LN2;
+  const uint32_t s32 = seed32(seed);
+  const uint32_t rowidx = (uint32_t)(((int)bh * T + qi) * (T + (T & 1)));
+  f32x4 o[DT];
+#pragma unroll
+  for (int dt = 0; dt < DT; ++dt) o[dt] = (f32x4){0.f, 0.f, 0.f, 0.f};
+#pragma unroll
+  for (int c = 0; c < NKT / 2; ++c) {
+    if (2 * c < nkt) {
+      f32x4 pp[2] = {s[2 * c], s[2 * c + 1]};
+#pragma unroll
+      for (int hf = 0; hf < 2; ++hf) {
+        const int t = 2 * c + hf;
+        const float sc = t < nkt ? inv : 0.f;
+        if (a.drop_p > 0.f) {
+          float m[4];
+          const uint32_t base = rowidx + (uint32_t)(t * 16 + 4 * g);
+          drop_mul2(a.drop_p, s32, base, m[0], m[1]);
+          drop_mul2(a.drop_p, s32, base + 2, m[2], m[3]);
+#pragma unroll
+          for (int r = 0; r < 4; ++r) pp[hf][r] *= sc * m[r];
+        } else {
+#pragma unroll
+          for (int r = 0; r < 4; ++r) pp[hf][r] *= sc;
+        }
+      }
+      const bf16x8 pb = pack8(pp[0], pp[1]);
+#pragma unroll
+      for (int dt = 0; dt < DT; ++dt) o[dt] = mfma16(tr_frag(Vs, LD, 32 * c, 16 * dt, lane), pb, o[dt]);
+    }
+  }
+  if (qrow < a.T) {
+    bf16* O = a.out + (b * a.T + qrow) * a.ldout + h * DH;
+#pragma unroll
+    for (int dt = 0; dt < DT; ++dt) {
+      bf4 w;
+      w[0] = (bf16)o[dt][0]; w[1] = (bf16)o[dt][1]; w[2] = (bf16)o[dt][2]; w[3] = (bf16)o[dt][3];
+      *reinterpret_cast<bf4*>(O + 16 * dt + 4 * g) = w;
+    }
+  }
+}
+
+template <int DH>
 __global__ __launch_bounds__(NT) void attn_fwd_lds_kernel(AttnLdsArgs a) {
   constexpr int LD = Img<DH>::LD, KC = DH / 32, DT = DH / 16, NKT = 16;
   extern __shared__ __attribute__((aligned(16))) char smem[];
@@ -278,103 +375,17 @@
   if (wave >= NW / 2) __builtin_amdgcn_s_setprio(1);
 
   for (int qt = split + wave * a.nsplit; qt < nq; qt += NW * a.nsplit) {
-    const int q0 = qt * 16;
-    const int64_t qrow = q0 + cl;
     if (qt != split + wave * a.nsplit) {
+      const int64_t qrow = qt * 16 + cl;
 #pragma unroll
       for (int kc = 0; kc < KC; ++kc) qf[kc] = gload8(Qg, a.ldq, qrow, a.T, kc * 32 + 8 * g);
     }
-    const int nkt = a.mask_kind == 0 ? qt + 1 : nq;
-    const float sl2 = a.scale * LOG2E;
-    const int qi = q0 + cl;
-    f32x4 s[NKT];
-    float mx = NEG_INF;
-#pragma unroll
-    for (int kt = 0; kt < NKT; ++kt) {
-      s[kt] = (f32x4){0.f, 0.f, 0.f, 0.f};
-      if (kt < nkt) {
-#pragma unroll
-        for (int kc = 0; kc < KC; ++kc) s[kt] = mfma16(row_frag(Ks, LD, kt * 16 + cl, kc * 32 + 8 * g), qf[kc], s[kt]);
-        const bool need = a.mask_kind != 0 || kt == qt || kt * 16 + 16 > T;
-        const int kb = kt * 16 + 4 * g;
-        if (need) {
-          const f32x4 kmv = *reinterpret_cast<const f32x4*>(km + kb);
-#pragma unroll
-          for (int r = 0; r < 4; ++r) {
-            const int k = kb + r;
-            const bool dead = (k >= T) | ((a.mask_kind == 0) & (k > qi));
-            const float x = s[kt][r] * sl2;
-            s[kt][r] = dead ? NEG_INF : (kmv[r] != 0.f ? MASK2 : x);
-            mx = fmaxf(mx, s[kt][r]);
-          }
-        } else {
-#pragma unroll
-          for (int r = 0; r < 4; ++r) {
-            s[kt][r] *= sl2;
-            mx = fmaxf(mx, s[kt][r]);
-          }
-        }
-      }
-    }
-    mx = max_xor32(max_xor16(mx));
-    float sm = 0.f;
-#pragma unroll
-    for (int kt = 0; kt < NKT; ++kt) {
-      if (kt < nkt) {
-#pragma unroll
-        for (int r = 0; r < 4; ++r) {
-          const float e = ex2(s[kt][r] - mx);
-          s[kt][r] = e;
-          sm += e;
-        }
-      }
-    }
-    sm = add_xor32(add_xor16(sm));
-    const float inv = 1.f / sm;
-    if (g == 0 && qrow < a.T) a.lse[bh * a.T + qrow] = (mx + __builtin_amdgcn_logf(sm)) * LN2;
-    const uint32_t s32 = seed32(seed);
-    const uint32_t rowidx = (uint32_t)(((int)bh * T + qi) * (T + (T & 1)));
-    f32x4 o[DT];
-#pragma unroll
-    for (int dt = 0; dt < DT; ++dt) o[dt] = (f32x4){0.f, 0.f, 0.f, 0.f};
-#pragma unroll
-    for (int c = 0; c < NKT / 2; ++c) {
-      if (2 * c < nkt) {
-        f32x4 pp[2] = {s[2 * c], s[2 * c + 1]};
-#pragma unroll
-        for (int hf = 0; hf < 2; ++hf) {
-          const int t = 2 * c + hf;
-          const float sc = t < nkt ? inv : 0.f;
-          if (a.drop_p > 0.f) {
-            float m[4];
-            const uint32_t base = rowidx + (uint32_t)(t * 16 + 4 * g);
-            drop_mul2(a.drop_p, s32, base, m[0], m[1]);
-            drop_mul2(a.drop_p, s32, base + 2, m[2], m[3]);
-#pragma unroll
-            for (int r = 0; r < 4; ++r) pp[hf][r] *= sc * m[r];
-          } else {
-#pragma unroll
-            for (int r = 0; r < 4; ++r) pp[hf][r] *= sc;
-          }
-        }
-        const bf16x8 pb = pack8(pp[0], pp[1]);
-#pragma unroll
-        for (int dt = 0; dt < DT; ++dt) o[dt] = mfma16(tr_frag(Vs, LD, 32 * c, 16 * dt, lane), pb, o[dt]);
-      }
-    }
-    if (qrow < a.T) {
-      bf16* O = a.out + (b * a.T + qrow) * a.ldout + h * DH;
-#pragma unroll
-      for (int dt = 0; dt < DT; ++dt) {
-        bf4 w;
-        w[0] = (bf16)o[dt][0]; w[1] = (bf16)o[dt][1]; w[2] = (bf16)o[dt][2]; w[3] = (bf16)o[dt][3];
-        *reinterpret_cast<bf4*>(O + 16 * dt + 4 * g) = w;
-      }
-    }
+    attn_fwd_tile<DH>(a, Ks, Vs, km, qf, qt, bh, b, h, T, nq, seed, lane);
   }
   APROF(2);
 }
 
+#ifndef ATTN_LDS_DEVICE_ONLY
 template <int DH>
 __device__ __forceinline__ void attn_bwd_dq_body(const AttnLdsArgs& a, int64_t lin) {
   constexpr int LD = Img<DH>::LD, KC = DH / 32, DT = DH / 16;
@@ -854,6 +865,7 @@
 }
 
 static int fwd_split(const AttnLdsArgs& a) { return pick_split(a.B * a.H, (int)cdiv(a.T, 16)); }
+int attn_lds_fwd_nsplit(int64_t BH, int64_t T) { return pick_split(BH, (int)cdiv(T, 16)); }
 
 template <int DH>
 static hipError_t fwd_t(AttnLdsArgs& a, hipStream_t s) {
@@ -1024,3 +1036,4 @@
   if (Dh == 64) return bwd_t<64>(a, s);
   return bwd_t<32>(a, s);
 }
+#endif
diff --git a/recommender-baseline-model_amd/csrc/block_in_attn.hip b/recommender-baseline-model_amd/csrc/block_in_attn.hip
--- /dev/null
+++ b/recommender-baseline-model_amd/csrc/block_in_attn.hip
@@ -0,0 +1,243 @@
+#define RC_DEVICE_ONLY
+#include "rowchain.hip"
+#define ATTN_LDS_DEVICE_ONLY
+#include "attention_lds.hip"
+
+int attn_lds_fwd_nsplit(int64_t BH, int64_t T);
+bool attn_lds_supported(int64_t T, int64_t Dh);
+
+namespace ia {
+
+using rc::Lay;
+using rc::Raw;
+using rc::Tile;
+
+constexpr int WAVES = 8;
+
+template <int D> struct Slots {
+  static constexpr int WB = Lay<D>::WBYTES;
+  static constexpr size_t STATIC = (size_t)WB + 5 * D * 4 + WAVES * 4;
+};
+static __host__ __device__ inline int k_rows(int nq) { return 16 * nq; }
+static __host__ __device__ inline int v_rows(int nq) { return 32 * ((nq + 1) / 2); }
+template <int D> static size_t dyn_lds_bytes(int T) {
+  const int nq = (T + 15) / 16;
+  const size_t v = (size_t)v_rows(nq) * Img<D>::LD * 2 + (size_t)v_rows(nq) * 4, w = 2 * (size_t)Slots<D>::WB;
+  return (size_t)k_rows(nq) * Img<D>::LD * 2 + (v > w ? v : w);
+}
+
+__device__ __forceinline__ Tile seq_tile(int64_t b, int T, int t, int cl) {
+  Tile x;
+  const int row = 16 * t + cl;
+  x.ok = row < T;
+  x.m = b * T + row;
+  x.mc = x.ok ? x.m : b * T + T - 1;
+  return x;
+}
+__device__ __forceinline__ int other_tile(int i, int split, int ns, int ntile) {
+  if (ns == 1) return -1;
+  const int j = i % (ns - 1), t = (i / (ns - 1)) * ns + (j < split ? j : j + 1);
+  return t < ntile ? t : -1;
+}
+template <int D>
+__device__ __forceinline__ void put_rows(bf16* img, int t, const Raw<D>& r, bool ok, int g, int cl) {
+  bf16* p = img + (16 * t + cl) * Img<D>::LD + 8 * g;
+  bf16x8 z;
+#pragma unroll
+  for (int e = 0; e < 8; ++e) z[e] = (bf16)0.f;
+#pragma unroll
+  for (int s = 0; s < Lay<D>::S; ++s) *reinterpret_cast<bf16x8*>(p + 32 * s) = ok ? r.v[s] : z;
+}
+
+
+struct Args {
+  rs_sas_in_args in;
+  AttnLdsArgs a;
+  int ncount;
+};
+typedef const __attribute__((address_space(4))) Args* ArgsPtr;
+__device__ __forceinline__ ArgsPtr args_late() {
+  ArgsPtr kp = (ArgsPtr)__builtin_amdgcn_kernarg_segment_ptr();
+  asm volatile("" : "+s"(kp));
+  return kp;
+}
+
+template <int D>
+__global__ __launch_bounds__(64 * WAVES) void block_in_attn_kernel(Args k) {
+  const rs_sas_in_args& in = k.in;
+  const int ncount = k.ncount;
+  AttnLdsArgs a = {};
+  a.B = k.a.B, a.T = k.a.T, a.H = 1, a.nsplit = k.a.nsplit;
+  typedef Slots<D> SL;
+  constexpr int LD = Img<D>::LD, KC = D / 32;
+  __shared__ __attribute__((aligned(16))) char wv[SL::WB];
+  __shared__ __attribute__((aligned(16))) float lv[5 * D];
+  __shared__ int wcnt[WAVES];
+  extern __shared__ __attribute__((aligned(16))) char smem[];
+  const int tid = threadIdx.x, lane = tid & 63, wave = __builtin_amdgcn_readfirstlane(tid >> 6), g = lane >> 4,
+            cl = lane & 15;
+  int64_t b;
+  int split;
+  block_coords(a, b, split);
+  const int T = (int)a.T, nq = (T + 15) / 16, ns = a.nsplit;
+  const int ntile = last_tile_of_split(nq, split, ns) + 1;
+  bf16* Ks = reinterpret_cast<bf16*>(smem);
+  bf16* Vs = Ks + k_rows(nq) * LD;
+  float* km = reinterpret_cast<float*>(Vs + v_rows(nq) * LD);
+  char* wk = reinterpret_cast<char*>(Vs);
+  char* wq = wk + SL::WB;
+  const int qt = split + wave * ns;
+  const bool hasq = qt < nq;
+  const int oA = other_tile(WAVES - 1 - wave, split, ns, ntile);
+  const int tA = hasq ? qt : oA, tB = hasq ? oA : other_tile(2 * WAVES - 1 - wave, split, ns, ntile);
+  const bool hasA = tA >= 0, hasB = tB >= 0;
+  const Tile TA = seq_tile(b, T, hasA ? tA : 0, cl), TB = seq_tile(b, T, hasB ? tB : 0, cl);
+  const rs_sas_embed_args& e = in.e;
+  const uint32_t es32 = e.drop_p > 0.f ? seed32(eff_seed(e.salt, e.seed_base)) : 0u;
+  Raw<D> xa, xb;
+  int cnt = 0;
+  {
+    const int64_t cid = e.count_ids && hasq && TA.ok && g == 0 ? e.count_ids[TA.mc] : 0;
+    if (hasA) rc::embed_tile<D>(xa, e, TA, es32, g);
+    if (hasB) rc::embed_tile<D>(xb, e, TB, es32, g);
+    if (e.count_ids) cnt = __popcll(__ballot(cid != 0));
+    if (hasq) rc::store_raw<D>(e.x0, D, TA.m, TA.ok, xa, g);
+  }
+  rc::stage_slot<D>(wk, in.Wkv, D, wave, lane);
+  rc::stage_slot<D>(wq, in.Wq, D, wave, lane);
+  rc::stage_slot<D>(wv, in.Wkv + (int64_t)D * D, D, wave, lane);
+  {
+    const float* const V[5] = {in.ln_w, in.ln_b, in.bq, in.bkv, in.bkv + D};
+    rc::stage_v<D, 5>(lv, V, tid);
+  }
+  if (lane == 0) wcnt[wave] = cnt;
+  __syncthreads();
+  if (e.count_parts && tid == 0) {
+    int c = 0;
+#pragma unroll
+    for (int w = 0; w < WAVES; ++w) c += wcnt[w];
+    const int64_t nwg = (int64_t)ns * a.B, lin = blockIdx.x + (int64_t)ns * blockIdx.y;
+    e.count_parts[lin] = c;
+    for (int64_t i = lin + nwg; i < ncount; i += nwg) e.count_parts[i] = 0;
+  }
+  Tile SA = TA, SB = TB;
+  SA.ok = TA.ok && hasq;
+  SB.ok = false;
+  Raw<D> r;
+  if (hasB) {
+    Raw<D> r2;
+    rc::fwd_in_kv_half2<D>(xa, xb, SA, SB, rc::wimg(wk), lv, in.kv, 0, lane, r, r2);
+    put_rows<D>(Ks, tA, r, TA.ok, g, cl);
+    put_rows<D>(Ks, tB, r2, TB.ok, g, cl);
+  } else if (hasA) {
+    rc::fwd_in_kv_half<D>(xa, SA, rc::wimg(wk), lv, in.kv, 0, lane, r);
+    put_rows<D>(Ks, tA, r, TA.ok, g, cl);
+  }
+  bf16x8 qf[KC];
+  if (hasq) {
+    rc::fwd_in_q_x<D>(xa, TA, rc::wimg(wq), lv, in.eps, in.Q, in.mean, in.rstd, in.q, lane, r);
+#pragma unroll
+    for (int kc = 0; kc < KC; ++kc) {
+      typedef __attribute__((ext_vector_type(4))) unsigned u4;
+      u4 v = __builtin_bit_cast(u4, r.v[kc]);
+      v &= TA.ok ? 0xffffffffu : 0u;
+      qf[kc] = __builtin_bit_cast(bf16x8, v);
+    }
+  }
+  __syncthreads();
+  asm volatile("" ::: "memory");
+  for (int i = tid; i < v_rows(nq); i += 64 * WAVES) km[i] = 0.f;
+  if (ntile & 1) {
+    bf16x8 z;
+#pragma unroll
+    for (int kk = 0; kk < 8; ++kk) z[kk] = (bf16)0.f;
+    for (int i = tid; i < 16 * LD / 8; i += 64 * WAVES) reinterpret_cast<bf16x8*>(Vs + 16 * ntile * LD)[i] = z;
+  }
+  if (hasB) {
+    Raw<D> r2;
+    rc::fwd_in_kv_half2<D>(xa, xb, SA, SB, rc::wimg(wv), lv, in.kv, 1, lane, r, r2);
+    put_rows<D>(Vs, tA, r, TA.ok, g, cl);
+    put_rows<D>(Vs, tB, r2, TB.ok, g, cl);
+  } else if (hasA) {
+    rc::fwd_in_kv_half<D>(xa, SA, rc::wimg(wv), lv, in.kv, 1, lane, r);
+    put_rows<D>(Vs, tA, r, TA.ok, g, cl);
+  }
+  __syncthreads();
+  asm volatile("" ::: "memory");
+  if (!hasq) return;
+  {
+    const ArgsPtr kp = args_late();
+    a.out = kp->a.out, a.ldout = kp->a.ldout, a.lse = kp->a.lse, a.scale = kp->a.scale, a.mask_kind = 0;
+    a.drop_p = kp->a.drop_p, a.seed = kp->a.seed, a.seed_base = kp->a.seed_base;
+  }
+  const uint64_t seed = eff_seed(a.seed, a.seed_base);
+  if (wave >= WAVES / 2) __builtin_amdgcn_s_setprio(1);
+  attn_fwd_tile<D>(a, Ks, Vs, km, qf, qt, b, b, 0, T, nq, seed, lane);
+}
+
+static bool aligned16(const void* p) { return ((uintptr_t)p & 15) == 0; }
+
+static int plan(int64_t d, int64_t B, int64_t T, int* nsplit, size_t* lds) {
+  if (d != 64 && d != 128) return RS_ERR_UNSUPPORTED;
+  if (B <= 0 || T <= 0) return RS_ERR_ARG;
+  if (!attn_lds_supported(T, d) || B * T * (T + (T & 1)) >= ((int64_t)1 << 32)) return RS_ERR_UNSUPPORTED;
+  const int ns = attn_lds_fwd_nsplit(B, T), nq = (int)((T + 15) / 16);
+  if (ns > nq || (nq + ns - 1) / ns > WAVES) return RS_ERR_UNSUPPORTED;
+  const size_t dyn = d == 64 ? dyn_lds_bytes<64>((int)T) : dyn_lds_bytes<128>((int)T);
+  const size_t stat = d == 64 ? Slots<64>::STATIC : Slots<128>::STATIC;
+  if (dyn + stat > 160 * 1024) return RS_ERR_UNSUPPORTED;
+  *nsplit = ns;
+  *lds = dyn;
+  return 0;
+}
+
+template <int D>
+static int launch(const rs_sas_in_args& in, const AttnLdsArgs& a, int ncount, size_t lds, hipStream_t s) {
+  const void* fn = reinterpret_cast<const void*>(block_in_attn_kernel<D>);
+  (void)hipFuncSetAttribute(fn, hipFuncAttributeMaxDynamicSharedMemorySize, (int)lds);
+  const Args k = {in, a, ncount};
+  hipLaunchKernelGGL((block_in_attn_kernel<D>), dim3((unsigned)a.nsplit, (unsigned)a.B), dim3(64 * WAVES), lds, s, k);
+  return (int)hipGetLastError();
+}
+
+}
+
+extern "C" {
+
+int rs_sas_block_in_attn_nsplit(int64_t d, int64_t B, int64_t T) {
+  int ns = 0;
+  size_t lds = 0;
+  return ia::plan(d, B, T, &ns, &lds) == 0 ? ns : 0;
+}
+
+int rs_sas_block_in_attn(int64_t d, const rs_sas_in_attn_args* k, void* stream) {
+  if (!k || k->in.M <= 0 || k->B <= 0) return RS_ERR_ARG;
+  const rs_sas_in_args& in = k->in;
+  const rs_sas_embed_args& e = in.e;
+  if (e.T <= 0 || k->B * e.T != in.M) return RS_ERR_ARG;
+  if (!e.ids || !e.item_emb || !e.pos_emb || !e.x0 || !e.count_ids != !e.count_parts) return RS_ERR_ARG;
+  if (!in.ln_w || !in.ln_b || !in.Q || !in.mean || !in.rstd || !in.Wq || !in.bq || !in.q || !in.Wkv || !in.bkv ||
+      !in.kv || !k->o || !k->lse)
+    return RS_ERR_ARG;
+  if (!ia::aligned16(e.item_emb) || !ia::aligned16(e.pos_emb) || !ia::aligned16(e.x0) || !ia::aligned16(in.Q) ||
+      !ia::aligned16(in.q) || !ia::aligned16(in.kv) || !ia::aligned16(in.Wq) || !ia::aligned16(in.Wkv) ||
+      !ia::aligned16(k->o))
+    return RS_ERR_ARG;
+  int ns = 0;
+  size_t lds = 0;
+  const int pc = ia::plan(d, k->B, e.T, &ns, &lds);
+  if (pc) return pc;
+  if (e.count_parts && k->ncount < (int64_t)ns * k->B) return RS_ERR_ARG;
+  rs_sas_in_args a = in;
+  a.x = e.x0;
+  a.ldx = d;
+  AttnLdsArgs t = {};
+  t.B = k->B; t.T = e.T; t.H = 1;
+  t.out = (bf16*)k->o; t.ldout = d; t.lse = k->lse; t.scale = k->scale; t.mask_kind = 0; t.ids = e.ids;
+  t.drop_p = k->drop_p; t.seed = k->salt; t.seed_base = e.seed_base; t.nsplit = ns;
+  const int nc = (int)(k->ncount < 0x7fffffff ? k->ncount : 0x7fffffff);
+  return d == 64 ? ia::launch<64>(a, t, nc, lds, (hipStream_t)stream)
+                 : ia::launch<128>(a, t, nc, lds, (hipStream_t)stream);
+}
+
+}
diff --git a/recommender-baseline-model_amd/csrc/misc.hip b/recommender-baseline-model_amd/csrc/misc.hip
--- a/recommender-baseline-model_amd/csrc/misc.hip
+++ b/recommender-baseline-model_amd/csrc/misc.hip
@@ -535,6 +535,7 @@
     case RS_SIZEOF_SAS_OUT_ARGS: return sizeof(rs_sas_out_args);
     case RS_SIZEOF_SAS_OUT_BWD_ARGS: return sizeof(rs_sas_out_bwd_args);
     case RS_SIZEOF_SAS_IN_BWD_ARGS: return sizeof(rs_sas_in_bwd_args);
+    case RS_SIZEOF_SAS_IN_ATTN_ARGS: return sizeof(rs_sas_in_attn_args);
     default: return -1;
   }
 }
diff --git a/recommender-baseline-model_amd/csrc/rowchain.hip b/recommender-baseline-model_amd/csrc/rowchain.hip
--- a/recommender-baseline-model_amd/csrc/rowchain.hip
+++ b/recommender-baseline-model_amd/csrc/rowchain.hip
@@ -107,6 +107,32 @@
 #pragma unroll
     for (int s = 0; s < S; ++s)
       acc.v[j] = __builtin_amdgcn_mfma_f32_16x16x32_bf16(f[j & 1][s], b.v[s], acc.v[j], 0, 0, 0);
+    __builtin_amdgcn_sched_barrier(0);
+  }
+}
+template <int D>
+__device__ __forceinline__ void mm2(const bf16* wl, const Raw<D>& b0, const Raw<D>& b1, Act<D>& acc0, Act<D>& acc1,
+                                    int lane) {
+  constexpr int J = Lay<D>::J, S = Lay<D>::S;
+  const int g = lane >> 4, cl = lane & 15;
+  auto frag = [&](int j, int s) {
+    const int n = 16 * j + cl;
+    return *reinterpret_cast<const bf16x8*>(wl + n * D + 8 * ((4 * s + g) ^ swz<D>(n)));
+  };
+  bf16x8 f[2][S];
+#pragma unroll
+  for (int s = 0; s < S; ++s) f[0][s] = frag(0, s);
+#pragma unroll
+  for (int j = 0; j < J; ++j) {
+    if (j + 1 < J) {
+#pragma unroll
+      for (int s = 0; s < S; ++s) f[(j + 1) & 1][s] = frag(j + 1, s);
+    }
+#pragma unroll
+    for (int s = 0; s < S; ++s) {
+      acc0.v[j] = __builtin_amdgcn_mfma_f32_16x16x32_bf16(f[j & 1][s], b0.v[s], acc0.v[j], 0, 0, 0);
+      acc1.v[j] = __builtin_amdgcn_mfma_f32_16x16x32_bf16(f[j & 1][s], b1.v[s], acc1.v[j], 0, 0, 0);
+    }
     __builtin_amdgcn_sched_barrier(0);
   }
 }
@@ -292,8 +318,8 @@
   return x;
 }
 template <int D>
-__device__ __forceinline__ void fwd_in_q(const Raw<D>& xr, const Tile& T, const bf16* wq, const float* lv, float eps,
-                                         bf16* Q, float* mean, float* rstd, bf16* q, int lane) {
+__device__ __forceinline__ void fwd_in_q_x(const Raw<D>& xr, const Tile& T, const bf16* wq, const float* lv, float eps,
+                                           bf16* Q, float* mean, float* rstd, bf16* q, int lane, Raw<D>& r) {
   const int g = lane >> 4;
   Act<D> y;
   to_act<D>(y, xr);
@@ -311,24 +337,53 @@
   mm<D>(wq, Qr, acc, lane);
 #pragma unroll
   for (int j = 0; j < Lay<D>::J; ++j) acc.v[j] += vec4<D>(lv + 2 * D, j, g);
-  Raw<D> r;
   round_act<D>(acc, r);
   store_raw<D>(q, D, T.m, T.ok, r, g);
 }
 template <int D>
+__device__ __forceinline__ void fwd_in_q(const Raw<D>& xr, const Tile& T, const bf16* wq, const float* lv, float eps,
+                                         bf16* Q, float* mean, float* rstd, bf16* q, int lane) {
+  Raw<D> r;
+  fwd_in_q_x<D>(xr, T, wq, lv, eps, Q, mean, rstd, q, lane, r);
+}
+template <int D>
+__device__ __forceinline__ void fwd_in_kv_half(const Raw<D>& xr, const Tile& T, const bf16* w, const float* lv, bf16* kv,
+                                               int h, int lane, Raw<D>& r) {
+  const int g = lane >> 4;
+  Act<D> acc;
+  zero<D>(acc);
+  mm<D>(w, xr, acc, lane);
+#pragma unroll
+  for (int j = 0; j < Lay<D>::J; ++j) acc.v[j] += vec4<D>(lv + (3 + h) * D, j, g);
+  round_act<D>(acc, r);
+  store_raw<D>(kv + h * D, 2 * D, T.m, T.ok, r, g);
+}
+template <int D>
+__device__ __forceinline__ void fwd_in_kv_half2(const Raw<D>& x0, const Raw<D>& x1, const Tile& T0, const Tile& T1,
+                                                const bf16* w, const float* lv, bf16* kv, int h, int lane, Raw<D>& r0,
+                                                Raw<D>& r1) {
+  const int g = lane >> 4;
+  Act<D> a0, a1;
+  zero<D>(a0);
+  zero<D>(a1);
+  mm2<D>(w, x0, x1, a0, a1, lane);
+#pragma unroll
+  for (int j = 0; j < Lay<D>::J; ++j) {
+    a0.v[j] += vec4<D>(lv + (3 + h) * D, j, g);
+    a1.v[j] += vec4<D>(lv + (3 + h) * D, j, g);
+  }
+  round_act<D>(a0, r0);
+  round_act<D>(a1, r1);
+  store_raw<D>(kv + h * D, 2 * D, T0.m, T0.ok, r0, g);
+  store_raw<D>(kv + h * D, 2 * D, T1.m, T1.ok, r1, g);
+}
+template <int D>
 __device__ __forceinline__ void fwd_in_kv(const Raw<D>& xr, const Tile& T, const bf16* wk, const bf16* wv,
                                           const float* lv, bf16* kv, int lane) {
-  const int g = lane >> 4;
 #pragma unroll
   for (int h = 0; h < 2; ++h) {
-    Act<D> acc;
-    zero<D>(acc);
-    mm<D>(h == 0 ? wk : wv, xr, acc, lane);
-#pragma unroll
-    for (int j = 0; j < Lay<D>::J; ++j) acc.v[j] += vec4<D>(lv + (3 + h) * D, j, g);
     Raw<D> r;
-    round_act<D>(acc, r);
-    store_raw<D>(kv + h * D, 2 * D, T.m, T.ok, r, g);
+    fwd_in_kv_half<D>(xr, T, h == 0 ? wk : wv, lv, kv, h, lane, r);
   }
 }
 
@@ -1116,6 +1171,9 @@
   }
 }
 
+#ifdef RC_DEVICE_ONLY
+}
+#else
 static int g_ncu = 0;
 static int64_t grid_for(int64_t M) {
   if (g_ncu == 0) {
@@ -1332,3 +1390,4 @@
 }
 
 }
+#endif
diff --git a/recommender-baseline-model_amd/models/sas_model/sas.py b/recommender-baseline-model_amd/models/sas_model/sas.py
--- a/recommender-baseline-model_amd/models/sas_model/sas.py
+++ b/recommender-baseline-model_amd/models/sas_model/sas.py
@@ -206,6 +206,7 @@
         self._wT = None
         self.boundary_fuse = os.environ.get("RS_SAS_BOUNDARY_FUSE", "1") != "0"
         self.turnaround_fuse = os.environ.get("RS_SAS_TURNAROUND_FUSE", "1") != "0"
+        self.in_attn_fuse = os.environ.get("RS_SAS_IN_ATTN_FUSE", "1") != "0"
         salt0 = int(torch.randint(0, 2 ** 62, (1,)).item())
         self.salt = {"emb": site_salt(salt0, 0)}
         for i in range(self.L):
@@ -365,7 +366,14 @@
                     self.salt[f"ffn1_{i}"], self.salt[f"ffn2_{i}"], sb)
 
         ln_w, ln_b, Q, mu1, r1, Wq, bq, q, Wkv, bkv, kv = in_args(0)
-        if emb is not None:
+        in_attn = False
+        if emb is not None and self.in_attn_fuse and H == 1:
+            ns = ops.sas_block_in_attn_nsplit(d, B, T)
+            in_attn = ns >= 2 and (emb[-1] is None or emb[-1].numel() >= ns * B)
+        if in_attn:
+            ops.sas_block_in_attn(*emb, ln_w, ln_b, LN_EPS, Q, mu1, r1, Wq, bq, q, Wkv, bkv, kv, lay[0]["o"],
+                                  lay[0]["lse"], 1.0 / math.sqrt(Dh), self.salt["attn0"])
+        elif emb is not None:
             ops.sas_block_in_embed(*emb, ln_w, ln_b, LN_EPS, Q, mu1, r1, Wq, bq, q, Wkv, bkv, kv)
         else:
             ops.sas_block_in(x, ln_w, ln_b, LN_EPS, Q, mu1, r1, Wq, bq, q, Wkv, bkv, kv)
@@ -374,8 +382,9 @@
         xs = [x]
         for i in range(L):
             b = lay[i]
-            ops.attn_fwd(B, T, H, Dh, b["q"], b["kv"][:, :d], b["kv"][:, d:], b["o"], b["lse"], 1.0 / math.sqrt(Dh),
-                         0, ids, p, self.salt[f"attn{i}"], sb)
+            if i > 0 or not in_attn:
+                ops.attn_fwd(B, T, H, Dh, b["q"], b["kv"][:, :d], b["kv"][:, d:], b["o"], b["lse"],
+                             1.0 / math.sqrt(Dh), 0, ids, p, self.salt[f"attn{i}"], sb)
             if i + 1 < L:
                 ln_w, ln_b, Q, mu1, r1, Wq, bq, q, Wkv, bkv, kv = in_args(i + 1)
                 if self.boundary_fuse:
diff --git a/recommender-baseline-model_amd/ops.py b/recommender-baseline-model_amd/ops.py
--- a/recommender-baseline-model_amd/ops.py
+++ b/recommender-baseline-model_amd/ops.py
@@ -546,6 +546,24 @@
     call("rs_sas_block_in", d, C.byref(a), stream())
 
 
+def sas_block_in_attn_nsplit(d, B, T):
+    return int(_lib.lib().rs_sas_block_in_attn_nsplit(d, B, T))
+
+
+def sas_block_in_attn(ids, T, item_emb, pos_emb, scale, drop_p, salt, seed_base, x0, count_ids, count_parts,
+                      ln_w, ln_b, eps, Q, mean, rstd, Wq, bq, q, Wkv, bkv, kv, o, lse, attn_scale, attn_salt):
+    M, d = x0.shape
+    assert ids.numel() == M and M % T == 0 and item_emb.dtype == torch.bfloat16 and x0.dtype == torch.bfloat16
+    if count_parts is not None:
+        assert count_parts.dtype == torch.int32
+    e = _sas_args(_lib.SasEmbedArgs, ids=ids, item_emb=item_emb, pos_emb=pos_emb, T=T, scale=scale, drop_p=drop_p,
+                  salt=salt, seed_base=seed_base, x0=x0, count_ids=count_ids, count_parts=count_parts)
+    a = _sas_in(x0, ln_w, ln_b, eps, Q, mean, rstd, Wq, bq, q, Wkv, bkv, kv, embed=e)
+    k = _sas_args(_lib.SasInAttnArgs, B=M // T, o=o, lse=lse, scale=attn_scale, drop_p=drop_p, salt=attn_salt,
+                  ncount=0 if count_parts is None else count_parts.numel(), **{"in": a})
+    call("rs_sas_block_in_attn", d, C.byref(k), stream())
+
+
 def sas_block_out_head(out_args, E, pos, neg, lnl_w, lnl_b, count_parts, divisor, f, pl, nl, dpl, dnl, dx, lnpart,
                        part):
     M, d = out_args[0].shape
```

Result: faster. 509,000 sequences/s, median of 6 (+1.9%).
